# davidcombei/xAI-Audio-Deepfakes

Measured on AMD Instinct MI355X. Metric: explanations/sec (16 kHz, 4 s clips), higher is better.
Workload: dtype f32; 1 GPU; BASELINE config 2 extended to the full explanation: batch 64 x 4 s clips, STFT + wav2vec2-base embedder (to hidden layer 9) + logreg + U-Net mask decoder + masked ISTFT x2 + embedder re-forward x2 + LMAC metrics; batch_per_gpu=64, clip_samples=64000, embedder=wav2vec2-base (seeded random weights)

## Files before the change

include/addvisor_hip.h:

```cpp
#ifndef ADDVISOR_HIP_H
#define ADDVISOR_HIP_H

#include <stdint.h>

#ifdef __cplusplus
extern "C" {
#endif

typedef void* advh_stream_t;

enum {
    ADVH_OK = 0,
    ADVH_EINVAL = -1,
    ADVH_ELAUNCH = -2,
    ADVH_ENOTINIT = -3,
    ADVH_EUNSUPPORTED = -4
};

const char* advh_version(void);

int advh_init(void);

int advh_set_option(const char* name, int value);

int advh_stft_forward(const float* wave, int64_t wave_stride, int n_in, int B, int L, int hop, int win,
                      const float* window, float* X, float* mag, float* phase, int T, advh_stream_t stream);

enum { ADVH_MASK_NONE = 0, ADVH_MASK_LINEAR = 1, ADVH_MASK_LOG1P = 2 };
int advh_istft_masked(const float* mag, const float* phase, const float* mask, int Fm, int Tm, int mode,
                      float* wave_in, float* wave_out, int64_t wave_stride, int B, int T, int L, int hop,
                      int win, const float* window, advh_stream_t stream);

int advh_istft_masked_c64(const float* spec, const float* mask, int Fm, int Tm, int mode, float* wave_in, float* wave_out,
                          int64_t wave_stride, int B, int T, int L, int hop, int win, const float* window,
                          advh_stream_t stream);

int advh_istft_c64(const float* spec, float* wave, int64_t wave_stride, int B, int T, int L, int hop, int win,
                   const float* window, advh_stream_t stream);

int advh_istft_bandswap(const float* spec_a, const float* spec_b, int k0, int kw, int nbands, float* waves,
                        int64_t wave_stride, int64_t band_stride, int B, int T, int L, int hop, int win,
                        const float* window, advh_stream_t stream);

int advh_istft_masked_bwd(const float* g_wave, int64_t g_stride, const float* mag, const float* phase, const float* mask,
                          int Fm, int Tm, int mode, int which, float* dmask, int B, int T, int L, int hop, int win,
                          const float* window, advh_stream_t stream);

enum { ADVH_ACT_NONE = 0, ADVH_ACT_GELU = 1, ADVH_ACT_LEAKY = 2 };
enum { ADVH_TILE_AUTO = 0, ADVH_TILE_128x128 = 1, ADVH_TILE_256x64 = 2, ADVH_TILE_256x32 = 3,
       ADVH_TILE_256x128_W8 = 9, ADVH_TILE_128x256_W8 = 10  };

typedef struct advh_gemm_desc {
    const void* A0;
    const void* A1;
    const void* W;
    const int32_t* ktab;
    const float* bias;
    const void* resid;
    void* out_h;
    void* out_f;
    int32_t M, N, Ktot, w_rows;
    int32_t Hg, Wg, h0, h1, w0, w1, halo_zero;
    int64_t a_sB[2], a_sH[2], a_sW[2], a_c0[2], a_sZ[2];
    int64_t w_sZ, bias_sZ;
    int64_t o_sB, o_sH, o_sW, o_c0, o_sNhi, o_sZ;
    int32_t n_div, nz;
    int32_t act;
    float slope;
    int32_t resid_f32;
    int32_t ktab_identity;
    void* out_h2;
    float slope2;
    int32_t ph_r, ph_pad, ph_T;
    void* out_pre;
    const void* dact_src;
    int32_t wide;
    int64_t w_ld;
    int32_t sc;
    int32_t n_sub;
    int64_t o_sNhh;
    int32_t nz_lo, z_inner;
    int64_t a_sZ2[2];
    int64_t o_sZ2;
    int32_t plain;
    int32_t plain_out;
    int32_t split;
    int64_t a_lo[2];
    int64_t w_lo;
    int64_t o_lo;
} advh_gemm_desc;

int advh_gemm_f16(const advh_gemm_desc* desc, int tile, advh_stream_t stream);

int advh_w2v2_frontend(const float* wave, int64_t wave_stride, int n_in, int B, int L, const float* w0,
                       const float* bias0, const float* gamma, const float* beta, int mode, int normalize, float* stats_ws,
                       float* norm_ws, float* mr_ws, void* out, int T0, int P0, int C0, advh_stream_t stream);

int advh_layernorm(const void* in, int in_is_f32, int64_t in_ld, const float* gamma, const float* beta,
                   float* out_f, void* out_h, int64_t out_ld, int M, int C, float eps, int gelu,
                   advh_stream_t stream);
int advh_layernorm_add(const void* in, int in_is_f32, int64_t in_ld, const void* add_h, int64_t add_ld, const float* gamma,
                       const float* beta, float* out_f, void* out_h, int64_t out_ld, int M, int C, float eps, int gelu,
                       advh_stream_t stream);

int advh_posconv_gather(const float* h, void* xg, int B, int T, int H, int G, int K, int pad_left, const void* dact_src,
                        advh_stream_t stream);

typedef struct advh_posconv_desc {
    const void* xg;
    const void* W;
    const float* bias;
    const float* resid;
    float* out;
    int B, T, H, G, K;
} advh_posconv_desc;
int advh_posconv_tile_f16(const advh_posconv_desc* d, advh_stream_t stream);
int advh_posconv_tile_lds_bytes(int Cg, int T);

int advh_attention_f16(const void* qkv, void* ctx, int B, int T, int H, int heads, advh_stream_t stream);

int advh_pool_logreg(const float* h, const float* coef, float intercept, float* logit, float* prob,
                     float* pooled, int B, int T, int H, advh_stream_t stream);

int advh_unet_stem(const float* mag, int Fq, int Tq, int B, int H, int W, const float* wgt, const float* bias,
                   void* out, int PH, int PW, float slope, advh_stream_t stream);
int advh_unet_pack_x(const float* mag, int Fq, int Tq, int B, int H, int W, void* cat, int C, int c0, int PH, int PW,
                     advh_stream_t stream);
int advh_unet_head(const void* y, int B, int H, int W, int PH, int PW, const float* wgt, float bias, float* mask,
                   float* logits, advh_stream_t stream);

int advh_lmac_metrics_accumulate(const float* predictions, const float* theta_out, const float* masked_predictions,
                                 int n, double* sums6, float* per_clip, advh_stream_t stream);

int advh_hifigan_pack_mel(const float* mel, void* out, int B, int C, int T, int halo, advh_stream_t stream);
int advh_hifigan_pack_mel_pad(const float* mel, void* out, int B, int C, int T, int pad, int halo, advh_stream_t stream);
int advh_halo_fill_f16(void* x, int B, int T, int C, int halo, int mode, advh_stream_t stream);
int advh_hifigan_mrf_mix(const void* a, const void* b, const void* c, void* y, float slope, int64_t numel, advh_stream_t stream);
int advh_hifigan_conv_post(const void* x, const float* w, float bias, float* wav, int B, int C, int T, int halo, int k,
                           advh_stream_t stream);
int advh_mel_log(const float* mag, const float* fb, float* out, int B, int F, int T, int n_mels, advh_stream_t stream);

int advh_layernorm_bwd(const void* x, int x_is_f32, const void* dy, int dy_is_f32, const float* gamma, const float* beta,
                       int gelu_fwd, const float* add, const void* dact_src, float* out_f, void* out_h, int M, int C,
                       float eps, int remap_T, int remap_P, advh_stream_t stream);
int advh_attention_bwd_f16(const void* qkv, const void* dctx, void* dqkv, int B, int T, int H, int heads, advh_stream_t stream);
int advh_pool_logreg_bwd(const float* coef, const float* dlogit, float* dh, void* dh16, int B, int T, int H, advh_stream_t stream);
int advh_w2v2_frontend_bwd_group(const float* wave, int64_t wave_stride, int n_in, int B, int L, const float* w0,
                                 const float* gamma, const float* stats_ws, const float* norm_ws, const float* mr_ws,
                                 const void* dy0, float* part_ws, float* sums_ws, void* dz0, int T0, int P0, int C0,
                                 advh_stream_t stream);
int advh_wave_bwd(const float* g, const float* wave, int64_t wave_stride, int n_in, int B, int L, const float* stats_ws,
                  float* dxhat_ws, float* part_ws, int normalize, float out_scale, float* dx, int64_t dx_stride, int T0, int P0,
                  advh_stream_t stream);
int advh_scale_rows(const float* x, int x_rows, const float* alpha, float* y, int rows, int64_t n, int accumulate,
                    advh_stream_t stream);
int advh_attr_finalize(const float* g, const float* x, float* out, int mode, int64_t total, advh_stream_t stream);
int advh_time_mask(const float* attr, float* mask, float* wave_in, float* wave_out, const float* wave, int B, int64_t n,
                   advh_stream_t stream);

typedef struct advh_path_desc {
    const float* x;
    const float* base;
    const int32_t* bidx;
    int64_t n;
    uint64_t seed;
    int B, S, base_rows;
    int clip_major;
    float sigma;
} advh_path_desc;
int advh_attr_path_points(const advh_path_desc* d, const float* alpha, int64_t row0, int rows, float* out, advh_stream_t stream);
int advh_attr_path_accumulate(const advh_path_desc* d, const float* grad, const float* w, int mode, int64_t row0, int rows,
                              float* total, float* row_sum, advh_stream_t stream);
int advh_philox_normal(uint64_t seed, int64_t row0, int rows, int64_t n, int raw, float* out, advh_stream_t stream);

int advh_nt_fold(const float* attr, int B, int p, int64_t n, double* sum, double* sumsq, advh_stream_t stream);
int advh_nt_finalize(const double* sum, const double* sumsq, int B, int64_t n, int S, int nt_type, float* out, advh_stream_t stream);

typedef struct advh_metric_desc {
    const float* x;
    const float* attr;
    const float* base;
    int64_t n;
    uint64_t seed;
    int B, S, s0, p;
    int base_rows;
    int mode;
    int mul;
    float scale;
} advh_metric_desc;
int advh_metric_rows(const advh_metric_desc* d, int64_t row0, int rows, float* out, float* dot, advh_stream_t stream);
int advh_metric_row_dot(const float* pert, const float* attr, int B, int p, int64_t n, float* dot, advh_stream_t stream);
int advh_infidelity_fold(const float* dot, const float* f0, const float* fk, int B, int p, int normalize, double* acc, advh_stream_t stream);
int advh_infidelity_finalize(const double* acc, int B, int S, int normalize, float* out, advh_stream_t stream);
int advh_row_norm(const float* v, int rows, int64_t n, int ord, float* out, advh_stream_t stream);
int advh_sensitivity_fold(const float* e, const float* et, const float* enorm, int B, int p, int64_t n, int ord, float* ratio,
                          float* smax, advh_stream_t stream);

typedef struct advh_ablation_desc {
    const float* x;
    const float* base;
    const int32_t* mask;
    int64_t n;
    int B, base_rows, mask_rows;
    int mode;
    int win, stride;
    int K;
} advh_ablation_desc;
int advh_ablation_points(const advh_ablation_desc* d, int64_t row0, int rows, float* out, advh_stream_t stream);
int advh_ablation_accumulate(const advh_ablation_desc* d, const float* f0, const float* fk, float* attr, advh_stream_t stream);

typedef struct advh_coalition_desc {
    const float* x;
    const float* base;
    const int32_t* index;
    const int32_t* rank;
    const uint8_t* present;
    int64_t n;
    int64_t p0;
    int64_t rows;
    int B, base_rows, index_rows;
    int mode;
    int K;
    int P;
} advh_coalition_desc;
int advh_coalition_points(const advh_coalition_desc* d, int64_t row0, int rows, float* out, advh_stream_t stream);
int advh_shapley_accumulate(const advh_coalition_desc* d, const float* fbase, const float* fk, int64_t p0, int np, float* total,
                            float finalize_div, advh_stream_t stream);
int advh_coalition_scatter(const advh_coalition_desc* d, const float* coef, float* attr, advh_stream_t stream);

typedef struct advh_permutation_desc {
    const float* x;
    const int32_t* index;
    const int32_t* perm;
    int64_t n;
    int B, K;
} advh_permutation_desc;
int advh_permutation_points(const advh_permutation_desc* d, int64_t row0, int rows, float* out, advh_stream_t stream);
int advh_row_similarity(const float* rows_ptr, const float* x, int64_t row0, int rows, int B, int64_t n, int mode, float kernel_width,
                        float* sim, advh_stream_t stream);
int advh_lasso_cd(const double* X, const double* y, int S, int K, double alpha, double tol, int max_iter, double* coef, double* gap,
                  int* iters);

int advh_split_overflow(int reset);
int advh_w2v2_frontend_split(const float* wave, int64_t wave_stride, int n_in, int B, int L, const float* w0,
                             const float* bias0, const float* gamma, const float* beta, int mode, int normalize, float* stats_ws,
                             float* norm_ws, float* mr_ws, void* out, int64_t out_lo, int T0, int P0, int C0, advh_stream_t stream);
int advh_layernorm_split(const void* in, int in_is_f32, int64_t in_ld, int64_t in_lo, const void* add_h, int64_t add_ld,
                         int64_t add_lo, const float* gamma, const float* beta, float* out_f, void* out_h, int64_t out_ld,
                         int64_t out_lo, int M, int C, float eps, int gelu, advh_stream_t stream);
int advh_posconv_gather_split(const float* h, void* xg, int64_t xg_lo, int B, int T, int H, int G, int K, int pad_left,
                              advh_stream_t stream);
int advh_attention_split(const void* qkv, int64_t qkv_lo, void* ctx, int64_t ctx_lo, int B, int T, int H, int heads,
                         advh_stream_t stream);
int advh_unet_stem_split(const float* mag, int Fq, int Tq, int B, int H, int W, const float* wgt, const float* bias,
                         void* out, int64_t out_lo, int PH, int PW, float slope, advh_stream_t stream);
int advh_unet_pack_x_split(const float* mag, int Fq, int Tq, int B, int H, int W, void* cat, int64_t cat_lo, int C, int c0,
                           int PH, int PW, advh_stream_t stream);
int advh_unet_head_split(const void* y, int64_t y_lo, int B, int H, int W, int PH, int PW, const float* wgt, float bias,
                         float* mask, float* logits, advh_stream_t stream);
int advh_layernorm_bwd_split(const void* x, int x_is_f32, int64_t x_lo, const void* dy, int dy_is_f32, int64_t dy_lo,
                             const float* gamma, const float* beta, int gelu_fwd, const float* add, const void* dact_src,
                             int64_t dact_lo, float* out_f, void* out_h, int64_t out_lo, int M, int C, float eps, int remap_T,
                             int remap_P, advh_stream_t stream);
int advh_attention_bwd_split(const void* qkv, int64_t qkv_lo, const void* dctx, int64_t dctx_lo, void* dqkv, int64_t dqkv_lo,
                             int B, int T, int H, int heads, advh_stream_t stream);
int advh_pool_logreg_bwd_split(const float* coef, const float* dlogit, float* dh, void* dh16, int64_t dh16_lo, int B, int T, int H,
                               advh_stream_t stream);
int advh_split_f32(const float* src, void* dst, int64_t dst_lo, int64_t n, advh_stream_t stream);
int advh_posconv_gather_bwd_split(const float* dh, void* xg, int64_t xg_lo, int B, int T, int H, int G, int K, int pad_left,
                                  const void* dact_src, int64_t dact_lo, advh_stream_t stream);
int advh_w2v2_frontend_bwd_group_split(const float* wave, int64_t wave_stride, int n_in, int B, int L, const float* w0,
                                       const float* gamma, const float* stats_ws, const float* norm_ws, const float* mr_ws,
                                       const void* dy0, int64_t dy_lo, float* part_ws, float* sums_ws, void* dz0, int64_t dz_lo,
                                       int T0, int P0, int C0, advh_stream_t stream);
typedef struct advh_resblock_x3_desc {
    const void* X;
    const void* W1;
    const float* b1;
    const void* W2;
    const float* b2;
    void* out_h;
    int M, Wg, w0, w1, k, dil;
    float slope;
    int64_t x_lo, o_lo, w_lo;
} advh_resblock_x3_desc;
int advh_resblock_pair_x3_lds_bytes(int C, int k, int dil);
int advh_resblock_pair_x3(const advh_resblock_x3_desc* d, int C, advh_stream_t stream);
int advh_hifigan_pack_mel_split(const float* mel, void* out, int64_t out_lo, int B, int C, int T, int pad, int halo,
                                advh_stream_t stream);
int advh_hifigan_mrf_mix_split(const void* a, const void* b, const void* c, void* y, float slope, int64_t numel, int64_t lo,
                               advh_stream_t stream);
int advh_hifigan_conv_post_split(const void* x, int64_t x_lo, const float* w, float bias, float* wav, int B, int C, int T, int halo,
                                 int k, advh_stream_t stream);

typedef struct advh_taps_desc {
    const void* X;
    const void* W;
    const float* bias;
    const void* resid;
    void* out_h;
    void* out_h2;
    int M, Hg, Wg, h0, h1, w0, w1;
    int ntap;
    int toff[16];
    int act;
    float slope, slope2;
    int pre_act;
    float pre_slope;
} advh_taps_desc;
int advh_conv_taps_split_tile(int C, int ntap, int span);
int advh_conv_taps_split(const advh_taps_desc* d, int C, int64_t x_lo, int64_t w_lo, int64_t r_lo, int64_t o_lo, advh_stream_t stream);
typedef struct advh_taps2d_desc {
    const void* X;
    const void* W;
    const float* bias;
    void* out_h;
    int B, H, W_, PH, PW;
    int act;
    float slope;
} advh_taps2d_desc;
int advh_conv_taps2d_f16(const advh_taps2d_desc* d, int C, advh_stream_t stream);
int advh_conv_taps2d_split_lds_bytes(int C);
int advh_conv_taps2d_split(const advh_taps2d_desc* d, int C, int64_t x_lo, int64_t w_lo, int64_t o_lo, advh_stream_t stream);
typedef struct advh_upconv_desc {
    const void* Xc;
    const void* Xs;
    const void* W;
    const float* bias;
    void* out_h;
    int B, Hc, W_, PHc, PWc, PHs, PWs, PHo, PWo;
    int act;
    float slope;
} advh_upconv_desc;
int advh_upconv21_tile_f16(const advh_upconv_desc* d, advh_stream_t stream);
int advh_upconv21_tile_lds_bytes(void);
typedef struct advh_convs21_desc {
    const void* X;
    const void* W;
    const float* bias;
    void* out_h;
    int B, Ho, W_, PHi, PWi, PHo, PWo;
    int act;
    float slope;
} advh_convs21_desc;
int advh_conv53s21_tile_f16(const advh_convs21_desc* d, advh_stream_t stream);
int advh_conv53s21_tile_lds_bytes(void);
int advh_conv_taps_tile(int C, int ntap, int span);
int advh_conv_taps_lds_bytes(int C, int ntap, int span);
int advh_conv_taps_f16(const advh_taps_desc* d, int C, advh_stream_t stream);

typedef struct advh_map_geom { int B, H, W, C, PH, PW; } advh_map_geom;
int advh_bn_partial_count(void);
int advh_bn_coef(const float* sums, const float* gamma, const float* beta, int C, float n, float eps, float momentum,
                 float* running_mean, float* running_var, int64_t* num_batches_tracked, float* coef, advh_stream_t stream);
int advh_bn_bwd_coef(const float* sums, const float* coef, int C, float n, float inv_scale, float* coef_b, float* dgamma,
                     float* dbeta, advh_stream_t stream);
int advh_bn_stats(const void* z, const advh_map_geom* g, float* partial, float* sums, advh_stream_t stream);
int advh_bn_apply(const void* z, const advh_map_geom* g, const float* coef, float slope, void* a, advh_stream_t stream);
int advh_bn_bwd_sums(const void* z, const void* g_a, int g_f32, const advh_map_geom* g, const float* coef, float slope,
                     float* partial, float* sums, advh_stream_t stream);
int advh_bn_bwd_apply(const void* z, const void* g_a, int g_f32, const advh_map_geom* g, const float* coef, const float* coef_b, float slope,
                      void* dz, int64_t d_sB, int64_t d_sH, int64_t d_sW, int64_t d_c0, advh_stream_t stream);
typedef struct advh_transpose_desc {
    int B, Hg, Wg, GH, GW, H, W;
    int Hs, Ws, PHs, PWs, Cs, c0, nC;
    int sy, sx, ntap, oy[16], ox[16];
    int64_t ld, col0;
    int rpt, r0;
} advh_transpose_desc;
int advh_transpose_gather(const void* src, void* dst, const advh_transpose_desc* d, advh_stream_t stream);
int advh_unet_head_bwd(const float* dmask, const float* mask, const float* w32, float scale, int64_t total, float* dlogit,
                       void* dy1, int dy_f32, advh_stream_t stream);
int advh_unet_head_wgrad(const float* dlogit, const void* y1, int64_t total, float* partial, float* dw33, advh_stream_t stream);
int advh_unet_stem_wgrad(const void* dz, int Fq, int Tq, int B, int H, int W, const float* mag, int PH, int PW,
                         float* partial, float* dw, advh_stream_t stream);

int advh_bn_stats_split(const void* z, int64_t z_lo, const advh_map_geom* g, float* partial, float* sums, advh_stream_t stream);
int advh_bn_apply_split(const void* z, int64_t z_lo, const advh_map_geom* g, const float* coef, float slope, void* a, int64_t a_lo,
                        advh_stream_t stream);
int advh_bn_bwd_sums_split(const void* z, int64_t z_lo, const void* g_a, int64_t g_lo, const advh_map_geom* g, const float* coef,
                           float slope, float* partial, float* sums, advh_stream_t stream);
int advh_bn_bwd_apply_split(const void* z, int64_t z_lo, const void* g_a, int64_t g_lo, const advh_map_geom* g, const float* coef,
                            const float* coef_b, float slope, void* dz, int64_t dz_lo, int64_t d_sB, int64_t d_sH, int64_t d_sW,
                            int64_t d_c0, advh_stream_t stream);
int advh_unet_head_bwd_split(const float* dmask, const float* mask, const float* w32, float scale, int64_t total, float* dlogit,
                             void* dy1, int64_t dy_lo, advh_stream_t stream);
int advh_unet_head_wgrad_split(const float* dlogit, const void* y1, int64_t y_lo, int64_t total, float* partial, float* dw33,
                               advh_stream_t stream);
int advh_unet_stem_wgrad_split(const void* dz, int64_t dz_lo, int Fq, int Tq, int B, int H, int W, const float* mag, int PH, int PW,
                               float* partial, float* dw, advh_stream_t stream);
int advh_unet_skip_wgrad(const void* dz, int Fq, int Tq, int B, int H, int W, const float* mag, int PH, int PW, float* partial, float* dw,
                         advh_stream_t stream);
int advh_unet_skip_wgrad_split(const void* dz, int64_t dz_lo, int Fq, int Tq, int B, int H, int W, const float* mag, int PH, int PW,
                               float* partial, float* dw, advh_stream_t stream);

typedef struct advh_wgrad2d_desc {
    const void* X;
    const void* DZ;
    float* partial;
    int B, H, W_, PHx, PWx, PHz, PWz;
} advh_wgrad2d_desc;
int advh_conv_wgrad2d_parts(int C, int B, int H, int W);
int advh_conv_wgrad2d_f16(const advh_wgrad2d_desc* d, int C, float* dw, advh_stream_t stream);
int advh_conv_wgrad2d_split_parts(int CI, int CO, int B, int H, int W);
int advh_conv_wgrad2d_split(const advh_wgrad2d_desc* d, int CI, int CO, int Cx, int cx0, int Cz, int cz0, int64_t x_lo, int64_t dz_lo,
                            float* dw, advh_stream_t stream);

typedef struct advh_resblock_desc {
    const void* X;
    const void* W1;
    const float* b1;
    const void* W2;
    const float* b2;
    void* out_h;
    int M, Wg, w0, w1, k, dil;
    float slope;
} advh_resblock_desc;
int advh_resblock_pair_lds_bytes(int C, int k, int dil);
int advh_resblock_pair_f16(const advh_resblock_desc* d, int C, advh_stream_t stream);

#ifdef __cplusplus
}
#endif
#endif
```

xai-audio-deepfakes_amd/addvisor_hip/_lib.py:

```python
from __future__ import annotations

import ctypes as C
import os
import subprocess

_HERE = os.path.dirname(os.path.abspath(__file__))
LIB_PATH = os.environ.get("ADDVISOR_HIP_LIB") or os.path.join(_HERE, "libaddvisor_hip.so")
CSRC = os.path.join(os.path.dirname(_HERE), "csrc")

ERRORS = {-1: "ADVH_EINVAL (bad argument)", -2: "ADVH_ELAUNCH (HIP launch failed)",
          -3: "ADVH_ENOTINIT (advh_init not called)", -4: "ADVH_EUNSUPPORTED"}


class AdvhError(RuntimeError):
    pass


def build(verbose: bool = False) -> str:
    r = subprocess.run(["make", "-C", CSRC, "-j8"], capture_output=True, text=True)
    if r.returncode != 0:
        raise AdvhError("building libaddvisor_hip.so failed:\n" + r.stdout[-4000:] + r.stderr[-4000:])
    if verbose:
        print(r.stdout)
    return LIB_PATH


_p, _i, _i64, _f = C.c_void_p, C.c_int, C.c_int64, C.c_float

SIGNATURES = {
    "advh_version": (C.c_char_p, []),
    "advh_init": (_i, []),
    "advh_set_option": (_i, [C.c_char_p, _i]),
    "advh_stft_forward": (_i, [_p, _i64, _i, _i, _i, _i, _i, _p, _p, _p, _p, _i, _p]),
    "advh_istft_masked": (_i, [_p, _p, _p, _i, _i, _i, _p, _p, _i64, _i, _i, _i, _i, _i, _p, _p]),
    "advh_istft_masked_c64": (_i, [_p, _p, _i, _i, _i, _p, _p, _i64, _i, _i, _i, _i, _i, _p, _p]),
    "advh_istft_c64": (_i, [_p, _p, _i64, _i, _i, _i, _i, _i, _p, _p]),
    "advh_gemm_f16": (_i, [_p, _i, _p]),
    "advh_w2v2_frontend": (_i, [_p, _i64, _i, _i, _i, _p, _p, _p, _p, _i, _i, _p, _p, _p, _p, _i, _i, _i, _p]),
    "advh_layernorm": (_i, [_p, _i, _i64, _p, _p, _p, _p, _i64, _i, _i, _f, _i, _p]),
    "advh_layernorm_add": (_i, [_p, _i, _i64, _p, _i64, _p, _p, _p, _p, _i64, _i, _i, _f, _i, _p]),
    "advh_posconv_gather": (_i, [_p, _p, _i, _i, _i, _i, _i, _i, _p, _p]),
    "advh_attention_f16": (_i, [_p, _p, _i, _i, _i, _i, _p]),
    "advh_pool_logreg": (_i, [_p, _p, _f, _p, _p, _p, _i, _i, _i, _p]),
    "advh_unet_stem": (_i, [_p, _i, _i, _i, _i, _i, _p, _p, _p, _i, _i, _f, _p]),
    "advh_unet_pack_x": (_i, [_p, _i, _i, _i, _i, _i, _p, _i, _i, _i, _i, _p]),
    "advh_unet_head": (_i, [_p, _i, _i, _i, _i, _i, _p, _f, _p, _p, _p]),
    "advh_lmac_metrics_accumulate": (_i, [_p, _p, _p, _i, _p, _p, _p]),
    "advh_hifigan_pack_mel": (_i, [_p, _p, _i, _i, _i, _i, _p]),
    "advh_hifigan_pack_mel_pad": (_i, [_p, _p, _i, _i, _i, _i, _i, _p]),
    "advh_halo_fill_f16": (_i, [_p, _i, _i, _i, _i, _i, _p]),
    "advh_hifigan_mrf_mix": (_i, [_p, _p, _p, _p, _f, _i64, _p]),
    "advh_hifigan_conv_post": (_i, [_p, _p, _f, _p, _i, _i, _i, _i, _i, _p]),
    "advh_mel_log": (_i, [_p, _p, _p, _i, _i, _i, _i, _p]),
    "advh_layernorm_bwd": (_i, [_p, _i, _p, _i, _p, _p, _i, _p, _p, _p, _p, _i, _i, _f, _i, _i, _p]),
    "advh_attention_bwd_f16": (_i, [_p, _p, _p, _i, _i, _i, _i, _p]),
    "advh_pool_logreg_bwd": (_i, [_p, _p, _p, _p, _i, _i, _i, _p]),
    "advh_w2v2_frontend_bwd_group": (_i, [_p, _i64, _i, _i, _i, _p, _p, _p, _p, _p, _p, _p, _p, _p, _i, _i, _i, _p]),
    "advh_wave_bwd": (_i, [_p, _p, _i64, _i, _i, _i, _p, _p, _p, _i, _f, _p, _i64, _i, _i, _p]),
    "advh_scale_rows": (_i, [_p, _i, _p, _p, _i, _i64, _i, _p]),
    "advh_attr_finalize": (_i, [_p, _p, _p, _i, _i64, _p]),
    "advh_time_mask": (_i, [_p, _p, _p, _p, _p, _i, _i64, _p]),
    "advh_attr_path_points": (_i, [_p, _p, _i64, _i, _p, _p]),
    "advh_attr_path_accumulate": (_i, [_p, _p, _p, _i, _i64, _i, _p, _p, _p]),
    "advh_philox_normal": (_i, [C.c_uint64, _i64, _i, _i64, _i, _p, _p]),
    "advh_nt_fold": (_i, [_p, _i, _i, _i64, _p, _p, _p]),
    "advh_nt_finalize": (_i, [_p, _p, _i, _i64, _i, _i, _p, _p]),
    "advh_metric_rows": (_i, [_p, _i64, _i, _p, _p, _p]),
    "advh_metric_row_dot": (_i, [_p, _p, _i, _i, _i64, _p, _p]),
    "advh_infidelity_fold": (_i, [_p, _p, _p, _i, _i, _i, _p, _p]),
    "advh_infidelity_finalize": (_i, [_p, _i, _i, _i, _p, _p]),
    "advh_row_norm": (_i, [_p, _i, _i64, _i, _p, _p]),
    "advh_sensitivity_fold": (_i, [_p, _p, _p, _i, _i, _i64, _i, _p, _p, _p]),
    "advh_ablation_points": (_i, [_p, _i64, _i, _p, _p]),
    "advh_ablation_accumulate": (_i, [_p, _p, _p, _p, _p]),
    "advh_coalition_points": (_i, [_p, _i64, _i, _p, _p]),
    "advh_shapley_accumulate": (_i, [_p, _p, _p, _i64, _i, _p, _f, _p]),
    "advh_coalition_scatter": (_i, [_p, _p, _p, _p]),
    "advh_permutation_points": (_i, [_p, _i64, _i, _p, _p]),
    "advh_row_similarity": (_i, [_p, _p, _i64, _i, _i, _i64, _i, _f, _p, _p]),
    "advh_lasso_cd": (_i, [_p, _p, _i, _i, C.c_double, C.c_double, _i, _p, _p, _p]),
    "advh_istft_masked_bwd": (_i, [_p, _i64, _p, _p, _p, _i, _i, _i, _i, _p, _i, _i, _i, _i, _i, _p, _p]),
    "advh_istft_bandswap": (_i, [_p, _p, _i, _i, _i, _p, _i64, _i64, _i, _i, _i, _i, _i, _p, _p]),
    "advh_bn_partial_count": (_i, []),
    "advh_bn_stats": (_i, [_p, _p, _p, _p, _p]),
    "advh_bn_coef": (_i, [_p, _p, _p, _i, _f, _f, _f, _p, _p, _p, _p, _p]),
    "advh_bn_bwd_coef": (_i, [_p, _p, _i, _f, _f, _p, _p, _p, _p]),
    "advh_bn_apply": (_i, [_p, _p, _p, _f, _p, _p]),
    "advh_bn_bwd_sums": (_i, [_p, _p, _i, _p, _p, _f, _p, _p, _p]),
    "advh_bn_bwd_apply": (_i, [_p, _p, _i, _p, _p, _p, _f, _p, _i64, _i64, _i64, _i64, _p]),
    "advh_transpose_gather": (_i, [_p, _p, _p, _p]),
    "advh_split_f32": (_i, [_p, _p, _i64, _i64, _p]),
    "advh_unet_head_bwd": (_i, [_p, _p, _p, _f, _i64, _p, _p, _i, _p]),
    "advh_unet_head_wgrad": (_i, [_p, _p, _i64, _p, _p, _p]),
    "advh_unet_stem_wgrad": (_i, [_p, _i, _i, _i, _i, _i, _p, _i, _i, _p, _p, _p]),
    "advh_conv_wgrad2d_parts": (_i, [_i, _i, _i, _i]),
    "advh_conv_wgrad2d_f16": (_i, [_p, _i, _p, _p]),
    "advh_conv_wgrad2d_split_parts": (_i, [_i, _i, _i, _i, _i]),
    "advh_conv_wgrad2d_split": (_i, [_p, _i, _i, _i, _i, _i, _i, _i64, _i64, _p, _p]),
    "advh_resblock_pair_lds_bytes": (_i, [_i, _i, _i]),
    "advh_resblock_pair_f16": (_i, [_p, _i, _p]),
    "advh_conv_taps_tile": (_i, [_i, _i, _i]),
    "advh_conv_taps_lds_bytes": (_i, [_i, _i, _i]),
    "advh_conv_taps_f16": (_i, [_p, _i, _p]),
    "advh_conv_taps_split_tile": (_i, [_i, _i, _i]),
    "advh_conv_taps_split": (_i, [_p, _i, _i64, _i64, _i64, _i64, _p]),
    "advh_conv_taps2d_f16": (_i, [_p, _i, _p]),
    "advh_conv_taps2d_split_lds_bytes": (_i, [_i]),
    "advh_conv_taps2d_split": (_i, [_p, _i, _i64, _i64, _i64, _p]),
    "advh_upconv21_tile_f16": (_i, [_p, _p]),
    "advh_posconv_tile_f16": (_i, [_p, _p]),
    "advh_conv53s21_tile_f16": (_i, [_p, _p]),
    "advh_conv53s21_tile_lds_bytes": (_i, []),
    "advh_posconv_tile_lds_bytes": (_i, [_i, _i]),
    "advh_w2v2_frontend_split": (_i, [_p, _i64, _i, _i, _i, _p, _p, _p, _p, _i, _i, _p, _p, _p, _p, _i64, _i, _i, _i, _p]),
    "advh_layernorm_split": (_i, [_p, _i, _i64, _i64, _p, _i64, _i64, _p, _p, _p, _p, _i64, _i64, _i, _i, _f, _i, _p]),
    "advh_posconv_gather_split": (_i, [_p, _p, _i64, _i, _i, _i, _i, _i, _i, _p]),
    "advh_attention_split": (_i, [_p, _i64, _p, _i64, _i, _i, _i, _i, _p]),
    "advh_unet_stem_split": (_i, [_p, _i, _i, _i, _i, _i, _p, _p, _p, _i64, _i, _i, _f, _p]),
    "advh_unet_pack_x_split": (_i, [_p, _i, _i, _i, _i, _i, _p, _i64, _i, _i, _i, _i, _p]),
    "advh_hifigan_pack_mel_split": (_i, [_p, _p, _i64, _i, _i, _i, _i, _i, _p]),
    "advh_hifigan_mrf_mix_split": (_i, [_p, _p, _p, _p, _f, _i64, _i64, _p]),
    "advh_hifigan_conv_post_split": (_i, [_p, _i64, _p, _f, _p, _i, _i, _i, _i, _i, _p]),
    "advh_unet_head_split": (_i, [_p, _i64, _i, _i, _i, _i, _i, _p, _f, _p, _p, _p]),
    "advh_upconv21_tile_lds_bytes": (_i, []),
    "advh_bn_stats_split": (_i, [_p, _i64, _p, _p, _p, _p]),
    "advh_bn_apply_split": (_i, [_p, _i64, _p, _p, _f, _p, _i64, _p]),
    "advh_bn_bwd_sums_split": (_i, [_p, _i64, _p, _i64, _p, _p, _f, _p, _p, _p]),
    "advh_bn_bwd_apply_split": (_i, [_p, _i64, _p, _i64, _p, _p, _p, _f, _p, _i64, _i64, _i64, _i64, _i64, _p]),
    "advh_unet_head_bwd_split": (_i, [_p, _p, _p, _f, _i64, _p, _p, _i64, _p]),
    "advh_unet_head_wgrad_split": (_i, [_p, _p, _i64, _i64, _p, _p, _p]),
    "advh_unet_stem_wgrad_split": (_i, [_p, _i64, _i, _i, _i, _i, _i, _p, _i, _i, _p, _p, _p]),
    "advh_unet_skip_wgrad": (_i, [_p, _i, _i, _i, _i, _i, _p, _i, _i, _p, _p, _p]),
    "advh_unet_skip_wgrad_split": (_i, [_p, _i64, _i, _i, _i, _i, _i, _p, _i, _i, _p, _p, _p]),
    "advh_split_overflow": (_i, [_i]),
    "advh_resblock_pair_x3_lds_bytes": (_i, [_i, _i, _i]),
    "advh_resblock_pair_x3": (_i, [_p, _i, _p]),
    "advh_layernorm_bwd_split": (_i, [_p, _i, _i64, _p, _i, _i64, _p, _p, _i, _p, _p, _i64, _p, _p, _i64, _i, _i, _f, _i, _i, _p]),
    "advh_attention_bwd_split": (_i, [_p, _i64, _p, _i64, _p, _i64, _i, _i, _i, _i, _p]),
    "advh_pool_logreg_bwd_split": (_i, [_p, _p, _p, _p, _i64, _i, _i, _i, _p]),
    "advh_posconv_gather_bwd_split": (_i, [_p, _p, _i64, _i, _i, _i, _i, _i, _i, _p, _i64, _p]),
    "advh_w2v2_frontend_bwd_group_split": (_i, [_p, _i64, _i, _i, _i, _p, _p, _p, _p, _p, _p, _i64, _p, _p, _p, _i64, _i, _i, _i, _p]),
}

_lib = None


def lib() -> C.CDLL:
    global _lib
    if _lib is None:
        import torch
        if not os.path.exists(LIB_PATH):
            raise AdvhError(f"{LIB_PATH} is missing: run `python -c 'import __graft_entry__ as g; g.build()'` "
                            "(there is no fallback path)")
        l = C.CDLL(LIB_PATH)
        for name, (res, args) in SIGNATURES.items():
            fn = getattr(l, name)
            fn.restype, fn.argtypes = res, args
        _lib = l
    return _lib


class SplitRangeError(AdvhError, FloatingPointError):
    """A kernel of the fp32-class mode met a value outside the split format's range (|x| > 65504)."""


def check_overflow(what: str = "") -> None:
    if _lib is not None and _lib.advh_split_overflow(1):
        raise SplitRangeError((what + ": " if what else "") + "a value left the fp32-class format's range (|x| > 65504 between two "
                              "matrix products): the split planes saturated.  Scale the input / weights, or run precision='f16' "
                              "diagnostics; the reference's fp32 has no such limit (include/addvisor_hip.h, advh_split_overflow)")


def check(rc: int, what: str) -> None:
    if rc != 0:
        raise AdvhError(f"{what}: {ERRORS.get(rc, rc)}")
    check_overflow(what)


_inited = set()


def init() -> None:
    import torch
    dev = torch.cuda.current_device() if torch.cuda.is_available() else -1
    if dev not in _inited:
        check(lib().advh_init(), "advh_init")
        _inited.add(dev)
```

xai-audio-deepfakes_amd/addvisor_hip/gemm.py:

```python
from __future__ import annotations

import ctypes as C
import os
from dataclasses import dataclass
from typing import Optional, Sequence, Tuple

import numpy as np
import torch

from . import _lib

BK = 64
ACT = {"none": 0, "gelu": 1, "leaky": 2}
WIDE_EPILOGUE = os.environ.get("ADDVISOR_GEMM_WIDE", "1") != "0"


def packed_row_channel(rows: int) -> np.ndarray:
    R = np.arange(rows)
    return ((R >> 5) << 5) + (((R >> 2) & 3) << 3) + (((R >> 4) & 1) << 2) + (R & 3)
TILE_AUTO, TILE_128x128, TILE_256x64, TILE_256x32 = 0, 1, 2, 3
TILE_256x128_W8, TILE_128x256_W8 = 9, 10
TILE_BN = {TILE_128x128: 128, TILE_256x64: 64, TILE_256x32: 32, TILE_256x128_W8: 128, TILE_128x256_W8: 256}
TILE_NAMES = {TILE_128x128: "128x128", TILE_256x64: "256x64", TILE_256x32: "256x32", TILE_256x128_W8: "256x128w8", TILE_128x256_W8: "128x256w8"}
TILE_KERNELS = {TILE_128x128: "gemm_f16_kernel<128, 128, 2, 2, 4>", TILE_128x256_W8: "gemm_f16_kernel<128, 256, 2, 4, 3>",
                TILE_256x128_W8: "gemm_f16_kernel<256, 128, 4, 2, 3>"}


class GemmDesc(C.Structure):
    _fields_ = [
        ("A0", C.c_void_p), ("A1", C.c_void_p), ("W", C.c_void_p), ("ktab", C.c_void_p),
        ("bias", C.c_void_p), ("resid", C.c_void_p), ("out_h", C.c_void_p), ("out_f", C.c_void_p),
        ("M", C.c_int32), ("N", C.c_int32), ("Ktot", C.c_int32), ("w_rows", C.c_int32),
        ("Hg", C.c_int32), ("Wg", C.c_int32), ("h0", C.c_int32), ("h1", C.c_int32),
        ("w0", C.c_int32), ("w1", C.c_int32), ("halo_zero", C.c_int32),
        ("a_sB", C.c_int64 * 2), ("a_sH", C.c_int64 * 2), ("a_sW", C.c_int64 * 2),
        ("a_c0", C.c_int64 * 2), ("a_sZ", C.c_int64 * 2),
        ("w_sZ", C.c_int64), ("bias_sZ", C.c_int64),
        ("o_sB", C.c_int64), ("o_sH", C.c_int64), ("o_sW", C.c_int64), ("o_c0", C.c_int64),
        ("o_sNhi", C.c_int64), ("o_sZ", C.c_int64),
        ("n_div", C.c_int32), ("nz", C.c_int32), ("act", C.c_int32), ("slope", C.c_float),
        ("resid_f32", C.c_int32), ("ktab_identity", C.c_int32),
        ("out_h2", C.c_void_p), ("slope2", C.c_float), ("ph_r", C.c_int32), ("ph_pad", C.c_int32), ("ph_T", C.c_int32),
        ("out_pre", C.c_void_p), ("dact_src", C.c_void_p), ("wide", C.c_int32), ("w_ld", C.c_int64), ("sc", C.c_int32), ("n_sub", C.c_int32), ("o_sNhh", C.c_int64),
        ("nz_lo", C.c_int32), ("z_inner", C.c_int32), ("a_sZ2", C.c_int64 * 2), ("o_sZ2", C.c_int64), ("plain", C.c_int32), ("plain_out", C.c_int32),
        ("split", C.c_int32), ("a_lo", C.c_int64 * 2), ("w_lo", C.c_int64), ("o_lo", C.c_int64),
    ]


X3_KERNELS = {TILE_128x128: "gemm_x3_kernel<128, 128, 2, 2", TILE_256x64: "gemm_x3_kernel<256, 64, 4, 1", TILE_256x32: "gemm_x3_kernel<256, 32, 4, 1"}


def kernel_name(tile: int, plain: bool, split: bool = False) -> str:
    if split:
        return X3_KERNELS[tile] + (", true>" if plain else ", false>")
    k = TILE_KERNELS.get(tile, "gemm_f16_kernel")
    if k.startswith("gemm_f16_kernel<"):
        k = k[:-1] + (", true>" if plain and tile == TILE_128x128 else ", false>")
    return k


class _Profile:

    def __init__(self):
        self.reset(False)

    def reset(self, enabled: bool):
        self.enabled, self.events = enabled, []

    def summary(self, kernel=None):
        per = {}
        for a, b, f, t, shape in self.events:
            r = per.setdefault(kernel_name(t, shape[4], shape[5] if len(shape) > 5 else False), [0.0, 0.0, 0])
            r[0] += a.elapsed_time(b); r[1] += f; r[2] += 1
        if not per:
            return 0.0, 0.0, 0
        if kernel is None:
            kernel = max(per, key=lambda k: per[k][0])
        self.kernel = kernel
        return tuple(per.get(kernel, (0.0, 0.0, 0)))

    def by_shape(self):
        per = {}
        for a, b, f, t, shape in self.events:
            r = per.setdefault(shape[:4] + (TILE_NAMES.get(t, str(t)) + ("+" if shape[4] else "") + ("x3" if len(shape) > 5 and shape[5] else ""),), [0.0, 0.0, 0])
            r[0] += a.elapsed_time(b); r[1] += f; r[2] += 1
        return per


PROFILE = _Profile()


class _Tuner:
    active = False
    log = []


TUNER = _Tuner()


def round_up(x: int, m: int) -> int:
    return (x + m - 1) // m * m


def split_planes(x: torch.Tensor) -> torch.Tensor:
    if x.is_cuda and x.dtype == torch.float32 and x.numel() % 4 == 0:
        src = x.detach().contiguous()
        if src.data_ptr() % 16:
            src = src.clone()
        out = torch.empty((2,) + tuple(src.shape), dtype=torch.float16, device=src.device)
        if src.numel():
            _lib.check(_lib.lib().advh_split_f32(src.data_ptr(), out.data_ptr(), src.numel(), src.numel(),
                                                 torch.cuda.current_stream(src.device).cuda_stream), "advh_split_f32")
        return out
    x64 = x.detach().to(torch.float64)
    bad = ~(x64.abs() <= 65504.0)
    if bool(bad.any()):
        raise ValueError(f"split format: {int(bad.sum())} value(s) outside |x| <= 65504 (or NaN); max |x| = {float(x64.abs().nan_to_num(float('inf')).max()):g}")
    hi = x64.to(torch.float16)
    hi = torch.where(x64.abs() < 2.0 ** -14, torch.zeros_like(hi), hi)
    lo = ((x64 - hi.to(torch.float64)) * 2048.0).to(torch.float16)
    return torch.stack([hi, lo])


def join_planes(t: torch.Tensor) -> torch.Tensor:
    return t[0].float() + t[1].float() * (1.0 / 2048.0)


W8_RULE = int(os.environ.get("ADDVISOR_GEMM_W8_MIN_M", "0"))
X3_SUPER_COLUMN_BYTES = int(os.environ.get("ADDVISOR_X3_SC_BYTES", "1600000"))
SUPER_COLUMN_BYTES = int(os.environ.get("ADDVISOR_GEMM_SC_BYTES", "1600000"))


def super_columns(N: int, Kp: int, M: int, bn: int = 128, split: bool = False) -> int:
    bpe = 4 if split else 2
    budget = X3_SUPER_COLUMN_BYTES if split else SUPER_COLUMN_BYTES
    if budget <= 0 or N <= bn:
        return 0
    tiles_n = (N + bn - 1) // bn
    if tiles_n * bn * Kp * bpe <= 3 * 1024 * 1024:
        return 0
    sc = min(tiles_n, budget // (bn * Kp * bpe))
    return sc if sc >= (3 if split else 4) else 0


PLAIN_ROWS = os.environ.get("ADDVISOR_GEMM_PLAIN", "1") != "0"


def pick_tile(N: int, M: int = 0) -> Tuple[int, int]:
    if N <= 32:
        return TILE_256x32, 32
    if N <= 64:
        return TILE_256x64, 64
    return TILE_128x128, 128


@dataclass
class Source:
    sB: int
    sH: int
    sW: int
    c0: int
    sZ: int = 0
    sZ2: int = 0


class GemmPlan:

    def __init__(self, *, M: int, N: int, w2: torch.Tensor, ktab: np.ndarray, sources: Sequence[Source],
                 Hg: int, Wg: int, window: Tuple[int, int, int, int], halo_zero: bool,
                 out: Tuple[int, int, int, int], n_div: Optional[int] = None, o_sNhi: int = 0,
                 o_sZ: int = 0, nz: int = 1, bias: Optional[torch.Tensor] = None, act: str = "none",
                 slope: float = 0.0, device=None, w_sZ: Optional[int] = None, bias_sZ: int = 0,
                 slope2: float = 0.0, phase: Tuple[int, int, int] = (0, 0, 0), cache: Optional[tuple] = None,
                 n_sub: int = 0, o_sNhh: int = 0, nz_lo: int = 0, z_inner: bool = False, o_sZ2: int = 0, plain: bool = False,
                 split: bool = False):
        K = 8 * len(ktab)
        self.split = bool(split)
        Kp = round_up(K, BK)
        n_div_v = n_div if n_div is not None else round_up(N, 4)
        wide = WIDE_EPILOGUE and N % 8 == 0 and n_div_v % 8 == 0 and all(int(x) % 8 == 0 for x in (*out, o_sNhi, o_sZ, o_sNhh, o_sZ2))
        tile, BN = pick_tile(N, M)
        if W8_RULE and N % 256 == 0 and M >= W8_RULE and bool((np.asarray(ktab) == np.arange(len(ktab))).all()):
            tile, BN = TILE_128x256_W8, 256
        w_rows = round_up(N, 256)
        store, ckey = cache if cache is not None else (None, None)
        hit = store.get(ckey) if store is not None else None
        if hit is None:
            w2t = w2() if callable(w2) else w2
            assert w2t.dim() == 3 and w2t.shape[0] == nz and w2t.shape[1] == N and w2t.shape[2] == K, (w2t.shape, nz, N, K)
            wp = torch.zeros(((2, nz, w_rows, Kp) if split else (nz, w_rows, Kp)), dtype=torch.float16)
            w16 = split_planes(w2t) if split else w2t.to(torch.float16)
            if wide:
                src = packed_row_channel(w_rows)
                keep = src < N
                wp[..., torch.from_numpy(np.nonzero(keep)[0]), :K] = w16[..., torch.from_numpy(src[keep]), :]
            else:
                wp[..., :N, :K] = w16
            wd = wp.to(device) if device is not None else wp
            bd = None
            if bias is not None:
                assert bias.numel() == nz * N or bias_sZ == 0
                bd = bias.to(torch.float32).contiguous()
                bd = bd.to(device) if device is not None else bd
            hit = (wd, bd, wide)
            if store is not None:
                store[ckey] = hit
        assert hit[2] == wide, "a cached packed weight is shared between plans of different output alignment"
        kt = np.concatenate([ktab, np.full((Kp - K) // 8, ktab[0], dtype=np.int64)]).astype(np.int64)
        assert (kt & 0x7FFFFFFF).max() < 2 ** 31
        self.ktab_host = kt
        self.K, self.Kp, self.tile, self.BN = K, Kp, tile, BN
        self.device = device
        self.w, self.bias = hit[0], hit[1]
        kt32 = torch.from_numpy(kt.astype(np.uint32).view(np.int32).copy())
        self.ktab = kt32.to(device) if device is not None else kt32
        d = GemmDesc()
        d.M, d.N, d.Ktot, d.w_rows = M, N, Kp, w_rows
        d.Hg, d.Wg = Hg, Wg
        d.h0, d.h1, d.w0, d.w1 = window
        d.halo_zero = int(halo_zero)
        for s, src in enumerate(sources):
            d.a_sB[s], d.a_sH[s], d.a_sW[s], d.a_c0[s], d.a_sZ[s] = src.sB, src.sH, src.sW, src.c0, src.sZ
            d.a_sZ2[s] = src.sZ2
        d.w_sZ = w_rows * Kp if w_sZ is None else w_sZ
        d.split = int(split)
        d.w_lo = nz * w_rows * Kp if split else 0
        assert not split or w_sZ is None
        d.bias_sZ = bias_sZ
        d.o_sB, d.o_sH, d.o_sW, d.o_c0 = out
        d.o_sNhi, d.o_sZ = o_sNhi, o_sZ
        d.n_sub, d.o_sNhh = n_sub, o_sNhh
        d.nz_lo, d.z_inner, d.o_sZ2 = nz_lo, int(z_inner), o_sZ2
        assert nz_lo <= 1 or nz % nz_lo == 0
        d.n_div = n_div_v
        d.wide = int(wide)
        d.nz = nz
        d.act, d.slope = ACT[act], slope
        d.slope2 = slope2
        d.ph_r, d.ph_pad, d.ph_T = phase
        d.ktab_identity = int(bool((kt == np.arange(len(kt))).all()))
        d.plain = int(bool(plain and PLAIN_ROWS and d.ktab_identity and len(sources) == 1))
        if d.plain:
            src = sources[0]
            assert Hg == 1 or src.sH == Wg * src.sW, "plain rows need h * a_sH == (h * Wg) * a_sW"
            assert M <= Hg * Wg or src.sB == Hg * Wg * src.sW, "plain rows need b * a_sB == (b * Hg * Wg) * a_sW"
        o_sB, o_sH, o_sW, _ = out
        d.plain_out = int(bool(d.plain and n_div_v >= N and phase[0] == 0 and n_sub <= 1 and tuple(window) == (0, Hg, 0, Wg)
                               and (Hg == 1 or o_sH == Wg * o_sW) and (M <= Hg * Wg or o_sB == Hg * Wg * o_sW)))
        d.sc = super_columns(N, Kp, M, 128, split)
        self.desc = d
        self.nsrc = len(sources)
        self.flops = 2.0 * M * N * K * nz

    def load_weights(self, w2: torch.Tensor, bias: Optional[torch.Tensor] = None):
        N, K = self.desc.N, self.K
        assert w2.shape == (self.desc.nz, N, K) and w2.device == self.w.device, (w2.shape, (self.desc.nz, N, K))
        w16 = split_planes(w2) if self.split else w2.to(torch.float16)
        if self.desc.wide:
            if not hasattr(self, "_perm"):
                src = packed_row_channel(self.w.shape[-2])
                keep = np.nonzero(src < N)[0]
                self._perm = (torch.from_numpy(keep).to(self.w.device), torch.from_numpy(src[keep]).to(self.w.device))
            dst_rows, src_rows = self._perm
            self.w[..., dst_rows, :K] = w16[..., src_rows, :]
        else:
            self.w[..., :N, :K] = w16
        if bias is not None:
            self.bias.copy_(bias.reshape(self.bias.shape).to(torch.float32))

    def run(self, A0: torch.Tensor, A1: Optional[torch.Tensor] = None, *, out_h: Optional[torch.Tensor] = None,
            out_f: Optional[torch.Tensor] = None, resid: Optional[torch.Tensor] = None, stream: Optional[int] = None,
            out_h2: Optional[torch.Tensor] = None, out_pre: Optional[torch.Tensor] = None,
            dact_src: Optional[torch.Tensor] = None):
        d = self.desc
        d.out_h2 = out_h2.data_ptr() if out_h2 is not None else None
        d.out_pre = out_pre.data_ptr() if out_pre is not None else None
        d.dact_src = dact_src.data_ptr() if dact_src is not None else None
        assert out_pre is None or out_pre.dtype == torch.float16
        assert dact_src is None or dact_src.dtype == torch.float16
        assert A0.dtype == torch.float16 and A0.is_cuda
        if self.split:
            o_lo = None
            for s_, t in enumerate((A0, A1)):
                if t is not None:
                    assert t.shape[0] == 2 and t.stride(0) % 8 == 0, "split operand must be a [2, ...] plane pair"
                    d.a_lo[s_] = t.stride(0) // 8
            for t in (out_h, out_h2, out_pre, dact_src, resid if (resid is not None and resid.dtype == torch.float16) else None):
                if t is not None:
                    assert t.shape[0] == 2 and t.stride(0) % 8 == 0 and o_lo in (None, t.stride(0)), "split outputs share one plane pitch"
                    o_lo = t.stride(0)
            d.o_lo = o_lo or 0
        d.A0 = A0.data_ptr()
        d.A1 = A1.data_ptr() if A1 is not None else None
        assert (A1 is not None) == (self.nsrc == 2)
        if d.plain:
            plane = A0.stride(0) if self.split else A0.numel()
            need = (int(d.a_c0[0]) + (d.M - 1) * int(d.a_sW[0])) * 8 + d.Ktot + int(d.a_sZ[0]) * 8 * max(0, d.nz - 1)
            if need > plane:
                raise ValueError(f"affine-row GEMM operand too small: the plan reads {need} halfs per plane, the tensor holds {plane} "
                                 "(missing slack rows behind the buffer?)")
        d.W, d.ktab = self.w.data_ptr(), self.ktab.data_ptr()
        d.bias = self.bias.data_ptr() if self.bias is not None else None
        d.out_h = out_h.data_ptr() if out_h is not None else None
        d.out_f = out_f.data_ptr() if out_f is not None else None
        if out_h is not None:
            assert out_h.dtype == torch.float16
        if out_f is not None:
            assert out_f.dtype == torch.float32
        if resid is not None:
            assert resid.dtype in (torch.float16, torch.float32)
            d.resid, d.resid_f32 = resid.data_ptr(), int(resid.dtype == torch.float32)
        else:
            d.resid, d.resid_f32 = None, 0
        if stream is None:
            stream = torch.cuda.current_stream().cuda_stream
        if self.split:
            d.sc = super_columns(d.N, self.Kp, d.M, TILE_BN.get(self.tile, 128), True)
        if TUNER.active and not getattr(self, "_tuned", False):
            self._tune(d, stream)
        prof = PROFILE.enabled and self.tile not in (TILE_256x64, TILE_256x32)
        if prof:
            e0, e1 = torch.cuda.Event(enable_timing=True), torch.cuda.Event(enable_timing=True)
            e0.record()
        _lib.check(_lib.lib().advh_gemm_f16(C.byref(d), self.tile, stream), "advh_gemm_f16")
        if prof:
            e1.record()
            PROFILE.events.append((e0, e1, self.flops, self.tile, (self.desc.M, self.desc.N, self.K, self.desc.nz, bool(self.desc.plain), self.split)))


def _tune(self, d, stream):
    cands = [TILE_128x128, TILE_128x256_W8, TILE_256x128_W8] if (self.desc.N > 64 and not self.split) else [self.tile]
    best, best_ms = self.tile, None
    if len(cands) > 1:
        for t in cands:
            _lib.check(_lib.lib().advh_gemm_f16(C.byref(d), t, stream), "advh_gemm_f16")
            e0, e1 = torch.cuda.Event(enable_timing=True), torch.cuda.Event(enable_timing=True)
            e0.record()
            for _ in range(3):
                _lib.check(_lib.lib().advh_gemm_f16(C.byref(d), t, stream), "advh_gemm_f16")
            e1.record()
            e1.synchronize()
            ms = e0.elapsed_time(e1) / 3
            if best_ms is None or ms < best_ms:
                best, best_ms = t, ms
        TUNER.log.append((self.desc.M, self.desc.N, self.K, self.desc.nz, TILE_NAMES[best], best_ms))
    self.tile, self._tuned = best, True


GemmPlan._tune = _tune


@dataclass
class FMap:
    B: int
    H: int
    W: int
    C: int
    PH: int
    PW: int
    t: Optional[torch.Tensor] = None
    split: bool = False

    @property
    def Hp(self):
        return self.H + 2 * self.PH

    @property
    def Wp(self):
        return self.W + 2 * self.PW

    def alloc(self, device):
        shape = (self.B, self.Hp, self.Wp, self.C)
        self.t = torch.zeros(((2,) + shape) if self.split else shape, dtype=torch.float16, device=device)
        return self

    def interior(self) -> torch.Tensor:
        t = self.t[0] if self.split else self.t
        return t[:, self.PH:self.PH + self.H, self.PW:self.PW + self.W, :]


def plan_linear(M: int, weight: torch.Tensor, bias: Optional[torch.Tensor], *, lda: Optional[int] = None,
                ldo: Optional[int] = None, o_c0: int = 0, act: str = "none", device=None, cache=None,
                split: bool = False) -> GemmPlan:
    N, K = weight.shape
    assert K % 8 == 0
    lda = K if lda is None else lda
    ldo = N if ldo is None else ldo
    assert lda % 8 == 0 and ldo % 4 == 0
    return GemmPlan(M=M, N=N, w2=lambda: weight[None].float(), ktab=np.arange(K // 8, dtype=np.int64),
                    sources=[Source(0, 0, lda // 8, 0)], Hg=1, Wg=M, window=(0, 1, 0, M), halo_zero=False,
                    out=(0, 0, ldo, o_c0), bias=bias, act=act, device=device, cache=cache, plain=True, split=split)


def plan_conv1d_cl(B: int, P_in: int, P_out: int, L_out: int, weight: torch.Tensor, bias: Optional[torch.Tensor],
                   stride: int, *, act: str = "gelu", compact_out: bool = False, device=None, cache=None,
                   slack_rows: int = 0, split: bool = False) -> GemmPlan:
    Cout, Cin, k = weight.shape
    assert Cin % 8 == 0
    w2 = lambda: weight.permute(0, 2, 1).reshape(1, Cout, k * Cin).float()
    out = (L_out * Cout, 0, Cout, 0) if compact_out else (P_out * Cout, 0, Cout, 0)
    return GemmPlan(M=B * P_out, N=Cout, w2=w2, ktab=np.arange(k * Cin // 8, dtype=np.int64),
                    sources=[Source(P_in * Cin // 8, 0, stride * Cin // 8, 0)], Hg=1, Wg=P_out,
                    window=(0, 1, 0, L_out), halo_zero=not compact_out, out=out, bias=bias, act=act, device=device,
                    cache=cache, plain=(slack_rows >= k - stride and P_in == P_out * stride), split=split)


def plan_conv2d(srcs: Sequence[FMap], dst: FMap, weight: torch.Tensor, bias: Optional[torch.Tensor], *,
                stride=(1, 1), padding=(1, 1), dilation=(1, 1), act: str = "leaky", slope: float = 0.2,
                dst_c0: int = 0, device=None) -> GemmPlan:
    Cout, Cin, KH, KW = weight.shape
    assert sum(s.C for s in srcs) == Cin and len(srcs) <= 2
    sh, sw = stride
    ph, pw = padding
    dh, dw = dilation
    B = dst.B
    Ho = (srcs[0].H + 2 * ph - dh * (KH - 1) - 1) // sh + 1
    Wo = (srcs[0].W + 2 * pw - dw * (KW - 1) - 1) // sw + 1
    assert (Ho, Wo) == (dst.H, dst.W), ((Ho, Wo), (dst.H, dst.W))
    ktabs, ws, sources = [], [], []
    c_lo = 0
    for s, f in enumerate(srcs):
        assert f.C % 8 == 0 and f.PH >= ph and f.PW >= pw and (f.H, f.W, f.B) == (srcs[0].H, srcs[0].W, B)
        cc = f.C // 8
        taps = (np.arange(KH)[:, None] * dh * f.Wp + np.arange(KW)[None, :] * dw).reshape(-1)
        kt = (taps[:, None] * cc + np.arange(cc)[None, :]).reshape(-1).astype(np.int64) | (s << 31)
        ktabs.append(kt)
        ws.append(weight[:, c_lo:c_lo + f.C].permute(0, 2, 3, 1).reshape(Cout, KH * KW * f.C))
        c0 = ((-sh * dst.PH + f.PH - ph) * f.Wp + (-sw * dst.PW + f.PW - pw)) * cc
        sources.append(Source(f.Hp * f.Wp * cc, sh * f.Wp * cc, sw * cc, c0))
        c_lo += f.C
    Ct = dst.C
    split = dst.split
    assert all(f.split == split for f in srcs)
    return GemmPlan(M=B * dst.Hp * dst.Wp, N=Cout, w2=torch.cat(ws, 1)[None] if split else torch.cat(ws, 1)[None].float(), ktab=np.concatenate(ktabs), split=split,
                    sources=sources, Hg=dst.Hp, Wg=dst.Wp,
                    window=(dst.PH, dst.PH + dst.H, dst.PW, dst.PW + dst.W), halo_zero=True,
                    out=(dst.Hp * dst.Wp * Ct, dst.Wp * Ct, Ct, dst_c0), bias=bias, act=act, slope=slope,
                    device=device)


def plan_convT2d(src: FMap, dst: FMap, weight: torch.Tensor, bias: torch.Tensor, *, stride, dst_c0: int = 0,
                 device=None) -> GemmPlan:
    Cin, Cout, KH, KW = weight.shape
    sh, sw = stride
    assert (KH, KW) == (sh, sw) and src.C == Cin and Cin % 8 == 0 and Cout % 4 == 0
    assert (dst.H, dst.W) == (src.H * sh, src.W * sw)
    cc = Cin // 8
    Ct = dst.C
    w2 = weight.permute(2, 3, 1, 0).reshape(1, sh * sw * Cout, Cin)
    w2 = w2 if dst.split else w2.float()
    assert src.split == dst.split
    b2 = bias.float().repeat(sh * sw)
    o_c0 = ((-sh * src.PH + dst.PH) * dst.Wp + (-sw * src.PW + dst.PW)) * Ct + dst_c0
    return GemmPlan(M=src.B * src.Hp * src.Wp, N=sh * sw * Cout, w2=w2, ktab=np.arange(cc, dtype=np.int64),
                    sources=[Source(src.Hp * src.Wp * cc, src.Wp * cc, cc, 0)], Hg=src.Hp, Wg=src.Wp,
                    window=(src.PH, src.PH + src.H, src.PW, src.PW + src.W), halo_zero=False,
                    out=(dst.Hp * dst.Wp * Ct, sh * dst.Wp * Ct, sw * Ct, o_c0), n_div=Cout,
                    o_sNhi=Ct if sw > 1 else dst.Wp * Ct, n_sub=sw if sw > 1 else 0, o_sNhh=dst.Wp * Ct if sw > 1 else 0,
                    bias=b2, bias_sZ=0, act="none", device=device, split=dst.split)


class PlanGroup:

    def __init__(self, plans: Sequence[GemmPlan], flops: float):
        self.plans, self.flops = list(plans), flops
        self.tile = self.plans[0].tile

    def run(self, A0: torch.Tensor, A1: Optional[torch.Tensor] = None, *, out_h: torch.Tensor, stream: Optional[int] = None):
        for p in self.plans:
            p.run(A0, A1, out_h=out_h, stream=stream)


def add_indicator(f: FMap, channel: int) -> FMap:
    f.interior()[..., channel] = 1.0
    return f


def compose_upconv_weights(wt: torch.Tensor, bt: torch.Tensor, wc: torch.Tensor, stride, indicator: Tuple[str, int]):
    sh, sw = stride
    Cb, Cu = wt.shape[:2]
    N, Cs = wc.shape[0], wc.shape[1] - Cu
    where, ich = indicator
    assert where in ("coarse", "skip") and ich >= (Cb if where == "coarse" else Cs)
    wt64, wc64, bt64 = wt.double(), wc.double(), bt.double()
    nth, ntw = 2, (2 if sw == 2 else 3)
    cu0 = (max(Cb, ich + 1 if where == "coarse" else 0) + 7) // 8
    cu1 = (max(Cs, ich + 1 if where == "skip" else 0) + 7) // 8
    w1 = torch.zeros(N, 3, 3, cu1 * 8, dtype=torch.float64)
    w1[..., :Cs] = wc64[:, Cu:].permute(0, 2, 3, 1)
    if where == "skip":
        w1[..., ich] = torch.einsum("nukl,u->nkl", wc64[:, :Cu], bt64)
    w2 = []
    for ph in range(sh):
        dh_min = (ph - 1) // sh
        for pw in range(sw):
            dw_min = (pw - 1) // sw
            w0 = torch.zeros(N, nth, ntw, cu0 * 8, dtype=torch.float64)
            for kh in range(3):
                for kw in range(3):
                    r, c = ph + kh - 1, pw + kw - 1
                    ti, tj = r // sh - dh_min, c // sw - dw_min
                    w0[:, ti, tj, :Cb] += torch.einsum("nu,bu->nb", wc64[:, :Cu, kh, kw], wt64[:, :, r % sh, c % sw])
                    if where == "coarse":
                        w0[:, ti, tj, ich] += wc64[:, :Cu, kh, kw] @ bt64
            w2.append(torch.cat([w0.reshape(N, -1), w1.reshape(N, -1)], 1))
    return w2, cu0, cu1


def plan_upconv2d(coarse: FMap, skip: FMap, dst: FMap, wt: torch.Tensor, bt: torch.Tensor, wc: torch.Tensor,
                  bc: torch.Tensor, *, stride, coarse_C: int, skip_C: int, indicator: Tuple[str, int],
                  slope: float = 0.2, device=None) -> PlanGroup:
    sh, sw = stride
    Cb, Cu = wt.shape[:2]
    N = wc.shape[0]
    Cs = wc.shape[1] - Cu
    assert (wt.shape[2], wt.shape[3]) == (sh, sw) and sh == 2 and sw in (1, 2) and wc.shape[2:] == (3, 3)
    assert coarse_C == Cb and skip_C == Cs and coarse.C >= Cb and skip.C >= Cs and coarse.C % 8 == 0 and skip.C % 8 == 0
    assert (dst.H, dst.W) == (coarse.H * sh, coarse.W * sw) == (skip.H, skip.W) and dst.B == coarse.B == skip.B
    assert coarse.PH >= 1 and coarse.PW >= 1 and skip.PH >= 1 and skip.PW >= 1 and dst.C % 8 == 0
    nth, ntw = 2, (2 if sw == 2 else 3)
    cc0, cc1, Ct = coarse.C // 8, skip.C // 8, dst.C
    w2, cu0, cu1 = compose_upconv_weights(wt, bt, wc, stride, indicator)
    assert cu0 <= cc0 and cu1 <= cc1
    where = indicator[0]
    kt1 = ((np.arange(3)[:, None] * skip.Wp + np.arange(3)[None, :]).reshape(-1)[:, None] * cc1
           + np.arange(cu1)[None, :]).reshape(-1).astype(np.int64) | (1 << 31)
    kt0 = ((np.arange(nth)[:, None] * coarse.Wp + np.arange(ntw)[None, :]).reshape(-1)[:, None] * cc0
           + np.arange(cu0)[None, :]).reshape(-1).astype(np.int64)
    c0_0 = ((coarse.PH - 1) * coarse.Wp + coarse.PW - 1) * cc0
    c0_1 = ((skip.PH - 1) * skip.Wp + skip.PW - 1) * cc1
    o_c0 = (dst.PH * dst.Wp + dst.PW) * Ct
    plan = GemmPlan(
        M=coarse.B * coarse.H * coarse.W, N=N, w2=torch.stack(w2) if dst.split else torch.stack(w2).float(), ktab=np.concatenate([kt0, kt1]), split=dst.split,
        sources=[Source(coarse.Hp * coarse.Wp * cc0, coarse.Wp * cc0, cc0, c0_0, sZ=coarse.Wp * cc0, sZ2=cc0 if sw == 2 else 0),
                 Source(skip.Hp * skip.Wp * cc1, sh * skip.Wp * cc1, sw * cc1, c0_1, sZ=skip.Wp * cc1, sZ2=cc1 if sw == 2 else 0)],
        Hg=coarse.H, Wg=coarse.W, window=(0, coarse.H, 0, coarse.W), halo_zero=False,
        out=(dst.Hp * dst.Wp * Ct, sh * dst.Wp * Ct, sw * Ct, o_c0), o_sZ=dst.Wp * Ct, o_sZ2=Ct if sw == 2 else 0,
        nz=sh * sw, nz_lo=sw, z_inner=os.environ.get("ADDVISOR_UPCONV_Z_INNER", "1") != "0", bias=bc, bias_sZ=0, act="leaky", slope=slope, device=device)
    plans = [plan]
    flops = 2.0 * dst.B * dst.H * dst.W * N * (nth * ntw * Cb + 9 * Cs + (nth * ntw if where == "coarse" else 9))
    return PlanGroup(plans, flops)


class ConvS21Desc(C.Structure):
    _fields_ = [("X", C.c_void_p), ("W", C.c_void_p), ("bias", C.c_void_p), ("out_h", C.c_void_p), ("B", C.c_int),
                ("Ho", C.c_int), ("W_", C.c_int), ("PHi", C.c_int), ("PWi", C.c_int), ("PHo", C.c_int), ("PWo", C.c_int),
                ("act", C.c_int), ("slope", C.c_float)]


def conv_s21_supported(srcs: Sequence[FMap], dst: FMap, weight: torch.Tensor, stride=(1, 1), padding=(1, 1),
                       dilation=(1, 1)) -> bool:
    return (len(srcs) == 1 and tuple(weight.shape) == (64, 32, 5, 3) and tuple(stride) == (2, 1) and tuple(padding) == (2, 1)
            and tuple(dilation) == (1, 1) and srcs[0].C == 32 and dst.C == 64 and srcs[0].PH >= 2 and srcs[0].PW >= 1
            and srcs[0].H == 2 * dst.H and srcs[0].W == dst.W)


class ConvS21TilePlan:

    def __init__(self, src: FMap, dst: FMap, weight: torch.Tensor, bias: torch.Tensor, *, slope: float = 0.2, device=None):
        assert conv_s21_supported([src], dst, weight, (2, 1), (2, 1))
        R = np.arange(64)
        ch = 32 * (R >> 5) + 8 * ((R >> 2) & 3) + 4 * ((R >> 4) & 1) + (R & 3)
        wp = weight.float()[torch.from_numpy(ch)].permute(2, 3, 0, 1).reshape(15, 64, 32).to(torch.float16).contiguous()
        self.w = wp.to(device) if device is not None else wp
        self.bias = bias.to(torch.float32).contiguous()
        self.bias = self.bias.to(device) if device is not None else self.bias
        d = ConvS21Desc()
        d.B, d.Ho, d.W_ = dst.B, dst.H, dst.W
        d.PHi, d.PWi, d.PHo, d.PWo = src.PH, src.PW, dst.PH, dst.PW
        d.act, d.slope = ACT["leaky"], slope
        self.desc = d
        self.numels = (src.B * src.Hp * src.Wp * 32, dst.B * dst.Hp * dst.Wp * 64)
        self.flops = 2.0 * dst.B * dst.H * dst.W * 64 * 32 * 15
        self.tile = None

    def run(self, A0: torch.Tensor, A1=None, *, out_h: torch.Tensor, stream: Optional[int] = None):
        d = self.desc
        for t, n in zip((A0, out_h), self.numels):
            assert t.dtype == torch.float16 and t.is_cuda and t.is_contiguous() and t.numel() == n
        d.X, d.W, d.bias, d.out_h = A0.data_ptr(), self.w.data_ptr(), self.bias.data_ptr(), out_h.data_ptr()
        if stream is None:
            stream = torch.cuda.current_stream().cuda_stream
        _lib.check(_lib.lib().advh_conv53s21_tile_f16(C.byref(d), stream), "advh_conv53s21_tile_f16")


class UpconvDesc(C.Structure):
    _fields_ = [("Xc", C.c_void_p), ("Xs", C.c_void_p), ("W", C.c_void_p), ("bias", C.c_void_p), ("out_h", C.c_void_p),
                ("B", C.c_int), ("Hc", C.c_int), ("W_", C.c_int), ("PHc", C.c_int), ("PWc", C.c_int), ("PHs", C.c_int),
                ("PWs", C.c_int), ("PHo", C.c_int), ("PWo", C.c_int), ("act", C.c_int), ("slope", C.c_float)]


def upconv_tile_supported(coarse: FMap, skip: FMap, dst: FMap, wt: torch.Tensor, wc: torch.Tensor, stride, indicator) -> bool:
    return (tuple(stride) == (2, 1) and tuple(wt.shape) == (64, 32, 2, 1) and tuple(wc.shape) == (32, 33, 3, 3)
            and coarse.C == 64 and skip.C == 8 and dst.C == 32 and tuple(indicator) == ("skip", 1) and coarse.H % 8 == 0
            and min(coarse.PH, coarse.PW, skip.PH, skip.PW) >= 1)


class UpconvTilePlan:

    def __init__(self, coarse: FMap, skip: FMap, dst: FMap, wt: torch.Tensor, bt: torch.Tensor, wc: torch.Tensor,
                 bc: torch.Tensor, *, slope: float = 0.2, device=None):
        assert upconv_tile_supported(coarse, skip, dst, wt, wc, (2, 1), ("skip", 1))
        w2, cu0, cu1 = compose_upconv_weights(wt, bt, wc, (2, 1), ("skip", 1))
        assert (cu0, cu1) == (8, 1) and w2[0].shape == (32, 456)
        R = np.arange(32)
        ch = 8 * ((R >> 2) & 3) + 4 * ((R >> 4) & 1) + (R & 3)
        wp = torch.zeros(2, 15, 32, 32, dtype=torch.float16)
        for ph in range(2):
            full = torch.zeros(32, 480, dtype=torch.float64)
            full[:, :456] = w2[ph]
            wp[ph] = full[torch.from_numpy(ch)].reshape(32, 15, 32).permute(1, 0, 2).to(torch.float16)
        self.w = wp.contiguous().to(device) if device is not None else wp.contiguous()
        self.bias = bc.to(torch.float32).contiguous()
        self.bias = self.bias.to(device) if device is not None else self.bias
        d = UpconvDesc()
        d.B, d.Hc, d.W_ = coarse.B, coarse.H, coarse.W
        d.PHc, d.PWc, d.PHs, d.PWs, d.PHo, d.PWo = coarse.PH, coarse.PW, skip.PH, skip.PW, dst.PH, dst.PW
        d.act, d.slope = ACT["leaky"], slope
        self.desc = d
        self.numels = (coarse.t.numel() if coarse.t is not None else 0, skip.t.numel() if skip.t is not None else 0,
                       dst.t.numel() if dst.t is not None else 0)
        self.flops = 2.0 * dst.B * dst.H * dst.W * 32 * (6 * 64 + 9 * 2)
        self.tile = None

    def run(self, A0: torch.Tensor, A1: torch.Tensor, *, out_h: torch.Tensor, stream: Optional[int] = None):
        d = self.desc
        for t, n in zip((A0, A1, out_h), self.numels):
            assert t.dtype == torch.float16 and t.is_cuda and t.is_contiguous() and (n == 0 or t.numel() == n)
        d.Xc, d.Xs, d.W, d.bias, d.out_h = A0.data_ptr(), A1.data_ptr(), self.w.data_ptr(), self.bias.data_ptr(), out_h.data_ptr()
        if stream is None:
            stream = torch.cuda.current_stream().cuda_stream
        _lib.check(_lib.lib().advh_upconv21_tile_f16(C.byref(d), stream), "advh_upconv21_tile_f16")


def replay_on_cpu(plan: GemmPlan, A0: torch.Tensor, A1: Optional[torch.Tensor], out_numel: int,
                  resid: Optional[torch.Tensor] = None, out_init: Optional[torch.Tensor] = None) -> torch.Tensor:
    d = plan.desc
    srcs = [A0.reshape(-1).float().numpy(), None if A1 is None else A1.reshape(-1).float().numpy()]
    W = plan.w.float().numpy()
    if d.wide:
        src = packed_row_channel(W.shape[1])
        Wl = np.zeros_like(W)
        Wl[:, src] = W
        W = Wl
    bias = None if plan.bias is None else plan.bias.numpy().reshape(-1)
    out = np.full(out_numel, np.nan, dtype=np.float32) if out_init is None else out_init.reshape(-1).float().numpy().copy()
    kt = plan.ktab_host
    sel, off = (kt >> 31).astype(np.int64), (kt & 0x7FFFFFFF).astype(np.int64)
    for z in range(d.nz):
        for m in range(d.M):
            w_, t_ = m % d.Wg, m // d.Wg
            h_, b_ = t_ % d.Hg, t_ // d.Hg
            ok = d.h0 <= h_ < d.h1 and d.w0 <= w_ < d.w1
            if not ok and not d.halo_zero:
                continue
            zh, zw = (z // d.nz_lo, z % d.nz_lo) if d.nz_lo > 1 else (z, 0)
            orow = b_ * d.o_sB + h_ * d.o_sH + w_ * d.o_sW + d.o_c0 + d.o_sZ * zh + d.o_sZ2 * zw
            cols = np.arange(d.N)
            qn = cols // d.n_div
            hi = (qn // d.n_sub) * d.o_sNhh + (qn % d.n_sub) * d.o_sNhi if d.n_sub > 1 else qn * d.o_sNhi
            o = orow + hi + cols % d.n_div
            if not ok:
                out[o] = 0.0
                continue
            row = np.empty(d.Ktot, dtype=np.float32)
            for c in range(d.Ktot // 8):
                s = sel[c]
                rb = b_ * d.a_sB[s] + h_ * d.a_sH[s] + w_ * d.a_sW[s] + d.a_c0[s] + d.a_sZ[s] * zh + d.a_sZ2[s] * zw
                a = (rb + off[c]) * 8
                row[c * 8:(c + 1) * 8] = srcs[s][a:a + 8]
            v = W[z, :d.N] @ row
            if bias is not None:
                v = v + bias[d.bias_sZ * z: d.bias_sZ * z + d.N]
            if d.act == 1:
                v = torch.nn.functional.gelu(torch.from_numpy(v)).numpy()
            elif d.act == 2:
                v = np.where(v > 0, v, d.slope * v)
            if resid is not None:
                v = v + resid.reshape(-1).float().numpy()[o]
            if d.ph_r > 0:
                to = w_ * d.ph_r + cols // d.n_div - d.ph_pad
                keep = (to >= 0) & (to < d.ph_T)
                o, v = o[keep], v[keep]
            out[o] = v
    return torch.from_numpy(out)


@dataclass
class Map1D:
    B: int
    T: int
    C: int
    halo: int
    t: Optional[torch.Tensor] = None
    split: bool = False

    @property
    def P(self):
        return self.T + 2 * self.halo

    def alloc(self, device):
        shape = (self.B, self.P, self.C)
        self.t = torch.zeros(((2,) + shape) if self.split else shape, dtype=torch.float16, device=device)
        return self

    def interior(self) -> torch.Tensor:
        t = self.t[0] if self.split else self.t
        return t[:, self.halo:self.halo + self.T]


def plan_conv1d_same(src: Map1D, dst: Map1D, weight: torch.Tensor, bias: Optional[torch.Tensor], *, dilation: int = 1,
                     act: str = "none", slope: float = 0.0, slope2: float = 0.0, device=None) -> GemmPlan:
    Cout, Cin, k = weight.shape
    pad = (k - 1) * dilation // 2
    assert src.C == Cin and Cin % 8 == 0 and src.halo >= pad and (src.B, src.T) == (dst.B, dst.T) and Cout <= dst.C
    cc = Cin // 8
    kt = (np.arange(k)[:, None] * dilation * cc + np.arange(cc)[None, :]).reshape(-1).astype(np.int64)
    w2 = weight.permute(0, 2, 1).reshape(1, Cout, k * Cin).float()
    assert src.split == dst.split
    return GemmPlan(M=dst.B * dst.P, N=Cout, w2=w2, ktab=kt,
                    sources=[Source(src.P * cc, 0, cc, (src.halo - dst.halo - pad) * cc)], Hg=1, Wg=dst.P,
                    window=(0, 1, dst.halo, dst.halo + dst.T), halo_zero=True, out=(dst.P * dst.C, 0, dst.C, 0),
                    bias=bias, act=act, slope=slope, slope2=slope2, device=device, split=dst.split)



class TapsDesc(C.Structure):
    _fields_ = [("X", C.c_void_p), ("W", C.c_void_p), ("bias", C.c_void_p), ("resid", C.c_void_p),
                ("out_h", C.c_void_p), ("out_h2", C.c_void_p),
                ("M", C.c_int), ("Hg", C.c_int), ("Wg", C.c_int), ("h0", C.c_int), ("h1", C.c_int),
                ("w0", C.c_int), ("w1", C.c_int), ("ntap", C.c_int), ("toff", C.c_int * 16),
                ("act", C.c_int), ("slope", C.c_float), ("slope2", C.c_float), ("pre_act", C.c_int), ("pre_slope", C.c_float)]


TAPS_MAX_LDS = 160 * 1024


def taps_tile(Cn: int, ntap: int, span: int) -> int:
    for nj in (4, 3, 2):
        if ntap * Cn * Cn * 2 + 2 * (((64 * nj + span) * (Cn // 8) + 63) // 64 * 64) * 16 <= TAPS_MAX_LDS:
            return 64 * nj
    return 0


def taps_lds_bytes(Cn: int, ntap: int, span: int) -> int:
    tt = taps_tile(Cn, ntap, span)
    return -1 if not tt else ntap * Cn * Cn * 2 + 2 * (((tt + span) * (Cn // 8) + 63) // 64 * 64) * 16


class TapsPlan:

    def __init__(self, *, M: int, Cn: int, w_taps: torch.Tensor, toff: Sequence[int], Hg: int, Wg: int,
                 window: Tuple[int, int, int, int], bias: Optional[torch.Tensor], act: str = "none",
                 slope: float = 0.0, slope2: float = 0.0, device=None, pre_slope: Optional[float] = None, split: bool = False):
        ntap = len(toff)
        assert w_taps.shape == (ntap, Cn, Cn) and Cn in (32, 64) and 0 < ntap <= 16
        span = max(max(toff), 0) - min(min(toff), 0)
        self.split = split
        if split:
            assert pre_slope is None and taps_split_tile(Cn, ntap, span) > 0
        else:
            assert taps_tile(Cn, ntap, span) > 0
        self.Cn, self.device = Cn, device
        self.w = split_planes(w_taps.double()).contiguous() if split else w_taps.to(torch.float16).contiguous()
        self.bias = None if bias is None else bias.to(torch.float32).contiguous()
        if device is not None:
            self.w = self.w.to(device)
            self.bias = None if self.bias is None else self.bias.to(device)
        d = TapsDesc()
        d.M, d.Hg, d.Wg = M, Hg, Wg
        d.h0, d.h1, d.w0, d.w1 = window
        d.ntap = ntap
        for i, t in enumerate(toff):
            d.toff[i] = int(t)
        d.act, d.slope, d.slope2 = ACT[act], slope, slope2
        d.pre_act, d.pre_slope = int(pre_slope is not None), float(pre_slope or 0.0)
        self.desc = d
        valid = (window[1] - window[0]) * (window[3] - window[2]) * (M // (Hg * Wg))
        self.flops = 2.0 * valid * Cn * Cn * ntap

    def run(self, A0: torch.Tensor, A1=None, *, out_h: torch.Tensor, resid: Optional[torch.Tensor] = None,
            out_h2: Optional[torch.Tensor] = None, stream: Optional[int] = None):
        d = self.desc
        planes = 2 if self.split else 1
        for t in (A0, out_h, resid, out_h2):
            assert t is None or (t.dtype == torch.float16 and t.is_cuda and t.numel() == planes * d.M * self.Cn and t.is_contiguous())
        d.X, d.W = A0.data_ptr(), self.w.data_ptr()
        d.bias = self.bias.data_ptr() if self.bias is not None else None
        d.resid = resid.data_ptr() if resid is not None else None
        d.out_h = out_h.data_ptr()
        d.out_h2 = out_h2.data_ptr() if out_h2 is not None else None
        if stream is None:
            stream = torch.cuda.current_stream().cuda_stream
        if self.split:
            n = d.M * self.Cn
            _lib.check(_lib.lib().advh_conv_taps_split(C.byref(d), self.Cn, n, self.w.stride(0), n if resid is not None else 0, n, stream),
                       "advh_conv_taps_split")
        else:
            _lib.check(_lib.lib().advh_conv_taps_f16(C.byref(d), self.Cn, stream), "advh_conv_taps_f16")


class Taps2dDesc(C.Structure):
    _fields_ = [("X", C.c_void_p), ("W", C.c_void_p), ("bias", C.c_void_p), ("out_h", C.c_void_p),
                ("B", C.c_int), ("H", C.c_int), ("W_", C.c_int), ("PH", C.c_int), ("PW", C.c_int),
                ("act", C.c_int), ("slope", C.c_float)]


def taps2d_supported(srcs: Sequence[FMap], dst: FMap, weight: torch.Tensor, stride=(1, 1), padding=(1, 1),
                     dilation=(1, 1)) -> bool:
    if len(srcs) != 1 or tuple(weight.shape[2:]) != (3, 3) or tuple(stride) != (1, 1) or tuple(padding) != (1, 1) \
            or tuple(dilation) != (1, 1):
        return False
    s, Cn = srcs[0], weight.shape[0]
    return (Cn in (32, 64) and weight.shape[1] == Cn and s.C == Cn and dst.C == Cn and s.PH >= 1 and s.PW >= 1
            and (s.B, s.H, s.W, s.PH, s.PW) == (dst.B, dst.H, dst.W, dst.PH, dst.PW))


class Taps2dPlan:

    def __init__(self, src: FMap, dst: FMap, weight: torch.Tensor, bias: Optional[torch.Tensor], *, act: str = "leaky",
                 slope: float = 0.2, device=None):
        assert taps2d_supported([src], dst, weight)
        Cn = weight.shape[0]
        self.Cn = Cn
        self.w = weight.permute(2, 3, 0, 1).reshape(9, Cn, Cn).to(torch.float16).contiguous()
        self.bias = None if bias is None else bias.to(torch.float32).contiguous()
        if device is not None:
            self.w = self.w.to(device)
            self.bias = None if self.bias is None else self.bias.to(device)
        d = Taps2dDesc()
        d.B, d.H, d.W_, d.PH, d.PW = dst.B, dst.H, dst.W, dst.PH, dst.PW
        d.act, d.slope = ACT[act], slope
        self.desc = d
        self.flops = 2.0 * dst.B * dst.H * dst.W * Cn * Cn * 9

    def run(self, A0: torch.Tensor, A1=None, *, out_h: torch.Tensor, stream: Optional[int] = None):
        d = self.desc
        n = d.B * (d.H + 2 * d.PH) * (d.W_ + 2 * d.PW) * self.Cn
        for t in (A0, out_h):
            assert t.dtype == torch.float16 and t.is_cuda and t.is_contiguous() and t.numel() == n
        d.X, d.W, d.out_h = A0.data_ptr(), self.w.data_ptr(), out_h.data_ptr()
        d.bias = self.bias.data_ptr() if self.bias is not None else None
        if stream is None:
            stream = torch.cuda.current_stream().cuda_stream
        _lib.check(_lib.lib().advh_conv_taps2d_f16(C.byref(d), self.Cn, stream), "advh_conv_taps2d_f16")


def taps2d_split_supported(srcs: Sequence[FMap], dst: FMap, weight: torch.Tensor, stride=(1, 1), padding=(1, 1),
                           dilation=(1, 1)) -> bool:
    return (len(srcs) == 1 and srcs[0].split and dst.split
            and taps2d_supported(srcs, dst, weight, stride=stride, padding=padding, dilation=dilation))


class Taps2dSplitPlan:

    def __init__(self, src: FMap, dst: FMap, weight: torch.Tensor, bias: Optional[torch.Tensor], *, act: str = "leaky",
                 slope: float = 0.2, device=None):
        assert taps2d_split_supported([src], dst, weight)
        Cn = weight.shape[0]
        self.Cn = Cn
        self.w = split_planes(weight.permute(2, 3, 0, 1).reshape(9, Cn, Cn)).contiguous()
        self.bias = None if bias is None else bias.to(torch.float32).contiguous()
        if device is not None:
            self.w = self.w.to(device)
            self.bias = None if self.bias is None else self.bias.to(device)
        d = Taps2dDesc()
        d.B, d.H, d.W_, d.PH, d.PW = dst.B, dst.H, dst.W, dst.PH, dst.PW
        d.act, d.slope = ACT[act], slope
        self.desc = d
        self.flops = 2.0 * dst.B * dst.H * dst.W * Cn * Cn * 9

    def run(self, A0: torch.Tensor, A1=None, *, out_h: torch.Tensor, stream: Optional[int] = None):
        d = self.desc
        n = d.B * (d.H + 2 * d.PH) * (d.W_ + 2 * d.PW) * self.Cn
        for t in (A0, out_h):
            assert t.dtype == torch.float16 and t.is_cuda and t.is_contiguous() and t.shape[0] == 2 and t.numel() == 2 * n
        d.X, d.W, d.out_h = A0.data_ptr(), self.w.data_ptr(), out_h.data_ptr()
        d.bias = self.bias.data_ptr() if self.bias is not None else None
        if stream is None:
            stream = torch.cuda.current_stream().cuda_stream
        _lib.check(_lib.lib().advh_conv_taps2d_split(C.byref(d), self.Cn, n, self.w.stride(0), n, stream), "advh_conv_taps2d_split")


class ResblockDesc(C.Structure):
    _fields_ = [("X", C.c_void_p), ("W1", C.c_void_p), ("b1", C.c_void_p), ("W2", C.c_void_p), ("b2", C.c_void_p),
                ("out_h", C.c_void_p), ("M", C.c_int), ("Wg", C.c_int), ("w0", C.c_int), ("w1", C.c_int), ("k", C.c_int),
                ("dil", C.c_int), ("slope", C.c_float)]


def resblock_pair_lds_bytes(Cn: int, k: int, dil: int) -> int:
    rows = max(256 + (k - 1) * dil, 272)
    buf = ((rows * (Cn // 8) + 63) // 64 * 64) * 16
    one = 2 * k * Cn * Cn * 2 + buf
    return one if (one <= 80 * 1024 or one + buf > TAPS_MAX_LDS) else one + buf


def resblock_pair_supported(src: Map1D, dst: Map1D, w1: torch.Tensor, w2: torch.Tensor, dilation: int) -> bool:
    Cn, k = w1.shape[0], w1.shape[2]
    return (Cn in (32, 64) and tuple(w1.shape) == (Cn, Cn, k) and tuple(w2.shape) == (Cn, Cn, k) and k % 2 == 1 and src.C == Cn
            and dst.C == Cn and (src.B, src.T, src.halo) == (dst.B, dst.T, dst.halo) and src.halo >= (k - 1) * dilation // 2
            and resblock_pair_lds_bytes(Cn, k, dilation) <= TAPS_MAX_LDS)


class ResblockPairPlan:

    def __init__(self, src: Map1D, dst: Map1D, w1, b1, w2, b2, *, dilation: int, slope: float, device=None):
        assert resblock_pair_supported(src, dst, w1, w2, dilation)
        Cn, k = w1.shape[0], w1.shape[2]
        self.Cn = Cn
        pack = lambda w: w.permute(2, 0, 1).to(torch.float16).contiguous()
        self.w1, self.w2 = pack(w1), pack(w2)
        self.b1, self.b2 = b1.to(torch.float32).contiguous(), b2.to(torch.float32).contiguous()
        if device is not None:
            self.w1, self.w2, self.b1, self.b2 = (t.to(device) for t in (self.w1, self.w2, self.b1, self.b2))
        d = ResblockDesc()
        d.M, d.Wg, d.w0, d.w1, d.k, d.dil, d.slope = dst.B * dst.P, dst.P, dst.halo, dst.halo + dst.T, k, dilation, slope
        self.desc = d
        self.flops = 2 * 2.0 * dst.B * dst.T * Cn * Cn * k

    def run(self, A0: torch.Tensor, A1=None, *, out_h: torch.Tensor, stream: Optional[int] = None, **_):
        d = self.desc
        for t in (A0, out_h):
            assert t.dtype == torch.float16 and t.is_cuda and t.is_contiguous() and t.numel() == d.M * self.Cn
        assert A0.data_ptr() != out_h.data_ptr()
        d.X, d.out_h = A0.data_ptr(), out_h.data_ptr()
        d.W1, d.W2, d.b1, d.b2 = self.w1.data_ptr(), self.w2.data_ptr(), self.b1.data_ptr(), self.b2.data_ptr()
        if stream is None:
            stream = torch.cuda.current_stream().cuda_stream
        _lib.check(_lib.lib().advh_resblock_pair_f16(C.byref(d), self.Cn, stream), "advh_resblock_pair_f16")


class ResblockX3Desc(C.Structure):
    _fields_ = [("X", C.c_void_p), ("W1", C.c_void_p), ("b1", C.c_void_p), ("W2", C.c_void_p), ("b2", C.c_void_p),
                ("out_h", C.c_void_p), ("M", C.c_int), ("Wg", C.c_int), ("w0", C.c_int), ("w1", C.c_int), ("k", C.c_int),
                ("dil", C.c_int), ("slope", C.c_float), ("x_lo", C.c_int64), ("o_lo", C.c_int64), ("w_lo", C.c_int64)]


def resblock_pair_x3_lds_bytes(Cn: int, k: int, dil: int) -> int:
    if Cn != 32 or k < 1 or k % 2 == 0 or k > 15 or dil < 1:
        return -1
    rows = max(256 + (k - 1) * dil, 272)
    buf = 2 * ((rows * 4 + 63) // 64 * 64) * 16
    one = 4 * k * 32 * 32 * 2 + buf
    lds = one if (one <= 80 * 1024 or one + buf > TAPS_MAX_LDS) else one + buf
    return lds if lds <= TAPS_MAX_LDS else -1


def resblock_pair_x3_supported(src: Map1D, dst: Map1D, w1: torch.Tensor, w2: torch.Tensor, dilation: int) -> bool:
    Cn, k = w1.shape[0], w1.shape[2]
    return (src.split and dst.split and Cn == 32 and tuple(w1.shape) == (Cn, Cn, k) and tuple(w2.shape) == (Cn, Cn, k) and k % 2 == 1
            and src.C == Cn and dst.C == Cn and (src.B, src.T, src.halo) == (dst.B, dst.T, dst.halo)
            and src.halo >= (k - 1) * dilation // 2 and resblock_pair_x3_lds_bytes(Cn, k, dilation) > 0)


class ResblockPairX3Plan:

    def __init__(self, src: Map1D, dst: Map1D, w1, b1, w2, b2, *, dilation: int, slope: float, device=None):
        assert resblock_pair_x3_supported(src, dst, w1, w2, dilation)
        Cn, k = w1.shape[0], w1.shape[2]
        self.Cn = Cn
        pack = lambda w: split_planes(w.permute(2, 0, 1)).contiguous()
        self.w1, self.w2 = pack(w1), pack(w2)
        self.b1, self.b2 = b1.to(torch.float32).contiguous(), b2.to(torch.float32).contiguous()
        if device is not None:
            self.w1, self.w2, self.b1, self.b2 = (t.to(device) for t in (self.w1, self.w2, self.b1, self.b2))
        d = ResblockX3Desc()
        d.M, d.Wg, d.w0, d.w1, d.k, d.dil, d.slope = dst.B * dst.P, dst.P, dst.halo, dst.halo + dst.T, k, dilation, slope
        d.w_lo = k * Cn * Cn
        self.desc = d
        self.flops = 2 * 2.0 * dst.B * dst.T * Cn * Cn * k
        self.tile = None

    def run(self, A0: torch.Tensor, A1=None, *, out_h: torch.Tensor, stream: Optional[int] = None, **_):
        d = self.desc
        for t in (A0, out_h):
            assert t.dtype == torch.float16 and t.is_cuda and t.shape[0] == 2 and t[0].is_contiguous() and t[0].numel() == d.M * self.Cn
        assert A0.data_ptr() != out_h.data_ptr()
        d.X, d.out_h, d.x_lo, d.o_lo = A0.data_ptr(), out_h.data_ptr(), A0.stride(0), out_h.stride(0)
        d.W1, d.W2, d.b1, d.b2 = self.w1.data_ptr(), self.w2.data_ptr(), self.b1.data_ptr(), self.b2.data_ptr()
        if stream is None:
            stream = torch.cuda.current_stream().cuda_stream
        _lib.check(_lib.lib().advh_resblock_pair_x3(C.byref(d), self.Cn, stream), "advh_resblock_pair_x3")


def taps_split_tile(Cn: int, ntap: int, span: int) -> int:
    if Cn != 64 or not 0 < ntap <= 16:
        return 0
    return 256 if 4 * 2 * 64 * 64 * 2 + 2 * (((256 + span) * 8 + 63) // 64 * 64) * 16 <= 160 * 1024 else 0


def taps_split_supported(src: Map1D, dst: Map1D, weight: torch.Tensor, dilation: int, min_k: int = 7) -> bool:
    Cout, Cin, k = weight.shape
    return (src.split and dst.split and Cout == Cin == 64 and src.C == 64 and dst.C == 64 and src.halo == dst.halo and min_k <= k <= 16
            and taps_split_tile(64, k, (k - 1) * dilation) > 0)


def taps_supported(src: Map1D, dst: Map1D, weight: torch.Tensor, dilation: int) -> bool:
    Cout, Cin, k = weight.shape
    return (Cout == Cin and Cin in (32, 64) and src.C == Cin and dst.C == Cout and src.halo == dst.halo and k <= 16
            and taps_tile(Cin, k, (k - 1) * dilation) > 0)


def plan_conv1d_taps(src: Map1D, dst: Map1D, weight: torch.Tensor, bias: Optional[torch.Tensor], *, dilation: int = 1,
                     act: str = "none", slope: float = 0.0, slope2: float = 0.0, device=None,
                     pre_slope: Optional[float] = None) -> TapsPlan:
    Cout, Cin, k = weight.shape
    pad = (k - 1) * dilation // 2
    split = bool(src.split)
    assert (taps_split_supported(src, dst, weight, dilation, min_k=1) if split else taps_supported(src, dst, weight, dilation))
    assert src.halo >= pad and (src.B, src.T) == (dst.B, dst.T)
    toff = [j * dilation - pad for j in range(k)]
    return TapsPlan(M=dst.B * dst.P, Cn=Cin, w_taps=weight.permute(2, 0, 1).float(), toff=toff, Hg=1, Wg=dst.P,
                    window=(0, 1, dst.halo, dst.halo + dst.T), bias=bias, act=act, slope=slope, slope2=slope2,
                    device=device, pre_slope=pre_slope, split=split)


def replay_taps_on_cpu(plan: TapsPlan, X: torch.Tensor, resid: Optional[torch.Tensor] = None) -> torch.Tensor:
    d, Cn = plan.desc, plan.Cn
    x = X.reshape(-1, Cn).float().numpy()
    W = plan.w.float().cpu().numpy()
    out = np.zeros((d.M, Cn), dtype=np.float32)
    rows = np.arange(d.M)
    w_, h_ = rows % d.Wg, (rows // d.Wg) % d.Hg
    ok = (h_ >= d.h0) & (h_ < d.h1) & (w_ >= d.w0) & (w_ < d.w1)
    if d.pre_act:
        x = np.where(x > 0, x, np.float32(np.float16(d.pre_slope)) * x).astype(np.float16).astype(np.float32)
    for t in range(d.ntap):
        src = np.clip(rows + d.toff[t], 0, d.M - 1)
        out += x[src] @ W[t].T
    if plan.bias is not None:
        out += plan.bias.cpu().numpy()[None]
    if d.act == 2:
        out = np.where(out > 0, out, d.slope * out)
    if resid is not None:
        out += resid.reshape(-1, Cn).float().numpy()
    out[~ok] = 0.0
    return torch.from_numpy(out)


def plan_convT1d(src: Map1D, dst: Map1D, weight: torch.Tensor, bias: torch.Tensor, *, stride: int,
                 slope2: float = 0.0, device=None) -> GemmPlan:
    Cin, Cout, k = weight.shape
    r = stride
    pad = (k - r) // 2
    assert k == 2 * r and src.C == Cin and Cin % 8 == 0 and Cout % 4 == 0 and src.halo >= 1
    assert dst.T == src.T * r and dst.C == Cout and dst.halo >= pad and dst.B == src.B
    cc = Cin // 8
    wk = weight.permute(2, 1, 0)
    w2 = torch.cat([wk[r:2 * r], wk[0:r]], dim=2).reshape(1, r * Cout, 2 * Cin).float()
    return GemmPlan(M=src.B * (src.T + 1), N=r * Cout, w2=w2, ktab=np.arange(2 * cc, dtype=np.int64),
                    sources=[Source(src.P * cc, 0, cc, (src.halo - 1) * cc)], Hg=1, Wg=src.T + 1,
                    window=(0, 1, 0, src.T + 1), halo_zero=False,
                    out=(dst.P * dst.C, 0, r * dst.C, (dst.halo - pad) * dst.C), n_div=Cout, o_sNhi=dst.C,
                    bias=bias.float().repeat(r), slope2=slope2, phase=(r, pad, dst.T), device=device, split=dst.split)
```

xai-audio-deepfakes_amd/addvisor_hip/unet.py:

```python
from __future__ import annotations

import os
from typing import Dict, Optional, Tuple

import torch

from . import _lib, gemm as G

SLOPE = 0.2
BN_EPS = 1e-5


def _fold_bn(sd, conv: str, bn: str, dtype=torch.float32) -> Tuple[torch.Tensor, torch.Tensor]:
    w, b = sd[conv + ".weight"].to(dtype), sd[conv + ".bias"].to(dtype)
    s = sd[bn + ".weight"].to(dtype) / torch.sqrt(sd[bn + ".running_var"].to(dtype) + BN_EPS)
    return w * s.view(-1, 1, 1, 1), (b - sd[bn + ".running_mean"].to(dtype)) * s + sd[bn + ".bias"].to(dtype)


def reference_flops(B: int, H: int, W: int) -> float:
    def conv(h, w, cin, cout, taps):
        return 2.0 * B * h * w * cin * cout * taps
    f = conv(H // 2, W, 1, 32, 15) + conv(H // 2, W, 32, 32, 9)
    f += conv(H // 4, W, 32, 64, 15) + conv(H // 4, W, 64, 64, 9)
    f += conv(H // 8, W // 2, 64, 128, 9) + conv(H // 8, W // 2, 128, 128, 9)
    f += conv(H // 16, W // 4, 128, 256, 9) + conv(H // 16, W // 4, 256, 256, 9)
    f += conv(H // 16, W // 4, 256, 512, 9) + conv(H // 16, W // 4, 512, 512, 9)
    f += conv(H // 16, W // 4, 512, 256, 4) + conv(H // 8, W // 2, 384, 256, 9) + conv(H // 8, W // 2, 256, 256, 9)
    f += conv(H // 8, W // 2, 256, 128, 4) + conv(H // 4, W, 192, 128, 9) + conv(H // 4, W, 128, 128, 9)
    f += conv(H // 4, W, 128, 64, 2) + conv(H // 2, W, 96, 64, 9) + conv(H // 2, W, 64, 64, 9)
    f += conv(H // 2, W, 64, 32, 2) + conv(H, W, 33, 32, 9) + conv(H, W, 32, 32, 9)
    return f + conv(H, W, 32, 1, 1)


class HipUNet:

    def __init__(self, sd: Dict[str, torch.Tensor], device, line_tile: Optional[bool] = None, fuse_up: Optional[bool] = None,
                 precision: Optional[str] = None):
        _lib.init()
        from .embedder import default_precision
        self.precision = precision or default_precision()
        if self.precision not in ("f16", "f32"):
            raise ValueError("precision must be 'f16' or 'f32'")
        self.split = self.precision == "f32"
        self.wdtype = torch.float64 if self.split else torch.float32
        if line_tile is None:
            line_tile = os.environ.get("ADDVISOR_UNET_LINE_TILE", "1") != "0"
        if fuse_up is None:
            fuse_up = os.environ.get("ADDVISOR_UNET_FUSE_UP", "1") != "0"
        self.dev, self.line_tile, self.fuse_up = device, line_tile, fuse_up
        self.sd = {k.replace("module.", ""): v.detach() for k, v in sd.items()}
        w, b = _fold_bn(self.sd, "e1.block.0", "e1.block.1", self.wdtype)
        self.stem_w = w.reshape(32, 15).float().contiguous().to(device)
        self.stem_b = b.float().contiguous().to(device)
        self.head_w = self.sd["mask_head.0.weight"].float().reshape(32).contiguous().to(device)
        self.head_b = float(self.sd["mask_head.0.bias"].float().reshape(-1)[0])
        self._ws: Dict[Tuple[int, int, int], dict] = {}

    def _line_tile_plan(self, srcs, dst, m, w, b, kw):
        if not self.line_tile:
            return None
        fs = [m[s] for s in srcs]
        if self.split:
            if G.taps2d_split_supported(fs, m[dst], w, **kw):
                return G.Taps2dSplitPlan(fs[0], m[dst], w, b, slope=SLOPE, device=self.dev)
        elif G.taps2d_supported(fs, m[dst], w, **kw):
            return G.Taps2dPlan(fs[0], m[dst], w, b, slope=SLOPE, device=self.dev)
        return None

    def _workspace(self, B: int, H: int, W: int) -> dict:
        key = (B, H, W)
        if key in self._ws:
            return self._ws[key]
        if H % 16 or W % 4:
            raise ValueError("U-Net input needs H % 16 == 0 and W % 4 == 0 (SURVEY.md D2)")
        dev, sd = self.dev, self.sd
        F = lambda h, w, c, ph, pw: G.FMap(B, h, w, c, ph, pw, split=self.split).alloc(dev)
        if self.fuse_up:
            return self._workspace_fused(B, H, W)
        m = dict(
            x1a=F(H // 2, W, 32, 2, 1), x1=F(H // 2, W, 32, 2, 1),
            x2a=F(H // 4, W, 64, 1, 1), x2=F(H // 4, W, 64, 1, 1),
            x3a=F(H // 8, W // 2, 128, 1, 1), x3=F(H // 8, W // 2, 128, 1, 1),
            x4a=F(H // 16, W // 4, 256, 1, 1), x4=F(H // 16, W // 4, 256, 2, 2),
            b1=F(H // 16, W // 4, 512, 4, 4), b2=F(H // 16, W // 4, 512, 0, 0),
            u4=F(H // 8, W // 2, 256, 1, 1), y4a=F(H // 8, W // 2, 256, 1, 1), y4=F(H // 8, W // 2, 256, 0, 0),
            u3=F(H // 4, W, 128, 1, 1), y3a=F(H // 4, W, 128, 1, 1), y3=F(H // 4, W, 128, 0, 0),
            u2=F(H // 2, W, 64, 1, 1), y2a=F(H // 2, W, 64, 1, 1), y2=F(H // 2, W, 64, 1, 1),
            u1=F(H, W, 40, 1, 1), y1a=F(H, W, 32, 1, 1), y1=F(H, W, 32, 1, 1),
        )
        steps = []

        def conv(srcs, dst, conv_name, bn_name, **kw):
            w, b = _fold_bn(sd, conv_name, bn_name, self.wdtype)
            cin = sum(m[s].C for s in srcs)
            if cin != w.shape[1]:
                w = torch.cat([w, w.new_zeros(w.shape[0], cin - w.shape[1], *w.shape[2:])], 1)
            plan = self._line_tile_plan(srcs, dst, m, w, b, kw)
            if plan is None:
                plan = G.plan_conv2d([m[s] for s in srcs], m[dst], w, b, slope=SLOPE, device=dev, **kw)
            steps.append((plan, srcs, dst))

        def block(srcs, mid, dst, name, **first):
            conv(srcs, mid, f"{name}.block.0", f"{name}.block.1", **first)
            conv([mid], dst, f"{name}.block.3", f"{name}.block.4")

        def up(src, dst, name, stride):
            plan = G.plan_convT2d(m[src], m[dst], sd[name + ".weight"].to(self.wdtype), sd[name + ".bias"].float(),
                                  stride=stride, device=dev)
            steps.append((plan, [src], dst))

        conv(["x1a"], "x1", "e1.block.3", "e1.block.4")
        block(["x1"], "x2a", "x2", "e2", stride=(2, 1), padding=(2, 1))
        block(["x2"], "x3a", "x3", "e3", stride=(2, 2))
        block(["x3"], "x4a", "x4", "e4", stride=(2, 2))
        conv(["x4"], "b1", "bottleneck.0", "bottleneck.1", padding=(2, 2), dilation=(2, 2))
        conv(["b1"], "b2", "bottleneck.3", "bottleneck.4", padding=(4, 4), dilation=(4, 4))
        up("b2", "u4", "up4", (2, 2))
        block(["u4", "x3"], "y4a", "y4", "d4")
        up("y4", "u3", "up3", (2, 2))
        block(["u3", "x2"], "y3a", "y3", "d3")
        up("y3", "u2", "up2", (2, 1))
        block(["u2", "x1"], "y2a", "y2", "d2")
        up("y2", "u1", "up1", (2, 1))
        block(["u1"], "y1a", "y1", "d1")
        ws = dict(maps=m, steps=steps, mask=torch.empty(B, H, W, dtype=torch.float32, device=dev),
                  logits=torch.empty(B, H, W, dtype=torch.float32, device=dev))
        ws["flops"] = reference_flops(B, H, W)
        self._ws[key] = ws
        return ws

    def _workspace_fused(self, B: int, H: int, W: int) -> dict:
        dev, sd = self.dev, self.sd
        F = lambda h, w, c, ph, pw: G.FMap(B, h, w, c, ph, pw, split=self.split).alloc(dev)
        m = dict(
            x1a=F(H // 2, W, 32, 2, 1), x1=F(H // 2, W, 32, 2, 1),
            x2a=F(H // 4, W, 64, 1, 1), x2=F(H // 4, W, 64, 1, 1),
            x3a=F(H // 8, W // 2, 128, 1, 1), x3=F(H // 8, W // 2, 128, 1, 1),
            x4a=F(H // 16, W // 4, 256, 1, 1), x4=F(H // 16, W // 4, 256, 2, 2),
            b1=F(H // 16, W // 4, 512, 4, 4), b2=G.add_indicator(F(H // 16, W // 4, 576, 1, 1), 512),
            y4a=F(H // 8, W // 2, 256, 1, 1), y4=G.add_indicator(F(H // 8, W // 2, 320, 1, 1), 256),
            y3a=F(H // 4, W, 128, 1, 1), y3=G.add_indicator(F(H // 4, W, 192, 1, 1), 128),
            y2a=F(H // 2, W, 64, 1, 1), y2=F(H // 2, W, 64, 1, 1),
            xin=G.add_indicator(F(H, W, 8, 1, 1), 1), y1a=F(H, W, 32, 1, 1), y1=F(H, W, 32, 1, 1),
        )
        steps = []

        def conv(srcs, dst, conv_name, bn_name, **kw):
            w, b = _fold_bn(sd, conv_name, bn_name, self.wdtype)
            plan = self._line_tile_plan(srcs, dst, m, w, b, kw)
            if plan is None and self.line_tile and not self.split and G.conv_s21_supported([m[s] for s in srcs], m[dst], w, **kw):
                plan = G.ConvS21TilePlan(m[srcs[0]], m[dst], w, b, slope=SLOPE, device=dev)
            if plan is None:
                plan = G.plan_conv2d([m[s] for s in srcs], m[dst], w, b, slope=SLOPE, device=dev, **kw)
            steps.append((plan, srcs, dst))

        def block(srcs, mid, dst, name, **first):
            conv(srcs, mid, f"{name}.block.0", f"{name}.block.1", **first)
            conv([mid], dst, f"{name}.block.3", f"{name}.block.4")

        def up_block(coarse, skip, mid, dst, up_name, name, stride, coarse_C, skip_C, indicator):
            wc, bc = _fold_bn(sd, f"{name}.block.0", f"{name}.block.1", self.wdtype)
            wt, bt = sd[up_name + ".weight"].to(self.wdtype), sd[up_name + ".bias"].to(self.wdtype)
            if self.line_tile and not self.split and G.upconv_tile_supported(m[coarse], m[skip], m[mid], wt, wc, stride, indicator):
                plan = G.UpconvTilePlan(m[coarse], m[skip], m[mid], wt, bt, wc, bc, slope=SLOPE, device=dev)
            else:
                plan = G.plan_upconv2d(m[coarse], m[skip], m[mid], wt, bt, wc, bc, stride=stride, coarse_C=coarse_C,
                                       skip_C=skip_C, indicator=indicator, slope=SLOPE, device=dev)
            steps.append((plan, [coarse, skip], mid))
            conv([mid], dst, f"{name}.block.3", f"{name}.block.4")

        conv(["x1a"], "x1", "e1.block.3", "e1.block.4")
        block(["x1"], "x2a", "x2", "e2", stride=(2, 1), padding=(2, 1))
        block(["x2"], "x3a", "x3", "e3", stride=(2, 2))
        block(["x3"], "x4a", "x4", "e4", stride=(2, 2))
        conv(["x4"], "b1", "bottleneck.0", "bottleneck.1", padding=(2, 2), dilation=(2, 2))
        conv(["b1"], "b2", "bottleneck.3", "bottleneck.4", padding=(4, 4), dilation=(4, 4))
        up_block("b2", "x3", "y4a", "y4", "up4", "d4", (2, 2), 512, 128, ("coarse", 512))
        up_block("y4", "x2", "y3a", "y3", "up3", "d3", (2, 2), 256, 64, ("coarse", 256))
        up_block("y3", "x1", "y2a", "y2", "up2", "d2", (2, 1), 128, 32, ("coarse", 128))
        up_block("y2", "xin", "y1a", "y1", "up1", "d1", (2, 1), 64, 1, ("skip", 1))
        ws = dict(maps=m, steps=steps, mask=torch.empty(B, H, W, dtype=torch.float32, device=dev),
                  logits=torch.empty(B, H, W, dtype=torch.float32, device=dev))
        ws["flops"] = reference_flops(B, H, W)
        self._ws[(B, H, W)] = ws
        return ws

    def flops(self, B: int, H: int, W: int) -> float:
        return self._workspace(B, H, W)["flops"]

    def forward(self, mag: torch.Tensor, H: int = 512, W: Optional[int] = None, want_logits: bool = False):
        if mag.dim() != 3 or mag.dtype != torch.float32 or not mag.is_cuda:
            raise ValueError("mag must be a CUDA fp32 tensor [B, F, T]")
        mag = mag.contiguous()
        B, Fq, Tq = mag.shape
        W = (Tq // 4) * 4 if W is None else W
        if H > Fq or W > Tq:
            raise ValueError("crop exceeds the spectrogram")
        ws = self._workspace(B, H, W)
        m, lib = ws["maps"], _lib.lib()
        st = torch.cuda.current_stream().cuda_stream
        x1a = m["x1a"]
        xcat, xc0 = (m["xin"], 0) if self.fuse_up else (m["u1"], 32)
        if self.split:
            _lib.check(lib.advh_unet_stem_split(mag.data_ptr(), Fq, Tq, B, H, W, self.stem_w.data_ptr(), self.stem_b.data_ptr(),
                                                x1a.t.data_ptr(), x1a.t.stride(0), x1a.PH, x1a.PW, SLOPE, st), "advh_unet_stem_split")
            _lib.check(lib.advh_unet_pack_x_split(mag.data_ptr(), Fq, Tq, B, H, W, xcat.t.data_ptr(), xcat.t.stride(0), xcat.C, xc0,
                                                  xcat.PH, xcat.PW, st), "advh_unet_pack_x_split")
        else:
            _lib.check(lib.advh_unet_stem(mag.data_ptr(), Fq, Tq, B, H, W, self.stem_w.data_ptr(), self.stem_b.data_ptr(),
                                          x1a.t.data_ptr(), x1a.PH, x1a.PW, SLOPE, st), "advh_unet_stem")
            _lib.check(lib.advh_unet_pack_x(mag.data_ptr(), Fq, Tq, B, H, W, xcat.t.data_ptr(), xcat.C, xc0, xcat.PH, xcat.PW, st),
                       "advh_unet_pack_x")
        for plan, srcs, dst in ws["steps"]:
            a0 = m[srcs[0]].t
            a1 = m[srcs[1]].t if len(srcs) > 1 else None
            plan.run(a0, a1, out_h=m[dst].t)
        y1 = m["y1"]
        if self.split:
            _lib.check(lib.advh_unet_head_split(y1.t.data_ptr(), y1.t.stride(0), B, H, W, y1.PH, y1.PW, self.head_w.data_ptr(),
                                                self.head_b, ws["mask"].data_ptr(), ws["logits"].data_ptr(), st), "advh_unet_head_split")
        else:
            _lib.check(lib.advh_unet_head(y1.t.data_ptr(), B, H, W, y1.PH, y1.PW, self.head_w.data_ptr(), self.head_b,
                                          ws["mask"].data_ptr(), ws["logits"].data_ptr(), st), "advh_unet_head")
        mask = ws["mask"].clone()
        return (mask, ws["logits"].clone()) if want_logits else mask
```

xai-audio-deepfakes_amd/csrc/common.h:

```cpp
#pragma once
#include <hip/hip_runtime.h>
#include "addvisor_hip.h"

int advh_init_rest();
int advh_init_attention();
int advh_split_flag_attention(int* flag);
int advh_split_flag_attention_bwd_f32(int* flag);
int advh_split_flag_attention_bwd_x3(int* flag);
int advh_split_flag_backward(int* flag);
int advh_split_flag_conv_taps(int* flag);
int advh_split_flag_frontend(int* flag);
int advh_split_flag_frontend_bwd(int* flag);
int advh_split_flag_gemm(int* flag);
int advh_split_flag_hifigan(int* flag);
int advh_split_flag_rowops(int* flag);
int advh_split_flag_unet_misc(int* flag);
int advh_split_flag_unet_train(int* flag);
int advh_split_flag_resblock_pair_x3(int* flag);
int advh_split_flag_conv_taps2d_x3(int* flag);

int advh_attention_bwd_x3_launch(const void* qkv, long qkv_lo, const void* dctx, long dctx_lo, void* dqkv, long dqkv_lo, int B, int T, int H,
                                 int heads, hipStream_t s);
extern int g_att_bwd_force_f32;

#include <mutex>
#include <set>
#include <utility>
inline int advh_ensure_lds(const void* fn, int bytes = 160 * 1024) {
    static std::mutex mu;
    static std::set<std::pair<const void*, int>> done;
    int dev = 0;
    if (hipGetDevice(&dev) != hipSuccess) return ADVH_ELAUNCH;
    std::lock_guard<std::mutex> lk(mu);
    if (done.count({fn, dev})) return ADVH_OK;
    if (hipFuncSetAttribute(fn, hipFuncAttributeMaxDynamicSharedMemorySize, bytes) != hipSuccess) return ADVH_ELAUNCH;
    done.insert({fn, dev});
    return ADVH_OK;
}

#define ADVH_LAUNCH_CHECK() (hipGetLastError() == hipSuccess ? ADVH_OK : ADVH_ELAUNCH)
```

xai-audio-deepfakes_amd/csrc/conv_taps2d_x3.hip:

```cpp
#include <hip/hip_runtime.h>
#include <hip/hip_fp16.h>
#include "addvisor_hip.h"
#include "common.h"
#include "device_math.h"

namespace advh {

typedef _Float16 f16x8 __attribute__((ext_vector_type(8)));
typedef float f32x4 __attribute__((ext_vector_type(4)));

#define GLOBAL_PTR(p) ((const __attribute__((address_space(1))) void*)(p))
#define LDS_PTR(p) ((__attribute__((address_space(3))) void*)(p))

template <int C> __device__ __forceinline__ int swz2(int r) { return C == 64 ? (r & 7) : ((r >> 1) & 2); }
__device__ __forceinline__ int cout_of2(int R) { return ((R >> 5) << 5) + (((R >> 2) & 3) << 3) + (((R >> 4) & 1) << 2) + (R & 3); }

template <int C> struct Taps2dX3Cfg;
template <> struct Taps2dX3Cfg<32> { static constexpr int NJ = 4, NW = 4, NSLOT = 9; static constexpr bool RES = true; };
template <> struct Taps2dX3Cfg<64> { static constexpr int NJ = 2, NW = 8, NSLOT = 4; static constexpr bool RES = false; };

constexpr int T2_PR = 18, T2_SR = T2_PR * T2_PR;

template <int C> constexpr int taps2d_x3_src() { return (T2_SR * (C / 8) + 63) & ~63; }
template <int C> constexpr int taps2d_x3_lds() { return Taps2dX3Cfg<C>::NSLOT * 2 * C * C * 2 + 2 * taps2d_x3_src<C>() * 16; }

template <int C>
__global__ __launch_bounds__(64 * Taps2dX3Cfg<C>::NW, 2 * 4 / Taps2dX3Cfg<C>::NW)
void conv_taps2d_x3_kernel(const advh_taps2d_desc p, long x_lo, long w_lo, long o_lo) {
    constexpr int NJ = Taps2dX3Cfg<C>::NJ, NW = Taps2dX3Cfg<C>::NW, NSLOT = Taps2dX3Cfg<C>::NSLOT;
    constexpr bool RES = Taps2dX3Cfg<C>::RES;
    static_assert(NJ * NW == 16, "one 16 x 16 output tile per workgroup");
    constexpr int CH = C / 8, CT = C / 16, KS = C / 32, NTH = 64 * NW, WTAP = C * C * 2, SRC = taps2d_x3_src<C>();
    constexpr int AHEAD = NSLOT - 1, WPT = RES ? 0 : 2 * (C * CH / NTH);
    static_assert(RES || C * CH == NTH, "a streamed tap is one 16-byte chunk per thread and plane");
    extern __shared__ __attribute__((aligned(16))) char lds[];
    const int tid = threadIdx.x, lane = tid & 63, wv = tid >> 6;
    const int fr = lane & 15, g = lane >> 4;
    char* Wl = lds;
    char* Xl = lds + NSLOT * 2 * WTAP;
    const _Float16* Wg = (const _Float16*)p.W;
    const _Float16* X = (const _Float16*)p.X;
    const int Hp = p.H + 2 * p.PH, Wp = p.W_ + 2 * p.PW;
    const int tx = (p.W_ + 15) / 16, ty = (p.H + 15) / 16, ntiles = p.B * ty * tx;
    auto origin = [&](int tile, int& b, int& y0, int& x0) {
        x0 = (tile % tx) * 16;
        const int r = tile / tx;
        y0 = (r % ty) * 16;
        b = r / ty;
    };
    auto load_weights = [&](int t, int slot) {
        char* dst = Wl + (size_t)slot * 2 * WTAP;
        for (int i = tid; i < C * CH; i += NTH) {
            const int row = i / CH, pos = i % CH;
            const _Float16* src = Wg + ((long)t * C + cout_of2(row)) * C + ((pos ^ swz2<C>(row)) * 8);
            __builtin_amdgcn_global_load_lds(GLOBAL_PTR(src), LDS_PTR(dst + (size_t)(i - lane) * 16), 16, 0, 0);
            __builtin_amdgcn_global_load_lds(GLOBAL_PTR(src + w_lo), LDS_PTR(dst + WTAP + (size_t)(i - lane) * 16), 16, 0, 0);
        }
    };
    auto load_patch = [&](int tile) {
        int b, y0, x0;
        origin(tile, b, y0, x0);
        for (int i = tid; i < SRC; i += NTH) {
            int row = i / CH;
            const int pos = i % CH;
            if (row >= T2_SR) row = 0;
            const int gy = min(y0 + p.PH - 1 + row / T2_PR, Hp - 1), gx = min(x0 + p.PW - 1 + row % T2_PR, Wp - 1);
            const _Float16* src = X + (((long)b * Hp + gy) * Wp + gx) * C + ((pos ^ swz2<C>(i / CH)) * 8);
            __builtin_amdgcn_global_load_lds(GLOBAL_PTR(src), LDS_PTR(Xl + (size_t)(i - lane) * 16), 16, 0, 0);
            __builtin_amdgcn_global_load_lds(GLOBAL_PTR(src + x_lo), LDS_PTR(Xl + (size_t)SRC * 16 + (size_t)(i - lane) * 16), 16, 0, 0);
        }
    };
    float4 bias[CT];
#pragma unroll
    for (int i = 0; i < CT; ++i)
        bias[i] = p.bias ? *(const float4*)(p.bias + (i >> 1) * 32 + g * 8 + (i & 1) * 4) : make_float4(0.f, 0.f, 0.f, 0.f);

    const int mytiles = (int)blockIdx.x < ntiles ? (ntiles - 1 - (int)blockIdx.x) / (int)gridDim.x + 1 : 0;
    const int ntot = mytiles * 9;
    if (RES) {
        if (mytiles)
            for (int t = 0; t < 9; ++t) load_weights(t, t);
    } else {
        for (int n = 0; n < AHEAD && n < ntot; ++n) load_weights(n % 9, n % NSLOT);
    }
    if (mytiles) load_patch(blockIdx.x);
    int n = 0;
    for (int tile = blockIdx.x; tile < ntiles; tile += gridDim.x) {
        f32x4 acc[CT][NJ], accx[CT][NJ];
#pragma unroll
        for (int i = 0; i < CT; ++i)
#pragma unroll
            for (int j = 0; j < NJ; ++j) { acc[i][j] = f32x4{0.f, 0.f, 0.f, 0.f}; accx[i][j] = f32x4{0.f, 0.f, 0.f, 0.f}; }
        f16x8 fwh[2][CT], fwl[2][CT], fxh[2][NJ], fxl[2][NJ];
        auto fetch = [&](int set, int slot, int t, int ks) {
            const char* wb = Wl + (size_t)slot * 2 * WTAP;
            const int c = ks * 4 + g, kh = t / 3, kw = t - kh * 3;
#pragma unroll
            for (int i = 0; i < CT; ++i) {
                const int wo = ((i * 16 + fr) * CH + (c ^ swz2<C>(fr))) * 16;
                fwh[set][i] = *(const f16x8*)(wb + wo);
                fwl[set][i] = *(const f16x8*)(wb + WTAP + wo);
            }
#pragma unroll
            for (int j = 0; j < NJ; ++j) {
                const int row = (wv * NJ + j + kh) * T2_PR + kw + fr;
                const int xo = (row * CH + (c ^ swz2<C>(row))) * 16;
                fxh[set][j] = *(const f16x8*)(Xl + xo);
                fxl[set][j] = *(const f16x8*)(Xl + (size_t)SRC * 16 + xo);
            }
        };
        auto mma = [&](int set) {
#pragma unroll
            for (int j = 0; j < NJ; ++j) {
#pragma unroll
                for (int i = 0; i < CT; ++i) accx[i][j] = __builtin_amdgcn_mfma_f32_16x16x32_f16(fwh[set][i], fxl[set][j], accx[i][j], 0, 0, 0);
#pragma unroll
                for (int i = 0; i < CT; ++i) acc[i][j] = __builtin_amdgcn_mfma_f32_16x16x32_f16(fwh[set][i], fxh[set][j], acc[i][j], 0, 0, 0);
#pragma unroll
                for (int i = 0; i < CT; ++i) accx[i][j] = __builtin_amdgcn_mfma_f32_16x16x32_f16(fwl[set][i], fxh[set][j], accx[i][j], 0, 0, 0);
            }
        };
        auto slot_of = [&](int t) { return RES ? t : (n + t) % NSLOT; };
#pragma unroll
        for (int t = 0; t < 9; ++t) {
            if (t == 0 || !RES) {
                if (t == 0 || n + t + 2 >= ntot) asm volatile("s_waitcnt vmcnt(0)" ::: "memory");
                else asm volatile("s_waitcnt vmcnt(%0)" ::"n"(WPT) : "memory");
                __syncthreads();
                if (!RES && n + t + AHEAD < ntot) load_weights((n + t + AHEAD) % 9, (n + t + AHEAD) % NSLOT);
            }
            if (t == 0) fetch(0, slot_of(0), 0, 0);
#pragma unroll
            for (int ks = 0; ks < KS; ++ks) {
                const int s = t * KS + ks, cur = s & 1;
                if (ks + 1 < KS) fetch(cur ^ 1, slot_of(t), t, ks + 1);
                else if (t + 1 < 9) fetch(cur ^ 1, slot_of(t + 1), t + 1, 0);
                __builtin_amdgcn_sched_barrier(0);
                mma(cur);
                __builtin_amdgcn_sched_barrier(0);
            }
        }
        n += 9;
        if (tile + (int)gridDim.x < ntiles) {
            __syncthreads();
            load_patch(tile + gridDim.x);
        }
        int b, y0, x0;
        origin(tile, b, y0, x0);
#pragma unroll
        for (int j = 0; j < NJ; ++j) {
            const int gy = y0 + wv * NJ + j, gx = x0 + fr;
            if (gy >= p.H || gx >= p.W_) continue;
            const long pos = ((long)b * Hp + gy + p.PH) * Wp + gx + p.PW;
#pragma unroll
            for (int q = 0; q < CT / 2; ++q) {
                const long o = pos * C + q * 32 + g * 8;
                float v[8];
#pragma unroll
                for (int r = 0; r < 4; ++r) {
                    v[r] = fmaf(accx[2 * q][j][r], SPLIT_LO_INV, acc[2 * q][j][r]);
                    v[4 + r] = fmaf(accx[2 * q + 1][j][r], SPLIT_LO_INV, acc[2 * q + 1][j][r]);
                }
                v[0] += bias[2 * q].x; v[1] += bias[2 * q].y; v[2] += bias[2 * q].z; v[3] += bias[2 * q].w;
                v[4] += bias[2 * q + 1].x; v[5] += bias[2 * q + 1].y; v[6] += bias[2 * q + 1].z; v[7] += bias[2 * q + 1].w;
                if (p.act == ADVH_ACT_LEAKY) {
#pragma unroll
                    for (int r = 0; r < 8; ++r) v[r] = v[r] > 0.f ? v[r] : p.slope * v[r];
                }
                store_h_rt<8>((_Float16*)p.out_h, o, o_lo, v);
            }
        }
    }
    asm volatile("s_waitcnt vmcnt(0)" ::: "memory");
}

}

using namespace advh;

extern "C" int advh_conv_taps2d_split_lds_bytes(int C) {
    return C == 32 ? taps2d_x3_lds<32>() : (C == 64 ? taps2d_x3_lds<64>() : -1);
}

extern "C" int advh_conv_taps2d_split(const advh_taps2d_desc* d, int C, int64_t x_lo, int64_t w_lo, int64_t o_lo, advh_stream_t stream) {
    if (!d || !d->X || !d->W || !d->out_h || d->B <= 0 || d->H <= 0 || d->W_ <= 0 || d->PH < 1 || d->PW < 1) return ADVH_EINVAL;
    if (C != 32 && C != 64) return ADVH_EUNSUPPORTED;
    if (d->act != ADVH_ACT_NONE && d->act != ADVH_ACT_LEAKY) return ADVH_EINVAL;
    if (d->X == d->out_h) return ADVH_EINVAL;
    const long plane = (long)d->B * (d->H + 2 * d->PH) * (d->W_ + 2 * d->PW) * C;
    if (x_lo < plane || o_lo < plane || w_lo < 9L * C * C || x_lo % 8 || w_lo % 8 || o_lo % 8) return ADVH_EINVAL;
    const long ntiles = (long)d->B * ((d->H + 15) / 16) * ((d->W_ + 15) / 16);
    if (ntiles > 0x7fffffffL) return ADVH_EINVAL;
    const int lds = advh_conv_taps2d_split_lds_bytes(C);
    const void* fn = C == 64 ? (const void*)conv_taps2d_x3_kernel<64> : (const void*)conv_taps2d_x3_kernel<32>;
    if (advh_ensure_lds(fn) != ADVH_OK) return ADVH_ELAUNCH;
    const long per_cu = 160 * 1024 / lds;
    const long grid = ntiles < 256 * per_cu ? ntiles : 256 * per_cu;
    if (C == 64) hipLaunchKernelGGL(conv_taps2d_x3_kernel<64>, dim3((unsigned)grid), dim3(512), lds, (hipStream_t)stream, *d, (long)x_lo, (long)w_lo, (long)o_lo);
    else hipLaunchKernelGGL(conv_taps2d_x3_kernel<32>, dim3((unsigned)grid), dim3(256), lds, (hipStream_t)stream, *d, (long)x_lo, (long)w_lo, (long)o_lo);
    return ADVH_LAUNCH_CHECK();
}

ADVH_SPLIT_FLAG_SETTER(advh_split_flag_conv_taps2d_x3)
```

xai-audio-deepfakes_amd/csrc/stft.hip:

```cpp
#include <hip/hip_runtime.h>
#include <mutex>
#include <string.h>
#include "addvisor_hip.h"
#include "common.h"
#include "fft512.h"

namespace advh {

__device__ cf g_twiddle[1024];
#ifdef ADVH_STAMPS
__device__ long long g_stamps[16];
#define STAMP(i) do { if (blockIdx.x == 3 && blockIdx.y == 5 && threadIdx.x == 0) g_stamps[i] = __builtin_amdgcn_s_memtime(); } while (0)
#else
#define STAMP(i) do { } while (0)
#endif
static bool g_init_done[64] = {false};
static bool init_done_here() { int dev = 0; return hipGetDevice(&dev) == hipSuccess && dev >= 0 && dev < 64 && g_init_done[dev]; }

constexpr int NFFT = 1024;
constexpr int NBIN = 513;
static int g_stft_fb = 8;
constexpr int THREADS = 512;

__device__ __forceinline__ void wave_fence() {
    __builtin_amdgcn_fence(__ATOMIC_ACQ_REL, "wavefront");
    __builtin_amdgcn_wave_barrier();
}

struct LaneTw { cf p8[7], p64[7], glue[4]; };
__device__ __forceinline__ void load_lane_twiddles(int lane, LaneTw& t) {
    fft512_lane_twiddles<8>(g_twiddle, lane, t.p8);
    fft512_lane_twiddles<64>(g_twiddle, lane, t.p64);
#pragma unroll
    for (int q = 0; q < 4; ++q) t.glue[q] = g_twiddle[lane + 1 + 64 * q];
}

template <int DIR, bool FROM_REGS, bool TO_REGS>
__device__ __forceinline__ void fft512_wave(float* re, float* im, int lane, const LaneTw& t, cf (&v)[8]) {
    if (FROM_REGS) dft8<DIR>(v);
    else { fft512_pass_load_tw<DIR, 1>(re, im, lane, t.p8, v); wave_fence(); }
    fft512_pass_store<1>(re, im, lane, v);
    wave_fence();
    fft512_pass_load_tw<DIR, 8>(re, im, lane, t.p8, v);
    wave_fence();
    fft512_pass_store<8>(re, im, lane, v);
    wave_fence();
    fft512_pass_load_tw<DIR, 64>(re, im, lane, t.p64, v);
    if (!TO_REGS) {
        wave_fence();
        fft512_pass_store<64>(re, im, lane, v);
        wave_fence();
    }
}

template <int FB> struct RowPitch { static constexpr int value = FFT_ROW + ((32 / FB - FFT_ROW % 32) + 32) % 32; };
static_assert(RowPitch<8>::value % 32 == 4 && RowPitch<16>::value % 32 == 2, "row pitch");

template <int FB>
__device__ __forceinline__ void carve(float* smem, float*& re, float*& im, float*& scratch) {
    re = smem;
    im = smem + FB * RowPitch<FB>::value;
    scratch = smem + 2 * FB * RowPitch<FB>::value;
}

__device__ __forceinline__ float fast_log1p(float x) {
    const float u = 1.f + x, d = u - 1.f;
    return d == 0.f ? x : __logf(u) * (x * __builtin_amdgcn_rcpf(d));
}
__device__ __forceinline__ float fast_expm1(float y) {
    const float u = __expf(y), d = u - 1.f;
    if (d == 0.f) return y;
    return d * (y * __builtin_amdgcn_rcpf(__logf(u)));
}
__device__ __forceinline__ float mask_factor(float m, float M, int mode) {
    if (mode == ADVH_MASK_LINEAR) return m;
    if (M < 1e-12f) return m;
    return (__builtin_amdgcn_exp2f(m * __builtin_amdgcn_logf(1.f + M)) - 1.f) * __builtin_amdgcn_rcpf(M);
}

struct AdjArgs { const float* mask; float* dmask; int Fm, Tm, mode, which; };

template <int FB, int ADJ>
__global__ __launch_bounds__(THREADS, 6) void stft_fwd_kernel(
    const float* __restrict__ wave, long wave_stride, int n_in, int L, int hop, int win,
    const float* __restrict__ window, float* __restrict__ X, float* __restrict__ mag,
    float* __restrict__ phase, int T, AdjArgs adj) {
    extern __shared__ __attribute__((aligned(16))) float smem[];
    constexpr int ROWP = RowPitch<FB>::value;
    float *re, *im, *smp;
    carve<FB>(smem, re, im, smp);
    const int tid = threadIdx.x, lane = tid & 63, wv = tid >> 6;
    const int b = blockIdx.y, tA = blockIdx.x * FB;
    const int left = (NFFT - win) / 2;
    const int span = (FB - 1) * hop + win;

    STAMP(0);
    const float* w = wave + (long)b * wave_stride;
    if (ADJ)
    for (int i = tid; i < span; i += THREADS) {
        int src = tA * hop + left + i - NFFT / 2;
        float v = 0.f;
        if (ADJ) {
            if (src >= 0 && src < L && src < n_in) {
                const int pp = tA * hop + left + i;
                const int R = (win + hop - 1) / hop, thi = (pp - left) / hop;
                float env = 0.f;
                for (int r = 0; r < R; ++r) {
                    int t = thi - r, j = pp - left - t * hop;
                    if (t >= 0 && t < T && j >= 0 && j < win) { float ww = window ? window[j] : 1.f; env += ww * ww; }
                }
                v = env > 1e-11f ? w[src] / env : 0.f;
            }
        } else {
            if (src < 0) src = -src;
            if (src >= L) src = 2 * (L - 1) - src;
            if (src >= 0 && src < n_in && src < L) v = w[src];
        }
        smp[i] = v;
    }
    if (ADJ) __syncthreads();
    STAMP(1);

    LaneTw ltw;
    load_lane_twiddles(lane, ltw);
    for (int f = wv; f < FB; f += THREADS / 64) {
        if (tA + f >= T) break;
        float* rr = re + f * ROWP;
        float* ii = im + f * ROWP;
        const float* fs = smp + f * hop;
        cf zv[8];
        if (ADJ) {
#pragma unroll
            for (int q = 0; q < 8; ++q) {
                const int n = lane + 64 * q;
                const int j0 = 2 * n - left, j1 = j0 + 1;
                float a = 0.f, c = 0.f;
                if (j0 >= 0 && j0 < win) a = window ? fs[j0] * window[j0] : fs[j0];
                if (j1 >= 0 && j1 < win) c = window ? fs[j1] * window[j1] : fs[j1];
                zv[q] = cf{a, c};
            }
        } else {
            const int s0 = (tA + f) * hop + left - NFFT / 2;
            const int nmax = min(n_in, L);
            float xa[8], xc[8], wa[8], wc[8];
            const bool interior = s0 >= 0 && s0 + win <= nmax && !window && !(left & 1) && !(s0 & 1) && !(wave_stride & 1);
            if (interior) {
#pragma unroll
                for (int q = 0; q < 8; ++q) {
                    const int j0 = 2 * (lane + 64 * q) - left;
                    const bool ok = j0 >= 0 && j0 < win;
                    const float2 v = ok ? *reinterpret_cast<const float2*>(w + s0 + j0) : make_float2(0.f, 0.f);
                    zv[q] = cf{v.x, v.y};
                }
            } else {
#pragma unroll
            for (int q = 0; q < 8; ++q) {
                const int n = lane + 64 * q;
                const int j0 = 2 * n - left, j1 = j0 + 1;
                int a0 = s0 + j0, a1 = s0 + j1;
                if (a0 < 0) a0 = -a0;
                if (a0 >= L) a0 = 2 * (L - 1) - a0;
                if (a1 < 0) a1 = -a1;
                if (a1 >= L) a1 = 2 * (L - 1) - a1;
                const bool ok0 = j0 >= 0 && j0 < win && a0 >= 0 && a0 < nmax, ok1 = j1 >= 0 && j1 < win && a1 >= 0 && a1 < nmax;
                xa[q] = ok0 ? w[a0] : 0.f;
                xc[q] = ok1 ? w[a1] : 0.f;
                wa[q] = (window && ok0) ? window[j0] : 1.f;
                wc[q] = (window && ok1) ? window[j1] : 1.f;
            }
#pragma unroll
            for (int q = 0; q < 8; ++q) zv[q] = cf{xa[q] * wa[q], xc[q] * wc[q]};
            }
        }
        fft512_wave<-1, true, false>(rr, ii, lane, ltw, zv);
        cf A[4], Bv[4];
#pragma unroll
        for (int q = 0; q < 4; ++q) {
            int k = lane + 1 + 64 * q;
            A[q] = cf{rr[fidx(k)], ii[fidx(k)]};
            Bv[q] = cf{rr[fidx(512 - k)], ii[fidx(512 - k)]};
        }
        cf Z0 = cf{rr[0], ii[0]};
        wave_fence();
#pragma unroll
        for (int q = 0; q < 4; ++q) {
            int k = lane + 1 + 64 * q;
            cf xk, xm;
            rfft_post_pair(A[q], Bv[q], ltw.glue[q], xk, xm);
            rr[fidx(k)] = xk.x; ii[fidx(k)] = xk.y;
            rr[fidx(512 - k)] = xm.x; ii[fidx(512 - k)] = xm.y;
        }
        if (lane == 0) {
            rr[0] = Z0.x + Z0.y; ii[0] = 0.f;
            rr[fidx(512)] = Z0.x - Z0.y; ii[fidx(512)] = 0.f;
        }
    }
    __syncthreads();
    STAMP(2);

    const int nvalid = min(FB, T - tA);
    for (int idx = tid; idx < NBIN * FB; idx += THREADS) {
        int tl = idx & (FB - 1), k = idx / FB;
        if (tl >= nvalid) continue;
        float xr = re[tl * ROWP + fidx(k)], xi = im[tl * ROWP + fidx(k)];
        long o = ((long)b * NBIN + k) * T + tA + tl;
        if (ADJ) {
            const int t = tA + tl;
            if (k >= adj.Fm || t >= adj.Tm) continue;
            const bool edge = k == 0 || k == NFFT / 2;
            const float sc = (edge ? 1.f : 2.f) / NFFT;
            float sn, cs;
            sincosf(phase[o], &sn, &cs);
            const float da = sc * (xr * cs + (edge ? 0.f : xi * sn));
            const long om = ((long)b * adj.Fm + k) * adj.Tm + t;
            const float M = mag[o];
            float dm;
            if (adj.mode == ADVH_MASK_LINEAR) {
                dm = adj.which ? -M * da : M * da;
            } else {
                float m = adj.mask[om];
                if (adj.which) m = 1.f - m;
                const float lg = log1pf(M);
                dm = lg * expf(m * lg) * da;
                if (adj.which) dm = -dm;
            }
            adj.dmask[om] = dm;
            continue;
        }
        if (X) reinterpret_cast<float2*>(X)[o] = make_float2(xr, xi);
        if (mag) mag[o] = __builtin_sqrtf(fmaf(xr, xr, xi * xi));
        if (phase) phase[o] = atan2f(xi, xr);
    }
    STAMP(3);
}

template <int SRC, int FB>
__global__ __launch_bounds__(THREADS, 4) void istft_kernel(
    const float* __restrict__ mag, const float* __restrict__ phase, const float* __restrict__ mask,
    int Fm, int Tm, int mode, int which0, float* __restrict__ out0, float* __restrict__ out1,
    long wave_stride, int T, int L, int hop, int win, int R, const float* __restrict__ window, long zstride) {
    extern __shared__ __attribute__((aligned(16))) float smem[];
    constexpr int ROWP = RowPitch<FB>::value;
    float *re, *im, *unused_scratch;
    carve<FB>(smem, re, im, unused_scratch);
    (void)unused_scratch;
    const int tid = threadIdx.x, lane = tid & 63, wv = tid >> 6;
    const int b = blockIdx.y, g = blockIdx.x;
    const int left = (NFFT - win) / 2;
    const int S = FB - R + 1;
    const int tA = g * S - (R - 1);
    const int pass = blockIdx.z;
    constexpr int NIT = (NBIN * FB + THREADS - 1) / THREADS;
    float2 ld0[NIT];
    float ldm[NIT];
    bool valid[NIT];
#pragma unroll
    for (int it = 0; it < NIT; ++it) {
        const int idx = tid + it * THREADS;
        const int tl = idx & (FB - 1), k = idx / FB, t = tA + tl;
        valid[it] = idx < NBIN * FB && t >= 0 && t < T;
        ld0[it] = make_float2(0.f, 0.f);
        ldm[it] = 0.f;
        if (valid[it]) {
            const long o = ((long)b * NBIN + k) * T + t;
            if (SRC == 0) ld0[it] = make_float2(mag[o], phase[o]);
            else if (SRC == 2) {
                const int lo = Fm + (int)blockIdx.z * Tm;
                ld0[it] = reinterpret_cast<const float2*>((k >= lo && k < lo + Tm) ? phase : mag)[o];
            } else ld0[it] = reinterpret_cast<const float2*>(mag)[o];
            if ((SRC == 0 || SRC == 3) && mode != ADVH_MASK_NONE && k < Fm && t < Tm) ldm[it] = mask[((long)b * Fm + k) * Tm + t];
        }
    }
    const int which = which0 + (SRC == 2 ? 0 : pass);
    float* out = (SRC == 2 ? out0 + (long)blockIdx.z * zstride : (pass == 0 ? out0 : out1)) + (long)b * wave_stride;
    if (pass == 0) STAMP(4);

#pragma unroll
    for (int it = 0; it < NIT; ++it) {
        const int idx = tid + it * THREADS;
        if (idx >= NBIN * FB) break;
        const int tl = idx & (FB - 1), k = idx / FB;
        float xr = ld0[it].x, xi = ld0[it].y;
        if (SRC == 3) {
            float m = ldm[it];
            if (which == 1) m = 1.f - m;
            const float f = valid[it] ? mask_factor(m, __builtin_sqrtf(fmaf(xr, xr, xi * xi)), mode) : 0.f;
            xr *= f; xi *= f;
        } else if (SRC == 0) {
            float a = ld0[it].x;
            const float ph = ld0[it].y;
            if (mode != ADVH_MASK_NONE) {
                float m = ldm[it];
                if (which == 1) m = 1.f - m;
                a = (mode == ADVH_MASK_LINEAR) ? m * a : fast_expm1(m * fast_log1p(a));
            }
            float sn, cs;
            sincosf(ph, &sn, &cs);
            xr = valid[it] ? a * cs : 0.f; xi = valid[it] ? a * sn : 0.f;
        }
        re[tl * ROWP + fidx(k)] = xr;
        im[tl * ROWP + fidx(k)] = xi;
    }
    __syncthreads();
    if (pass == 0) STAMP(5);
    LaneTw ltw;
    load_lane_twiddles(lane, ltw);

    static_assert(2 * RowPitch<FB>::value >= NFFT, "a frame's time samples must fit its two LDS rows");
    for (int f = wv; f < FB; f += THREADS / 64) {
        int t = tA + f;
        if (t < 0 || t >= T) continue;
        float* rr = re + f * ROWP;
        float* ii = im + f * ROWP;
        cf A[4], Bv[4];
#pragma unroll
        for (int q = 0; q < 4; ++q) {
            int k = lane + 1 + 64 * q;
            A[q] = cf{rr[fidx(k)], ii[fidx(k)]};
            Bv[q] = cf{rr[fidx(512 - k)], ii[fidx(512 - k)]};
        }
        float x0 = rr[0], xn = rr[fidx(512)];
        wave_fence();
#pragma unroll
        for (int q = 0; q < 4; ++q) {
            int k = lane + 1 + 64 * q;
            cf zk, zm;
            irfft_pre_pair(A[q], Bv[q], ltw.glue[q], zk, zm);
            rr[fidx(k)] = zk.x; ii[fidx(k)] = zk.y;
            rr[fidx(512 - k)] = zm.x; ii[fidx(512 - k)] = zm.y;
        }
        if (lane == 0) { rr[0] = 0.5f * (x0 + xn); ii[0] = 0.5f * (x0 - xn); }
        wave_fence();
        cf yv[8];
        fft512_wave<+1, false, true>(rr, ii, lane, ltw, yv);
        wave_fence();
#pragma unroll
        for (int q = 0; q < 8; ++q) {
            const int n = lane + 64 * q;
            const int j0 = 2 * n - left, j1 = j0 + 1;
            float a = yv[q].x * (1.f / 512.f), c = yv[q].y * (1.f / 512.f);
            if (!(left & 1)) {
                if (j0 < 0 || j0 >= win) continue;
                if (window) { a *= window[j0]; c *= window[j1]; }
                *reinterpret_cast<float2*>(j0 < ROWP ? rr + j0 : ii + (j0 - ROWP)) = make_float2(a, c);
            } else {
                if (j0 >= 0 && j0 < win) *(j0 < ROWP ? rr + j0 : ii + (j0 - ROWP)) = window ? a * window[j0] : a;
                if (j1 >= 0 && j1 < win) *(j1 < ROWP ? rr + j1 : ii + (j1 - ROWP)) = window ? c * window[j1] : c;
            }
        }
    }
    __syncthreads();
    if (pass == 0) STAMP(6);

    for (int sgm = 0; sgm < S; ++sgm) {
        const int thi = tA + R - 1 + sgm;
        const int n0 = thi * hop + left - NFFT / 2;
        for (int u = tid; u < hop; u += THREADS) {
            const int n = n0 + u;
            if (n < 0 || n >= L) continue;
            float env = 0.f, sum = 0.f;
            for (int r = 0; r < R; ++r) {
                const int t = thi - r, j = u + r * hop;
                if (t >= 0 && t < T && j < win) {
                    const float ww = window ? window[j] : 1.f;
                    env += ww * ww;
                    const int f = t - tA;
                    sum += j < ROWP ? re[f * ROWP + j] : im[f * ROWP + j - ROWP];
                }
            }
            out[n] = env > 1e-11f ? sum / env : 0.f;
        }
    }
    if (pass == 0) STAMP(7);
}

static size_t lds_rows_bytes(int FB) { return sizeof(float) * 2 * FB * (FB == 8 ? RowPitch<8>::value : RowPitch<16>::value); }
static size_t lds_bytes(int FB, int hop, int win) {
    const int pitch = FB == 8 ? RowPitch<8>::value : RowPitch<16>::value;
    return sizeof(float) * (2 * FB * pitch + (FB - 1) * hop + win);
}

}

using namespace advh;

extern "C" const char* advh_version(void) { return "addvisor_hip 0.1 (gfx950, wave64)"; }

#ifdef ADVH_STAMPS
extern "C" int advh_debug_stamps(long long* out) { return hipMemcpyFromSymbol(out, HIP_SYMBOL(g_stamps), sizeof(long long) * 16) == hipSuccess ? ADVH_OK : ADVH_ELAUNCH; }
#endif

static int* g_split_flag_host = nullptr;

extern "C" int advh_set_option(const char* name, int value) {
    if (!name) return ADVH_EINVAL;
    if (!strcmp(name, "stft_frames_per_workgroup")) {
        if (value != 8 && value != 16) return ADVH_EINVAL;
        g_stft_fb = value;
        return ADVH_OK;
    }
    if (!strcmp(name, "attention_bwd_mfma_f32")) {
        g_att_bwd_force_f32 = value != 0;
        return ADVH_OK;
    }
    return ADVH_EINVAL;
}

extern "C" int advh_init(void) {
    static std::mutex mu;
    std::lock_guard<std::mutex> lk(mu);
    int dev = 0;
    if (hipGetDevice(&dev) != hipSuccess || dev < 0 || dev >= 64) return ADVH_ELAUNCH;
    if (g_init_done[dev]) return ADVH_OK;
    cf host[1024];
    for (int k = 0; k < 1024; ++k) {
        host[k].x = (float)cos(2.0 * M_PI * k / 1024.0);
        host[k].y = (float)sin(2.0 * M_PI * k / 1024.0);
    }
    if (hipMemcpyToSymbol(HIP_SYMBOL(g_twiddle), host, sizeof(host)) != hipSuccess) return ADVH_ELAUNCH;
    const int maxlds = 160 * 1024;
    const void* big[] = {(const void*)stft_fwd_kernel<16, 0>, (const void*)stft_fwd_kernel<8, 0>, (const void*)stft_fwd_kernel<16, 1>,
                         (const void*)stft_fwd_kernel<8, 1>, (const void*)istft_kernel<0, 16>,
                         (const void*)istft_kernel<2, 16>, (const void*)istft_kernel<2, 8>,
                         (const void*)istft_kernel<1, 16>, (const void*)istft_kernel<0, 8>, (const void*)istft_kernel<1, 8>,
                         (const void*)istft_kernel<3, 16>, (const void*)istft_kernel<3, 8>};
    for (const void* f : big)
        if (hipFuncSetAttribute(f, hipFuncAttributeMaxDynamicSharedMemorySize, maxlds) != hipSuccess) return ADVH_ELAUNCH;
    int rc = advh_init_rest();
    if (rc != ADVH_OK) return rc;
    rc = advh_init_attention();
    if (rc != ADVH_OK) return rc;
    if (!g_split_flag_host) {
        if (hipHostMalloc((void**)&g_split_flag_host, sizeof(int), hipHostMallocMapped) != hipSuccess) return ADVH_ELAUNCH;
        *g_split_flag_host = 0;
    }
    int* dflag = nullptr;
    if (hipHostGetDevicePointer((void**)&dflag, g_split_flag_host, 0) != hipSuccess) return ADVH_ELAUNCH;
    int (*const setters[])(int*) = {advh_split_flag_attention, advh_split_flag_attention_bwd_f32, advh_split_flag_attention_bwd_x3, advh_split_flag_backward, advh_split_flag_conv_taps, advh_split_flag_frontend, advh_split_flag_frontend_bwd, advh_split_flag_gemm, advh_split_flag_hifigan, advh_split_flag_rowops, advh_split_flag_unet_misc, advh_split_flag_unet_train, advh_split_flag_resblock_pair_x3,
                                   advh_split_flag_conv_taps2d_x3};
    for (auto set : setters)
        if ((rc = set(dflag)) != ADVH_OK) return rc;
    g_init_done[dev] = true;
    return ADVH_OK;
}

extern "C" int advh_split_overflow(int reset) {
    if (!g_split_flag_host) return 0;
    const int v = *(volatile int*)g_split_flag_host;
    if (reset) *(volatile int*)g_split_flag_host = 0;
    return v != 0;
}

static int check_frame_args(int B, int T, int L, int hop, int win) {
    if (!init_done_here()) return ADVH_ENOTINIT;
    if (B <= 0 || L <= 0 || hop <= 0 || win <= 0 || win > NFFT || (win & 1) || T != 1 + L / hop) return ADVH_EINVAL;
    if (L <= NFFT / 2) return ADVH_EINVAL;
    if (lds_bytes(g_stft_fb, hop, win) > 160 * 1024) return ADVH_EUNSUPPORTED;
    return ADVH_OK;
}

extern "C" int advh_stft_forward(const float* wave, int64_t wave_stride, int n_in, int B, int L, int hop, int win,
                                 const float* window, float* X, float* mag, float* phase, int T,
                                 advh_stream_t stream) {
    int rc = check_frame_args(B, T, L, hop, win);
    if (rc) return rc;
    if (!wave || n_in <= 0 || wave_stride < (n_in < L ? n_in : L)) return ADVH_EINVAL;
    const int FB = g_stft_fb;
    dim3 grid((T + FB - 1) / FB, B);
    const AdjArgs none = {nullptr, nullptr, 0, 0, 0, 0};
    if (FB == 8)
        hipLaunchKernelGGL((stft_fwd_kernel<8, 0>), grid, dim3(THREADS), lds_rows_bytes(8), (hipStream_t)stream, wave,
                           (long)wave_stride, n_in, L, hop, win, window, X, mag, phase, T, none);
    else
        hipLaunchKernelGGL((stft_fwd_kernel<16, 0>), grid, dim3(THREADS), lds_rows_bytes(16), (hipStream_t)stream, wave,
                           (long)wave_stride, n_in, L, hop, win, window, X, mag, phase, T, none);
    return hipGetLastError() == hipSuccess ? ADVH_OK : ADVH_ELAUNCH;
}

extern "C" int advh_istft_masked_bwd(const float* g_wave, int64_t g_stride, const float* mag, const float* phase,
                                     const float* mask, int Fm, int Tm, int mode, int which, float* dmask, int B, int T,
                                     int L, int hop, int win, const float* window, advh_stream_t stream) {
    int rc = check_frame_args(B, T, L, hop, win);
    if (rc) return rc;
    if (!g_wave || !mag || !phase || !dmask || g_stride < L || Fm <= 0 || Tm <= 0 || Fm > NBIN || Tm > T) return ADVH_EINVAL;
    if (mode != ADVH_MASK_LINEAR && mode != ADVH_MASK_LOG1P) return ADVH_EINVAL;
    if (mode == ADVH_MASK_LOG1P && !mask) return ADVH_EINVAL;
    if (which != 0 && which != 1) return ADVH_EINVAL;
    const int FB = g_stft_fb;
    dim3 grid((Tm + FB - 1) / FB, B);
    const AdjArgs adj = {mask, dmask, Fm, Tm, mode, which};
    float* magp = const_cast<float*>(mag);
    float* php = const_cast<float*>(phase);
    if (FB == 8)
        hipLaunchKernelGGL((stft_fwd_kernel<8, 1>), grid, dim3(THREADS), lds_bytes(8, hop, win), (hipStream_t)stream, g_wave,
                           (long)g_stride, L, L, hop, win, window, (float*)nullptr, magp, php, T, adj);
    else
        hipLaunchKernelGGL((stft_fwd_kernel<16, 1>), grid, dim3(THREADS), lds_bytes(16, hop, win), (hipStream_t)stream, g_wave,
                           (long)g_stride, L, L, hop, win, window, (float*)nullptr, magp, php, T, adj);
    return hipGetLastError() == hipSuccess ? ADVH_OK : ADVH_ELAUNCH;
}

static int launch_istft(int src, const float* a, const float* ph, const float* mask, int Fm, int Tm, int mode,
                        float* o0, float* o1, int64_t ws, int B, int T, int L, int hop, int win,
                        const float* window, advh_stream_t stream, int nbands = 0, int64_t zstride = 0) {
    int rc = check_frame_args(B, T, L, hop, win);
    if (rc) return rc;
    const int R = (win + hop - 1) / hop;
    const int FB = g_stft_fb;
    if (R > FB / 2) return ADVH_EUNSUPPORTED;
    const int S = FB - R + 1, left = (NFFT - win) / 2;
    int which0 = 0, nz = 2;
    float *p0 = o0, *p1 = o1;
    if (!o0 && !o1) return ADVH_EINVAL;
    if (!o0) { which0 = 1; p0 = o1; nz = 1; }
    else if (!o1) { nz = 1; }
    if (src == 1) p1 = nullptr;
    if (src == 2) nz = nbands;
    else if (nz == 1) p1 = nullptr;
    const int nG = (NFFT / 2 + L - left + S * hop - 1) / (S * hop);
    dim3 grid(nG, B, nz);
#define ISTFT_LAUNCH(SRC_, FB_)                                                                                          \
    hipLaunchKernelGGL((istft_kernel<SRC_, FB_>), grid, dim3(THREADS), lds_rows_bytes(FB_), (hipStream_t)stream, a, ph,  \
                       mask, Fm, Tm, mode, which0, p0, p1, (long)ws, T, L, hop, win, R, window, (long)zstride)
    if (src == 0) { if (FB == 8) ISTFT_LAUNCH(0, 8); else ISTFT_LAUNCH(0, 16); }
    else if (src == 1) { if (FB == 8) ISTFT_LAUNCH(1, 8); else ISTFT_LAUNCH(1, 16); }
    else if (src == 3) { if (FB == 8) ISTFT_LAUNCH(3, 8); else ISTFT_LAUNCH(3, 16); }
    else { if (FB == 8) ISTFT_LAUNCH(2, 8); else ISTFT_LAUNCH(2, 16); }
#undef ISTFT_LAUNCH
    return hipGetLastError() == hipSuccess ? ADVH_OK : ADVH_ELAUNCH;
}

extern "C" int advh_istft_masked(const float* mag, const float* phase, const float* mask, int Fm, int Tm, int mode,
                                 float* wave_in, float* wave_out, int64_t wave_stride, int B, int T, int L, int hop,
                                 int win, const float* window, advh_stream_t stream) {
    if (!mag || !phase || wave_stride < L) return ADVH_EINVAL;
    if (mode != ADVH_MASK_NONE && (!mask || Fm <= 0 || Tm <= 0 || Fm > NBIN || Tm > T)) return ADVH_EINVAL;
    if (mode < 0 || mode > ADVH_MASK_LOG1P) return ADVH_EINVAL;
    if (mode == ADVH_MASK_NONE && wave_out) return ADVH_EINVAL;
    return launch_istft(0, mag, phase, mask, Fm, Tm, mode, wave_in, wave_out, wave_stride, B, T, L, hop, win, window, stream);
}

extern "C" int advh_istft_masked_c64(const float* spec, const float* mask, int Fm, int Tm, int mode, float* wave_in, float* wave_out,
                                     int64_t wave_stride, int B, int T, int L, int hop, int win, const float* window,
                                     advh_stream_t stream) {
    if (!spec || !mask || wave_stride < L || Fm <= 0 || Tm <= 0 || Fm > NBIN || Tm > T) return ADVH_EINVAL;
    if (mode != ADVH_MASK_LINEAR && mode != ADVH_MASK_LOG1P) return ADVH_EINVAL;
    return launch_istft(3, spec, nullptr, mask, Fm, Tm, mode, wave_in, wave_out, wave_stride, B, T, L, hop, win, window, stream);
}

extern "C" int advh_istft_bandswap(const float* spec_a, const float* spec_b, int k0, int kw, int nbands, float* waves,
                                   int64_t wave_stride, int64_t band_stride, int B, int T, int L, int hop, int win,
                                   const float* window, advh_stream_t stream) {
    if (!spec_a || !spec_b || !waves || wave_stride < L || nbands <= 0 || nbands > 65535 || k0 < 0 || kw <= 0 ||
        k0 + (long)nbands * kw > NBIN || band_stride < (int64_t)B * wave_stride)
        return ADVH_EINVAL;
    return launch_istft(2, spec_a, spec_b, nullptr, k0, kw, ADVH_MASK_NONE, waves, nullptr, wave_stride, B, T, L, hop, win, window,
                        stream, nbands, band_stride);
}

extern "C" int advh_istft_c64(const float* spec, float* wave, int64_t wave_stride, int B, int T, int L, int hop, int win,
                              const float* window, advh_stream_t stream) {
    if (!spec || !wave || wave_stride < L) return ADVH_EINVAL;
    return launch_istft(1, spec, nullptr, nullptr, 0, 0, ADVH_MASK_NONE, wave, nullptr, wave_stride, B, T, L, hop, win, window, stream);
}
```

Measured before the change: 1367 explanations/s.

## Fuse U-Net mask head into last split conv and add split-precision upconv tile kernel

Adds a templated head variant of the split-precision 3x3 32-channel conv kernel. It computes the final 32-channel dot product plus bias to write the mask and logits directly, so the y1 feature map is never allocated or stored and the separate head kernel launch is dropped. Also adds a new tiled MFMA kernel for the (2,1) upconv+skip+3x3 block on split-plane f16 data. Previously that block fell back to the generic composed upconv GEMM path when split precision was on. The new kernels add code and shape-specific restrictions and need correct hi/lo plane handling in the fused epilogue.

```diff
diff --git a/include/addvisor_hip.h b/include/addvisor_hip.h
--- a/include/addvisor_hip.h
+++ b/include/addvisor_hip.h
@@ -322,6 +322,8 @@
 int advh_conv_taps2d_f16(const advh_taps2d_desc* d, int C, advh_stream_t stream);
 int advh_conv_taps2d_split_lds_bytes(int C);
 int advh_conv_taps2d_split(const advh_taps2d_desc* d, int C, int64_t x_lo, int64_t w_lo, int64_t o_lo, advh_stream_t stream);
+int advh_conv_taps2d_split_head(const advh_taps2d_desc* d, int C, int64_t x_lo, int64_t w_lo, const float* head_w, float head_b,
+                                float* mask, float* logits, advh_stream_t stream);
 typedef struct advh_upconv_desc {
     const void* Xc;
     const void* Xs;
@@ -334,6 +336,9 @@
 } advh_upconv_desc;
 int advh_upconv21_tile_f16(const advh_upconv_desc* d, advh_stream_t stream);
 int advh_upconv21_tile_lds_bytes(void);
+int advh_upconv21_tile_split_lds_bytes(void);
+int advh_upconv21_tile_split(const advh_upconv_desc* d, int Cc, int N, int64_t xc_lo, int64_t xs_lo, int64_t w_lo, int64_t o_lo,
+                             advh_stream_t stream);
 typedef struct advh_convs21_desc {
     const void* X;
     const void* W;
diff --git a/xai-audio-deepfakes_amd/addvisor_hip/_lib.py b/xai-audio-deepfakes_amd/addvisor_hip/_lib.py
--- a/xai-audio-deepfakes_amd/addvisor_hip/_lib.py
+++ b/xai-audio-deepfakes_amd/addvisor_hip/_lib.py
@@ -107,6 +107,7 @@
     "advh_conv_taps2d_f16": (_i, [_p, _i, _p]),
     "advh_conv_taps2d_split_lds_bytes": (_i, [_i]),
     "advh_conv_taps2d_split": (_i, [_p, _i, _i64, _i64, _i64, _p]),
+    "advh_conv_taps2d_split_head": (_i, [_p, _i, _i64, _i64, _p, _f, _p, _p, _p]),
     "advh_upconv21_tile_f16": (_i, [_p, _p]),
     "advh_posconv_tile_f16": (_i, [_p, _p]),
     "advh_conv53s21_tile_f16": (_i, [_p, _p]),
@@ -123,6 +124,8 @@
     "advh_hifigan_conv_post_split": (_i, [_p, _i64, _p, _f, _p, _i, _i, _i, _i, _i, _p]),
     "advh_unet_head_split": (_i, [_p, _i64, _i, _i, _i, _i, _i, _p, _f, _p, _p, _p]),
     "advh_upconv21_tile_lds_bytes": (_i, []),
+    "advh_upconv21_tile_split_lds_bytes": (_i, []),
+    "advh_upconv21_tile_split": (_i, [_p, _i, _i, _i64, _i64, _i64, _i64, _p]),
     "advh_bn_stats_split": (_i, [_p, _i64, _p, _p, _p, _p]),
     "advh_bn_apply_split": (_i, [_p, _i64, _p, _p, _f, _p, _i64, _p]),
     "advh_bn_bwd_sums_split": (_i, [_p, _i64, _p, _i64, _p, _p, _f, _p, _p, _p]),
diff --git a/xai-audio-deepfakes_amd/addvisor_hip/gemm.py b/xai-audio-deepfakes_amd/addvisor_hip/gemm.py
--- a/xai-audio-deepfakes_amd/addvisor_hip/gemm.py
+++ b/xai-audio-deepfakes_amd/addvisor_hip/gemm.py
@@ -633,6 +633,50 @@
         _lib.check(_lib.lib().advh_upconv21_tile_f16(C.byref(d), stream), "advh_upconv21_tile_f16")
 
 
+def upconv_tile_split_supported(coarse: FMap, skip: FMap, dst: FMap, wt: torch.Tensor, wc: torch.Tensor, stride, indicator) -> bool:
+    return (coarse.split and skip.split and dst.split
+            and tuple(stride) == (2, 1) and tuple(wt.shape) == (64, 32, 2, 1) and tuple(wc.shape) == (32, 33, 3, 3)
+            and coarse.C == 64 and skip.C == 8 and dst.C == 32 and tuple(indicator) == ("skip", 1)
+            and min(coarse.PH, coarse.PW, skip.PH, skip.PW) >= 1
+            and (dst.B, dst.H, dst.W) == (coarse.B, 2 * coarse.H, coarse.W) == (skip.B, skip.H, skip.W))
+
+
+class UpconvSplitTilePlan:
+
+    def __init__(self, coarse: FMap, skip: FMap, dst: FMap, wt: torch.Tensor, bt: torch.Tensor, wc: torch.Tensor,
+                 bc: torch.Tensor, *, slope: float = 0.2, device=None):
+        assert upconv_tile_split_supported(coarse, skip, dst, wt, wc, (2, 1), ("skip", 1))
+        w2, cu0, cu1 = compose_upconv_weights(wt, bt, wc, (2, 1), ("skip", 1))
+        assert (cu0, cu1) == (8, 1) and w2[0].shape == (32, 456)
+        R = np.arange(32)
+        ch = torch.from_numpy(8 * ((R >> 2) & 3) + 4 * ((R >> 4) & 1) + (R & 3))
+        full = torch.zeros(2, 32, 480, dtype=torch.float64)
+        for ph in range(2):
+            full[ph, :, :456] = w2[ph]
+        wp = split_planes(full[:, ch].reshape(2, 32, 15, 32).permute(0, 2, 1, 3)).contiguous()
+        self.w = wp.to(device) if device is not None else wp
+        self.bias = bc.to(torch.float32).contiguous()
+        self.bias = self.bias.to(device) if device is not None else self.bias
+        d = UpconvDesc()
+        d.B, d.Hc, d.W_ = coarse.B, coarse.H, coarse.W
+        d.PHc, d.PWc, d.PHs, d.PWs, d.PHo, d.PWo = coarse.PH, coarse.PW, skip.PH, skip.PW, dst.PH, dst.PW
+        d.act, d.slope = ACT["leaky"], slope
+        self.desc = d
+        self.numels = tuple(2 * f.B * f.Hp * f.Wp * f.C for f in (coarse, skip, dst))
+        self.flops = 2.0 * dst.B * dst.H * dst.W * 32 * (6 * 64 + 9 * 2)
+        self.tile = None
+
+    def run(self, A0: torch.Tensor, A1: torch.Tensor, *, out_h: torch.Tensor, stream: Optional[int] = None):
+        d = self.desc
+        for t, n in zip((A0, A1, out_h), self.numels):
+            assert t.dtype == torch.float16 and t.is_cuda and t.is_contiguous() and t.shape[0] == 2 and t.numel() == n
+        d.Xc, d.Xs, d.W, d.bias, d.out_h = A0.data_ptr(), A1.data_ptr(), self.w.data_ptr(), self.bias.data_ptr(), out_h.data_ptr()
+        if stream is None:
+            stream = torch.cuda.current_stream().cuda_stream
+        _lib.check(_lib.lib().advh_upconv21_tile_split(C.byref(d), 64, 32, A0.stride(0), A1.stride(0), self.w.stride(0), out_h.stride(0),
+                                                       stream), "advh_upconv21_tile_split")
+
+
 def replay_on_cpu(plan: GemmPlan, A0: torch.Tensor, A1: Optional[torch.Tensor], out_numel: int,
                   resid: Optional[torch.Tensor] = None, out_init: Optional[torch.Tensor] = None) -> torch.Tensor:
     d = plan.desc
@@ -869,16 +913,34 @@
         d.act, d.slope = ACT[act], slope
         self.desc = d
         self.flops = 2.0 * dst.B * dst.H * dst.W * Cn * Cn * 9
-
-    def run(self, A0: torch.Tensor, A1=None, *, out_h: torch.Tensor, stream: Optional[int] = None):
+        self.head = None
+
+    def attach_head(self, head_w: torch.Tensor, head_b: float, mask: torch.Tensor, logits: Optional[torch.Tensor] = None):
+        d = self.desc
+        assert self.Cn == 32 and head_w.dtype == torch.float32 and head_w.numel() == 32 and head_w.is_contiguous()
+        for t in (mask, logits):
+            assert t is None or (t.dtype == torch.float32 and t.is_contiguous() and tuple(t.shape) == (d.B, d.H, d.W_))
+        self.head = (head_w, float(head_b), mask, logits)
+        self.flops += 2.0 * d.B * d.H * d.W_ * 32
+        return self
+
+    def run(self, A0: torch.Tensor, A1=None, *, out_h: Optional[torch.Tensor] = None, stream: Optional[int] = None):
         d = self.desc
         n = d.B * (d.H + 2 * d.PH) * (d.W_ + 2 * d.PW) * self.Cn
-        for t in (A0, out_h):
+        for t in (A0,) if self.head else (A0, out_h):
             assert t.dtype == torch.float16 and t.is_cuda and t.is_contiguous() and t.shape[0] == 2 and t.numel() == 2 * n
-        d.X, d.W, d.out_h = A0.data_ptr(), self.w.data_ptr(), out_h.data_ptr()
+        d.X, d.W = A0.data_ptr(), self.w.data_ptr()
         d.bias = self.bias.data_ptr() if self.bias is not None else None
         if stream is None:
             stream = torch.cuda.current_stream().cuda_stream
+        if self.head:
+            hw, hb, mask, logits = self.head
+            d.out_h = None
+            _lib.check(_lib.lib().advh_conv_taps2d_split_head(C.byref(d), self.Cn, n, self.w.stride(0), hw.data_ptr(), hb, mask.data_ptr(),
+                                                              logits.data_ptr() if logits is not None else None, stream),
+                       "advh_conv_taps2d_split_head")
+            return
+        d.out_h = out_h.data_ptr()
         _lib.check(_lib.lib().advh_conv_taps2d_split(C.byref(d), self.Cn, n, self.w.stride(0), n, stream), "advh_conv_taps2d_split")
 
 
diff --git a/xai-audio-deepfakes_amd/addvisor_hip/unet.py b/xai-audio-deepfakes_amd/addvisor_hip/unet.py
--- a/xai-audio-deepfakes_amd/addvisor_hip/unet.py
+++ b/xai-audio-deepfakes_amd/addvisor_hip/unet.py
@@ -67,6 +67,26 @@
             return G.Taps2dPlan(fs[0], m[dst], w, b, slope=SLOPE, device=self.dev)
         return None
 
+    @property
+    def _fused_head(self) -> bool:
+        return self.split and self.line_tile
+
+    def _y1(self, B: int, H: int, W: int) -> G.FMap:
+        y1 = G.FMap(B, H, W, 32, 1, 1, split=self.split)
+        return y1 if self._fused_head else y1.alloc(self.dev)
+
+    def _finish(self, key, m, steps) -> dict:
+        B, H, W = key
+        ws = dict(maps=m, steps=steps, mask=torch.empty(B, H, W, dtype=torch.float32, device=self.dev),
+                  logits=torch.empty(B, H, W, dtype=torch.float32, device=self.dev))
+        ws["flops"] = reference_flops(B, H, W)
+        if self._fused_head:
+            last = steps[-1][0]
+            assert isinstance(last, G.Taps2dSplitPlan), "d1.block.3 is a 3x3 32-channel same-geometry layer"
+            last.attach_head(self.head_w, self.head_b, ws["mask"], ws["logits"])
+        self._ws[key] = ws
+        return ws
+
     def _workspace(self, B: int, H: int, W: int) -> dict:
         key = (B, H, W)
         if key in self._ws:
@@ -86,7 +106,7 @@
             u4=F(H // 8, W // 2, 256, 1, 1), y4a=F(H // 8, W // 2, 256, 1, 1), y4=F(H // 8, W // 2, 256, 0, 0),
             u3=F(H // 4, W, 128, 1, 1), y3a=F(H // 4, W, 128, 1, 1), y3=F(H // 4, W, 128, 0, 0),
             u2=F(H // 2, W, 64, 1, 1), y2a=F(H // 2, W, 64, 1, 1), y2=F(H // 2, W, 64, 1, 1),
-            u1=F(H, W, 40, 1, 1), y1a=F(H, W, 32, 1, 1), y1=F(H, W, 32, 1, 1),
+            u1=F(H, W, 40, 1, 1), y1a=F(H, W, 32, 1, 1), y1=self._y1(B, H, W),
         )
         steps = []
 
@@ -123,11 +143,7 @@
         block(["u2", "x1"], "y2a", "y2", "d2")
         up("y2", "u1", "up1", (2, 1))
         block(["u1"], "y1a", "y1", "d1")
-        ws = dict(maps=m, steps=steps, mask=torch.empty(B, H, W, dtype=torch.float32, device=dev),
-                  logits=torch.empty(B, H, W, dtype=torch.float32, device=dev))
-        ws["flops"] = reference_flops(B, H, W)
-        self._ws[key] = ws
-        return ws
+        return self._finish(key, m, steps)
 
     def _workspace_fused(self, B: int, H: int, W: int) -> dict:
         dev, sd = self.dev, self.sd
@@ -141,7 +157,7 @@
             y4a=F(H // 8, W // 2, 256, 1, 1), y4=G.add_indicator(F(H // 8, W // 2, 320, 1, 1), 256),
             y3a=F(H // 4, W, 128, 1, 1), y3=G.add_indicator(F(H // 4, W, 192, 1, 1), 128),
             y2a=F(H // 2, W, 64, 1, 1), y2=F(H // 2, W, 64, 1, 1),
-            xin=G.add_indicator(F(H, W, 8, 1, 1), 1), y1a=F(H, W, 32, 1, 1), y1=F(H, W, 32, 1, 1),
+            xin=G.add_indicator(F(H, W, 8, 1, 1), 1), y1a=F(H, W, 32, 1, 1), y1=self._y1(B, H, W),
         )
         steps = []
 
@@ -163,6 +179,8 @@
             wt, bt = sd[up_name + ".weight"].to(self.wdtype), sd[up_name + ".bias"].to(self.wdtype)
             if self.line_tile and not self.split and G.upconv_tile_supported(m[coarse], m[skip], m[mid], wt, wc, stride, indicator):
                 plan = G.UpconvTilePlan(m[coarse], m[skip], m[mid], wt, bt, wc, bc, slope=SLOPE, device=dev)
+            elif self.line_tile and G.upconv_tile_split_supported(m[coarse], m[skip], m[mid], wt, wc, stride, indicator):
+                plan = G.UpconvSplitTilePlan(m[coarse], m[skip], m[mid], wt, bt, wc, bc, slope=SLOPE, device=dev)
             else:
                 plan = G.plan_upconv2d(m[coarse], m[skip], m[mid], wt, bt, wc, bc, stride=stride, coarse_C=coarse_C,
                                        skip_C=skip_C, indicator=indicator, slope=SLOPE, device=dev)
@@ -179,11 +197,7 @@
         up_block("y4", "x2", "y3a", "y3", "up3", "d3", (2, 2), 256, 64, ("coarse", 256))
         up_block("y3", "x1", "y2a", "y2", "up2", "d2", (2, 1), 128, 32, ("coarse", 128))
         up_block("y2", "xin", "y1a", "y1", "up1", "d1", (2, 1), 64, 1, ("skip", 1))
-        ws = dict(maps=m, steps=steps, mask=torch.empty(B, H, W, dtype=torch.float32, device=dev),
-                  logits=torch.empty(B, H, W, dtype=torch.float32, device=dev))
-        ws["flops"] = reference_flops(B, H, W)
-        self._ws[(B, H, W)] = ws
-        return ws
+        return self._finish((B, H, W), m, steps)
 
     def flops(self, B: int, H: int, W: int) -> float:
         return self._workspace(B, H, W)["flops"]
@@ -216,7 +230,9 @@
             a1 = m[srcs[1]].t if len(srcs) > 1 else None
             plan.run(a0, a1, out_h=m[dst].t)
         y1 = m["y1"]
-        if self.split:
+        if self._fused_head:
+            pass
+        elif self.split:
             _lib.check(lib.advh_unet_head_split(y1.t.data_ptr(), y1.t.stride(0), B, H, W, y1.PH, y1.PW, self.head_w.data_ptr(),
                                                 self.head_b, ws["mask"].data_ptr(), ws["logits"].data_ptr(), st), "advh_unet_head_split")
         else:
diff --git a/xai-audio-deepfakes_amd/csrc/common.h b/xai-audio-deepfakes_amd/csrc/common.h
--- a/xai-audio-deepfakes_amd/csrc/common.h
+++ b/xai-audio-deepfakes_amd/csrc/common.h
@@ -18,6 +18,8 @@
 int advh_split_flag_unet_train(int* flag);
 int advh_split_flag_resblock_pair_x3(int* flag);
 int advh_split_flag_conv_taps2d_x3(int* flag);
+int advh_split_flag_conv_taps2d_head_x3(int* flag);
+int advh_split_flag_upconv_tile_x3(int* flag);
 
 int advh_attention_bwd_x3_launch(const void* qkv, long qkv_lo, const void* dctx, long dctx_lo, void* dqkv, long dqkv_lo, int B, int T, int H,
                                  int heads, hipStream_t s);
diff --git a/xai-audio-deepfakes_amd/csrc/conv_taps2d_head_x3.hip b/xai-audio-deepfakes_amd/csrc/conv_taps2d_head_x3.hip
--- /dev/null
+++ b/xai-audio-deepfakes_amd/csrc/conv_taps2d_head_x3.hip
@@ -0,0 +1,17 @@
+#include "conv_taps2d_x3.h"
+
+using namespace advh;
+
+extern "C" int advh_conv_taps2d_split_head(const advh_taps2d_desc* d, int C, int64_t x_lo, int64_t w_lo, const float* head_w, float head_b,
+                                           float* mask, float* logits, advh_stream_t stream) {
+    const taps2d_head hd = {head_w, head_b, mask, logits};
+    const int lds = taps2d_x3_lds<32>();
+    long grid = 0;
+    const int rc = advh_taps2d_split_check(d, C, x_lo, w_lo, 0, &hd, lds, &grid);
+    if (rc != ADVH_OK) return rc;
+    if (advh_ensure_lds((const void*)conv_taps2d_x3_kernel<32, true>) != ADVH_OK) return ADVH_ELAUNCH;
+    hipLaunchKernelGGL((conv_taps2d_x3_kernel<32, true>), dim3((unsigned)grid), dim3(256), lds, (hipStream_t)stream, *d, (long)x_lo, (long)w_lo, 0L, hd);
+    return ADVH_LAUNCH_CHECK();
+}
+
+ADVH_SPLIT_FLAG_SETTER(advh_split_flag_conv_taps2d_head_x3)
diff --git a/xai-audio-deepfakes_amd/csrc/conv_taps2d_x3.h b/xai-audio-deepfakes_amd/csrc/conv_taps2d_x3.h
--- /dev/null
+++ b/xai-audio-deepfakes_amd/csrc/conv_taps2d_x3.h
@@ -0,0 +1,221 @@
+#pragma once
+#include <hip/hip_runtime.h>
+#include <hip/hip_fp16.h>
+#include "addvisor_hip.h"
+#include "common.h"
+#include "device_math.h"
+
+namespace advh {
+
+typedef _Float16 f16x8 __attribute__((ext_vector_type(8)));
+typedef float f32x4 __attribute__((ext_vector_type(4)));
+
+#define GLOBAL_PTR(p) ((const __attribute__((address_space(1))) void*)(p))
+#define LDS_PTR(p) ((__attribute__((address_space(3))) void*)(p))
+
+template <int C> __device__ __forceinline__ int swz2(int r) { return C == 64 ? (r & 7) : ((r >> 1) & 2); }
+__device__ __forceinline__ int cout_of2(int R) { return ((R >> 5) << 5) + (((R >> 2) & 3) << 3) + (((R >> 4) & 1) << 2) + (R & 3); }
+
+template <int C> struct Taps2dX3Cfg;
+template <> struct Taps2dX3Cfg<32> { static constexpr int NJ = 4, NW = 4, NSLOT = 9; static constexpr bool RES = true; };
+template <> struct Taps2dX3Cfg<64> { static constexpr int NJ = 2, NW = 8, NSLOT = 4; static constexpr bool RES = false; };
+
+constexpr int T2_PR = 18, T2_SR = T2_PR * T2_PR;
+
+template <int C> constexpr int taps2d_x3_src() { return (T2_SR * (C / 8) + 63) & ~63; }
+struct taps2d_head { const float* w; float bias; float* mask; float* logits; };
+
+template <int C> constexpr int taps2d_x3_lds() { return Taps2dX3Cfg<C>::NSLOT * 2 * C * C * 2 + 2 * taps2d_x3_src<C>() * 16; }
+
+template <int C, bool HEAD>
+__global__ __launch_bounds__(64 * Taps2dX3Cfg<C>::NW, 2 * 4 / Taps2dX3Cfg<C>::NW)
+void conv_taps2d_x3_kernel(const advh_taps2d_desc p, long x_lo, long w_lo, long o_lo, const taps2d_head hd) {
+    static_assert(!HEAD || C == 32, "the mask head is a 32-channel dot product (unet_head_kernel's four 8-channel chains)");
+    constexpr int NJ = Taps2dX3Cfg<C>::NJ, NW = Taps2dX3Cfg<C>::NW, NSLOT = Taps2dX3Cfg<C>::NSLOT;
+    constexpr bool RES = Taps2dX3Cfg<C>::RES;
+    static_assert(NJ * NW == 16, "one 16 x 16 output tile per workgroup");
+    constexpr int CH = C / 8, CT = C / 16, KS = C / 32, NTH = 64 * NW, WTAP = C * C * 2, SRC = taps2d_x3_src<C>();
+    constexpr int AHEAD = NSLOT - 1, WPT = RES ? 0 : 2 * (C * CH / NTH);
+    static_assert(RES || C * CH == NTH, "a streamed tap is one 16-byte chunk per thread and plane");
+    extern __shared__ __attribute__((aligned(16))) char lds[];
+    const int tid = threadIdx.x, lane = tid & 63, wv = tid >> 6;
+    const int fr = lane & 15, g = lane >> 4;
+    char* Wl = lds;
+    char* Xl = lds + NSLOT * 2 * WTAP;
+    const _Float16* Wg = (const _Float16*)p.W;
+    const _Float16* X = (const _Float16*)p.X;
+    const int Hp = p.H + 2 * p.PH, Wp = p.W_ + 2 * p.PW;
+    const int tx = (p.W_ + 15) / 16, ty = (p.H + 15) / 16, ntiles = p.B * ty * tx;
+    auto origin = [&](int tile, int& b, int& y0, int& x0) {
+        x0 = (tile % tx) * 16;
+        const int r = tile / tx;
+        y0 = (r % ty) * 16;
+        b = r / ty;
+    };
+    auto load_weights = [&](int t, int slot) {
+        char* dst = Wl + (size_t)slot * 2 * WTAP;
+        for (int i = tid; i < C * CH; i += NTH) {
+            const int row = i / CH, pos = i % CH;
+            const _Float16* src = Wg + ((long)t * C + cout_of2(row)) * C + ((pos ^ swz2<C>(row)) * 8);
+            __builtin_amdgcn_global_load_lds(GLOBAL_PTR(src), LDS_PTR(dst + (size_t)(i - lane) * 16), 16, 0, 0);
+            __builtin_amdgcn_global_load_lds(GLOBAL_PTR(src + w_lo), LDS_PTR(dst + WTAP + (size_t)(i - lane) * 16), 16, 0, 0);
+        }
+    };
+    auto load_patch = [&](int tile) {
+        int b, y0, x0;
+        origin(tile, b, y0, x0);
+        for (int i = tid; i < SRC; i += NTH) {
+            int row = i / CH;
+            const int pos = i % CH;
+            if (row >= T2_SR) row = 0;
+            const int gy = min(y0 + p.PH - 1 + row / T2_PR, Hp - 1), gx = min(x0 + p.PW - 1 + row % T2_PR, Wp - 1);
+            const _Float16* src = X + (((long)b * Hp + gy) * Wp + gx) * C + ((pos ^ swz2<C>(i / CH)) * 8);
+            __builtin_amdgcn_global_load_lds(GLOBAL_PTR(src), LDS_PTR(Xl + (size_t)(i - lane) * 16), 16, 0, 0);
+            __builtin_amdgcn_global_load_lds(GLOBAL_PTR(src + x_lo), LDS_PTR(Xl + (size_t)SRC * 16 + (size_t)(i - lane) * 16), 16, 0, 0);
+        }
+    };
+    float4 bias[CT];
+#pragma unroll
+    for (int i = 0; i < CT; ++i)
+        bias[i] = p.bias ? *(const float4*)(p.bias + (i >> 1) * 32 + g * 8 + (i & 1) * 4) : make_float4(0.f, 0.f, 0.f, 0.f);
+    float hw[8];
+#pragma unroll
+    for (int r = 0; r < 8; ++r) hw[r] = HEAD ? hd.w[g * 8 + r] : 0.f;
+
+    const int mytiles = (int)blockIdx.x < ntiles ? (ntiles - 1 - (int)blockIdx.x) / (int)gridDim.x + 1 : 0;
+    const int ntot = mytiles * 9;
+    if (RES) {
+        if (mytiles)
+            for (int t = 0; t < 9; ++t) load_weights(t, t);
+    } else {
+        for (int n = 0; n < AHEAD && n < ntot; ++n) load_weights(n % 9, n % NSLOT);
+    }
+    if (mytiles) load_patch(blockIdx.x);
+    int n = 0;
+    for (int tile = blockIdx.x; tile < ntiles; tile += gridDim.x) {
+        f32x4 acc[CT][NJ], accx[CT][NJ];
+#pragma unroll
+        for (int i = 0; i < CT; ++i)
+#pragma unroll
+            for (int j = 0; j < NJ; ++j) { acc[i][j] = f32x4{0.f, 0.f, 0.f, 0.f}; accx[i][j] = f32x4{0.f, 0.f, 0.f, 0.f}; }
+        f16x8 fwh[2][CT], fwl[2][CT], fxh[2][NJ], fxl[2][NJ];
+        auto fetch = [&](int set, int slot, int t, int ks) {
+            const char* wb = Wl + (size_t)slot * 2 * WTAP;
+            const int c = ks * 4 + g, kh = t / 3, kw = t - kh * 3;
+#pragma unroll
+            for (int i = 0; i < CT; ++i) {
+                const int wo = ((i * 16 + fr) * CH + (c ^ swz2<C>(fr))) * 16;
+                fwh[set][i] = *(const f16x8*)(wb + wo);
+                fwl[set][i] = *(const f16x8*)(wb + WTAP + wo);
+            }
+#pragma unroll
+            for (int j = 0; j < NJ; ++j) {
+                const int row = (wv * NJ + j + kh) * T2_PR + kw + fr;
+                const int xo = (row * CH + (c ^ swz2<C>(row))) * 16;
+                fxh[set][j] = *(const f16x8*)(Xl + xo);
+                fxl[set][j] = *(const f16x8*)(Xl + (size_t)SRC * 16 + xo);
+            }
+        };
+        auto mma = [&](int set) {
+#pragma unroll
+            for (int j = 0; j < NJ; ++j) {
+#pragma unroll
+                for (int i = 0; i < CT; ++i) accx[i][j] = __builtin_amdgcn_mfma_f32_16x16x32_f16(fwh[set][i], fxl[set][j], accx[i][j], 0, 0, 0);
+#pragma unroll
+                for (int i = 0; i < CT; ++i) acc[i][j] = __builtin_amdgcn_mfma_f32_16x16x32_f16(fwh[set][i], fxh[set][j], acc[i][j], 0, 0, 0);
+#pragma unroll
+                for (int i = 0; i < CT; ++i) accx[i][j] = __builtin_amdgcn_mfma_f32_16x16x32_f16(fwl[set][i], fxh[set][j], accx[i][j], 0, 0, 0);
+            }
+        };
+        auto slot_of = [&](int t) { return RES ? t : (n + t) % NSLOT; };
+#pragma unroll
+        for (int t = 0; t < 9; ++t) {
+            if (t == 0 || !RES) {
+                if (t == 0 || n + t + 2 >= ntot) asm volatile("s_waitcnt vmcnt(0)" ::: "memory");
+                else asm volatile("s_waitcnt vmcnt(%0)" ::"n"(WPT) : "memory");
+                __syncthreads();
+                if (!RES && n + t + AHEAD < ntot) load_weights((n + t + AHEAD) % 9, (n + t + AHEAD) % NSLOT);
+            }
+            if (t == 0) fetch(0, slot_of(0), 0, 0);
+#pragma unroll
+            for (int ks = 0; ks < KS; ++ks) {
+                const int s = t * KS + ks, cur = s & 1;
+                if (ks + 1 < KS) fetch(cur ^ 1, slot_of(t), t, ks + 1);
+                else if (t + 1 < 9) fetch(cur ^ 1, slot_of(t + 1), t + 1, 0);
+                __builtin_amdgcn_sched_barrier(0);
+                mma(cur);
+                __builtin_amdgcn_sched_barrier(0);
+            }
+        }
+        n += 9;
+        if (tile + (int)gridDim.x < ntiles) {
+            __syncthreads();
+            load_patch(tile + gridDim.x);
+        }
+        int b, y0, x0;
+        origin(tile, b, y0, x0);
+#pragma unroll
+        for (int j = 0; j < NJ; ++j) {
+            const int gy = y0 + wv * NJ + j, gx = x0 + fr;
+            const bool inside = gy < p.H && gx < p.W_;
+            if (!HEAD && !inside) continue;
+            const long pos = ((long)b * Hp + gy + p.PH) * Wp + gx + p.PW;
+#pragma unroll
+            for (int q = 0; q < CT / 2; ++q) {
+                const long o = pos * C + q * 32 + g * 8;
+                float v[8];
+#pragma unroll
+                for (int r = 0; r < 4; ++r) {
+                    v[r] = fmaf(accx[2 * q][j][r], SPLIT_LO_INV, acc[2 * q][j][r]);
+                    v[4 + r] = fmaf(accx[2 * q + 1][j][r], SPLIT_LO_INV, acc[2 * q + 1][j][r]);
+                }
+                v[0] += bias[2 * q].x; v[1] += bias[2 * q].y; v[2] += bias[2 * q].z; v[3] += bias[2 * q].w;
+                v[4] += bias[2 * q + 1].x; v[5] += bias[2 * q + 1].y; v[6] += bias[2 * q + 1].z; v[7] += bias[2 * q + 1].w;
+                if (p.act == ADVH_ACT_LEAKY) {
+#pragma unroll
+                    for (int r = 0; r < 8; ++r) v[r] = v[r] > 0.f ? v[r] : p.slope * v[r];
+                }
+                if (!HEAD) {
+                    store_h_rt<8>((_Float16*)p.out_h, o, o_lo, v);
+                } else {
+                    if (!inside) {
+#pragma unroll
+                        for (int r = 0; r < 8; ++r) v[r] = 0.f;
+                    }
+                    f16x8 hv, lv;
+                    split_f32_vec<8>(v, hv, lv);
+                    float s = 0.f;
+#pragma unroll
+                    for (int r = 0; r < 8; ++r) s = fmaf(join_f32(hv[r], lv[r]), hw[r], s);
+                    s += __shfl_xor(s, 16, 64);
+                    s += __shfl_xor(s, 32, 64);
+                    s += hd.bias;
+                    if (g == 0 && inside) {
+                        const long i = ((long)b * p.H + gy) * p.W_ + gx;
+                        if (hd.logits) hd.logits[i] = s;
+                        hd.mask[i] = 1.f / (1.f + expf(-s));
+                    }
+                }
+            }
+        }
+    }
+    asm volatile("s_waitcnt vmcnt(0)" ::: "memory");
+}
+
+}
+
+inline int advh_taps2d_split_check(const advh_taps2d_desc* d, int C, int64_t x_lo, int64_t w_lo, int64_t o_lo, const advh::taps2d_head* hd,
+                                   int lds, long* grid) {
+    if (!d || !d->X || !d->W || (!hd && !d->out_h) || d->B <= 0 || d->H <= 0 || d->W_ <= 0 || d->PH < 1 || d->PW < 1) return ADVH_EINVAL;
+    if (hd && (!hd->w || !hd->mask)) return ADVH_EINVAL;
+    if (C != 32 && (hd || C != 64)) return ADVH_EUNSUPPORTED;
+    if (d->act != ADVH_ACT_NONE && d->act != ADVH_ACT_LEAKY) return ADVH_EINVAL;
+    if (!hd && d->X == d->out_h) return ADVH_EINVAL;
+    const long plane = (long)d->B * (d->H + 2 * d->PH) * (d->W_ + 2 * d->PW) * C;
+    if (x_lo < plane || (!hd && o_lo < plane) || w_lo < 9L * C * C || x_lo % 8 || w_lo % 8 || (!hd && o_lo % 8)) return ADVH_EINVAL;
+    const long ntiles = (long)d->B * ((d->H + 15) / 16) * ((d->W_ + 15) / 16);
+    if (ntiles > 0x7fffffffL) return ADVH_EINVAL;
+    const long per_cu = 160 * 1024 / lds;
+    *grid = ntiles < 256 * per_cu ? ntiles : 256 * per_cu;
+    return ADVH_OK;
+}
diff --git a/xai-audio-deepfakes_amd/csrc/conv_taps2d_x3.hip b/xai-audio-deepfakes_amd/csrc/conv_taps2d_x3.hip
--- a/xai-audio-deepfakes_amd/csrc/conv_taps2d_x3.hip
+++ b/xai-audio-deepfakes_amd/csrc/conv_taps2d_x3.hip
@@ -1,180 +1,4 @@
-#include <hip/hip_runtime.h>
-#include <hip/hip_fp16.h>
-#include "addvisor_hip.h"
-#include "common.h"
-#include "device_math.h"
-
-namespace advh {
-
-typedef _Float16 f16x8 __attribute__((ext_vector_type(8)));
-typedef float f32x4 __attribute__((ext_vector_type(4)));
-
-#define GLOBAL_PTR(p) ((const __attribute__((address_space(1))) void*)(p))
-#define LDS_PTR(p) ((__attribute__((address_space(3))) void*)(p))
-
-template <int C> __device__ __forceinline__ int swz2(int r) { return C == 64 ? (r & 7) : ((r >> 1) & 2); }
-__device__ __forceinline__ int cout_of2(int R) { return ((R >> 5) << 5) + (((R >> 2) & 3) << 3) + (((R >> 4) & 1) << 2) + (R & 3); }
-
-template <int C> struct Taps2dX3Cfg;
-template <> struct Taps2dX3Cfg<32> { static constexpr int NJ = 4, NW = 4, NSLOT = 9; static constexpr bool RES = true; };
-template <> struct Taps2dX3Cfg<64> { static constexpr int NJ = 2, NW = 8, NSLOT = 4; static constexpr bool RES = false; };
-
-constexpr int T2_PR = 18, T2_SR = T2_PR * T2_PR;
-
-template <int C> constexpr int taps2d_x3_src() { return (T2_SR * (C / 8) + 63) & ~63; }
-template <int C> constexpr int taps2d_x3_lds() { return Taps2dX3Cfg<C>::NSLOT * 2 * C * C * 2 + 2 * taps2d_x3_src<C>() * 16; }
-
-template <int C>
-__global__ __launch_bounds__(64 * Taps2dX3Cfg<C>::NW, 2 * 4 / Taps2dX3Cfg<C>::NW)
-void conv_taps2d_x3_kernel(const advh_taps2d_desc p, long x_lo, long w_lo, long o_lo) {
-    constexpr int NJ = Taps2dX3Cfg<C>::NJ, NW = Taps2dX3Cfg<C>::NW, NSLOT = Taps2dX3Cfg<C>::NSLOT;
-    constexpr bool RES = Taps2dX3Cfg<C>::RES;
-    static_assert(NJ * NW == 16, "one 16 x 16 output tile per workgroup");
-    constexpr int CH = C / 8, CT = C / 16, KS = C / 32, NTH = 64 * NW, WTAP = C * C * 2, SRC = taps2d_x3_src<C>();
-    constexpr int AHEAD = NSLOT - 1, WPT = RES ? 0 : 2 * (C * CH / NTH);
-    static_assert(RES || C * CH == NTH, "a streamed tap is one 16-byte chunk per thread and plane");
-    extern __shared__ __attribute__((aligned(16))) char lds[];
-    const int tid = threadIdx.x, lane = tid & 63, wv = tid >> 6;
-    const int fr = lane & 15, g = lane >> 4;
-    char* Wl = lds;
-    char* Xl = lds + NSLOT * 2 * WTAP;
-    const _Float16* Wg = (const _Float16*)p.W;
-    const _Float16* X = (const _Float16*)p.X;
-    const int Hp = p.H + 2 * p.PH, Wp = p.W_ + 2 * p.PW;
-    const int tx = (p.W_ + 15) / 16, ty = (p.H + 15) / 16, ntiles = p.B * ty * tx;
-    auto origin = [&](int tile, int& b, int& y0, int& x0) {
-        x0 = (tile % tx) * 16;
-        const int r = tile / tx;
-        y0 = (r % ty) * 16;
-        b = r / ty;
-    };
-    auto load_weights = [&](int t, int slot) {
-        char* dst = Wl + (size_t)slot * 2 * WTAP;
-        for (int i = tid; i < C * CH; i += NTH) {
-            const int row = i / CH, pos = i % CH;
-            const _Float16* src = Wg + ((long)t * C + cout_of2(row)) * C + ((pos ^ swz2<C>(row)) * 8);
-            __builtin_amdgcn_global_load_lds(GLOBAL_PTR(src), LDS_PTR(dst + (size_t)(i - lane) * 16), 16, 0, 0);
-            __builtin_amdgcn_global_load_lds(GLOBAL_PTR(src + w_lo), LDS_PTR(dst + WTAP + (size_t)(i - lane) * 16), 16, 0, 0);
-        }
-    };
-    auto load_patch = [&](int tile) {
-        int b, y0, x0;
-        origin(tile, b, y0, x0);
-        for (int i = tid; i < SRC; i += NTH) {
-            int row = i / CH;
-            const int pos = i % CH;
-            if (row >= T2_SR) row = 0;
-            const int gy = min(y0 + p.PH - 1 + row / T2_PR, Hp - 1), gx = min(x0 + p.PW - 1 + row % T2_PR, Wp - 1);
-            const _Float16* src = X + (((long)b * Hp + gy) * Wp + gx) * C + ((pos ^ swz2<C>(i / CH)) * 8);
-            __builtin_amdgcn_global_load_lds(GLOBAL_PTR(src), LDS_PTR(Xl + (size_t)(i - lane) * 16), 16, 0, 0);
-            __builtin_amdgcn_global_load_lds(GLOBAL_PTR(src + x_lo), LDS_PTR(Xl + (size_t)SRC * 16 + (size_t)(i - lane) * 16), 16, 0, 0);
-        }
-    };
-    float4 bias[CT];
-#pragma unroll
-    for (int i = 0; i < CT; ++i)
-        bias[i] = p.bias ? *(const float4*)(p.bias + (i >> 1) * 32 + g * 8 + (i & 1) * 4) : make_float4(0.f, 0.f, 0.f, 0.f);
-
-    const int mytiles = (int)blockIdx.x < ntiles ? (ntiles - 1 - (int)blockIdx.x) / (int)gridDim.x + 1 : 0;
-    const int ntot = mytiles * 9;
-    if (RES) {
-        if (mytiles)
-            for (int t = 0; t < 9; ++t) load_weights(t, t);
-    } else {
-        for (int n = 0; n < AHEAD && n < ntot; ++n) load_weights(n % 9, n % NSLOT);
-    }
-    if (mytiles) load_patch(blockIdx.x);
-    int n = 0;
-    for (int tile = blockIdx.x; tile < ntiles; tile += gridDim.x) {
-        f32x4 acc[CT][NJ], accx[CT][NJ];
-#pragma unroll
-        for (int i = 0; i < CT; ++i)
-#pragma unroll
-            for (int j = 0; j < NJ; ++j) { acc[i][j] = f32x4{0.f, 0.f, 0.f, 0.f}; accx[i][j] = f32x4{0.f, 0.f, 0.f, 0.f}; }
-        f16x8 fwh[2][CT], fwl[2][CT], fxh[2][NJ], fxl[2][NJ];
-        auto fetch = [&](int set, int slot, int t, int ks) {
-            const char* wb = Wl + (size_t)slot * 2 * WTAP;
-            const int c = ks * 4 + g, kh = t / 3, kw = t - kh * 3;
-#pragma unroll
-            for (int i = 0; i < CT; ++i) {
-                const int wo = ((i * 16 + fr) * CH + (c ^ swz2<C>(fr))) * 16;
-                fwh[set][i] = *(const f16x8*)(wb + wo);
-                fwl[set][i] = *(const f16x8*)(wb + WTAP + wo);
-            }
-#pragma unroll
-            for (int j = 0; j < NJ; ++j) {
-                const int row = (wv * NJ + j + kh) * T2_PR + kw + fr;
-                const int xo = (row * CH + (c ^ swz2<C>(row))) * 16;
-                fxh[set][j] = *(const f16x8*)(Xl + xo);
-                fxl[set][j] = *(const f16x8*)(Xl + (size_t)SRC * 16 + xo);
-            }
-        };
-        auto mma = [&](int set) {
-#pragma unroll
-            for (int j = 0; j < NJ; ++j) {
-#pragma unroll
-                for (int i = 0; i < CT; ++i) accx[i][j] = __builtin_amdgcn_mfma_f32_16x16x32_f16(fwh[set][i], fxl[set][j], accx[i][j], 0, 0, 0);
-#pragma unroll
-                for (int i = 0; i < CT; ++i) acc[i][j] = __builtin_amdgcn_mfma_f32_16x16x32_f16(fwh[set][i], fxh[set][j], acc[i][j], 0, 0, 0);
-#pragma unroll
-                for (int i = 0; i < CT; ++i) accx[i][j] = __builtin_amdgcn_mfma_f32_16x16x32_f16(fwl[set][i], fxh[set][j], accx[i][j], 0, 0, 0);
-            }
-        };
-        auto slot_of = [&](int t) { return RES ? t : (n + t) % NSLOT; };
-#pragma unroll
-        for (int t = 0; t < 9; ++t) {
-            if (t == 0 || !RES) {
-                if (t == 0 || n + t + 2 >= ntot) asm volatile("s_waitcnt vmcnt(0)" ::: "memory");
-                else asm volatile("s_waitcnt vmcnt(%0)" ::"n"(WPT) : "memory");
-                __syncthreads();
-                if (!RES && n + t + AHEAD < ntot) load_weights((n + t + AHEAD) % 9, (n + t + AHEAD) % NSLOT);
-            }
-            if (t == 0) fetch(0, slot_of(0), 0, 0);
-#pragma unroll
-            for (int ks = 0; ks < KS; ++ks) {
-                const int s = t * KS + ks, cur = s & 1;
-                if (ks + 1 < KS) fetch(cur ^ 1, slot_of(t), t, ks + 1);
-                else if (t + 1 < 9) fetch(cur ^ 1, slot_of(t + 1), t + 1, 0);
-                __builtin_amdgcn_sched_barrier(0);
-                mma(cur);
-                __builtin_amdgcn_sched_barrier(0);
-            }
-        }
-        n += 9;
-        if (tile + (int)gridDim.x < ntiles) {
-            __syncthreads();
-            load_patch(tile + gridDim.x);
-        }
-        int b, y0, x0;
-        origin(tile, b, y0, x0);
-#pragma unroll
-        for (int j = 0; j < NJ; ++j) {
-            const int gy = y0 + wv * NJ + j, gx = x0 + fr;
-            if (gy >= p.H || gx >= p.W_) continue;
-            const long pos = ((long)b * Hp + gy + p.PH) * Wp + gx + p.PW;
-#pragma unroll
-            for (int q = 0; q < CT / 2; ++q) {
-                const long o = pos * C + q * 32 + g * 8;
-                float v[8];
-#pragma unroll
-                for (int r = 0; r < 4; ++r) {
-                    v[r] = fmaf(accx[2 * q][j][r], SPLIT_LO_INV, acc[2 * q][j][r]);
-                    v[4 + r] = fmaf(accx[2 * q + 1][j][r], SPLIT_LO_INV, acc[2 * q + 1][j][r]);
-                }
-                v[0] += bias[2 * q].x; v[1] += bias[2 * q].y; v[2] += bias[2 * q].z; v[3] += bias[2 * q].w;
-                v[4] += bias[2 * q + 1].x; v[5] += bias[2 * q + 1].y; v[6] += bias[2 * q + 1].z; v[7] += bias[2 * q + 1].w;
-                if (p.act == ADVH_ACT_LEAKY) {
-#pragma unroll
-                    for (int r = 0; r < 8; ++r) v[r] = v[r] > 0.f ? v[r] : p.slope * v[r];
-                }
-                store_h_rt<8>((_Float16*)p.out_h, o, o_lo, v);
-            }
-        }
-    }
-    asm volatile("s_waitcnt vmcnt(0)" ::: "memory");
-}
-
-}
+#include "conv_taps2d_x3.h"
 
 using namespace advh;
 
@@ -183,21 +7,15 @@
 }
 
 extern "C" int advh_conv_taps2d_split(const advh_taps2d_desc* d, int C, int64_t x_lo, int64_t w_lo, int64_t o_lo, advh_stream_t stream) {
-    if (!d || !d->X || !d->W || !d->out_h || d->B <= 0 || d->H <= 0 || d->W_ <= 0 || d->PH < 1 || d->PW < 1) return ADVH_EINVAL;
-    if (C != 32 && C != 64) return ADVH_EUNSUPPORTED;
-    if (d->act != ADVH_ACT_NONE && d->act != ADVH_ACT_LEAKY) return ADVH_EINVAL;
-    if (d->X == d->out_h) return ADVH_EINVAL;
-    const long plane = (long)d->B * (d->H + 2 * d->PH) * (d->W_ + 2 * d->PW) * C;
-    if (x_lo < plane || o_lo < plane || w_lo < 9L * C * C || x_lo % 8 || w_lo % 8 || o_lo % 8) return ADVH_EINVAL;
-    const long ntiles = (long)d->B * ((d->H + 15) / 16) * ((d->W_ + 15) / 16);
-    if (ntiles > 0x7fffffffL) return ADVH_EINVAL;
     const int lds = advh_conv_taps2d_split_lds_bytes(C);
-    const void* fn = C == 64 ? (const void*)conv_taps2d_x3_kernel<64> : (const void*)conv_taps2d_x3_kernel<32>;
+    long grid = 0;
+    const int rc = advh_taps2d_split_check(d, C, x_lo, w_lo, o_lo, nullptr, lds, &grid);
+    if (rc != ADVH_OK) return rc;
+    const void* fn = C == 64 ? (const void*)conv_taps2d_x3_kernel<64, false> : (const void*)conv_taps2d_x3_kernel<32, false>;
     if (advh_ensure_lds(fn) != ADVH_OK) return ADVH_ELAUNCH;
-    const long per_cu = 160 * 1024 / lds;
-    const long grid = ntiles < 256 * per_cu ? ntiles : 256 * per_cu;
-    if (C == 64) hipLaunchKernelGGL(conv_taps2d_x3_kernel<64>, dim3((unsigned)grid), dim3(512), lds, (hipStream_t)stream, *d, (long)x_lo, (long)w_lo, (long)o_lo);
-    else hipLaunchKernelGGL(conv_taps2d_x3_kernel<32>, dim3((unsigned)grid), dim3(256), lds, (hipStream_t)stream, *d, (long)x_lo, (long)w_lo, (long)o_lo);
+    const taps2d_head none = {nullptr, 0.f, nullptr, nullptr};
+    if (C == 64) hipLaunchKernelGGL((conv_taps2d_x3_kernel<64, false>), dim3((unsigned)grid), dim3(512), lds, (hipStream_t)stream, *d, (long)x_lo, (long)w_lo, (long)o_lo, none);
+    else hipLaunchKernelGGL((conv_taps2d_x3_kernel<32, false>), dim3((unsigned)grid), dim3(256), lds, (hipStream_t)stream, *d, (long)x_lo, (long)w_lo, (long)o_lo, none);
     return ADVH_LAUNCH_CHECK();
 }
 
diff --git a/xai-audio-deepfakes_amd/csrc/stft.hip b/xai-audio-deepfakes_amd/csrc/stft.hip
--- a/xai-audio-deepfakes_amd/csrc/stft.hip
+++ b/xai-audio-deepfakes_amd/csrc/stft.hip
@@ -437,7 +437,7 @@
     int* dflag = nullptr;
     if (hipHostGetDevicePointer((void**)&dflag, g_split_flag_host, 0) != hipSuccess) return ADVH_ELAUNCH;
     int (*const setters[])(int*) = {advh_split_flag_attention, advh_split_flag_attention_bwd_f32, advh_split_flag_attention_bwd_x3, advh_split_flag_backward, advh_split_flag_conv_taps, advh_split_flag_frontend, advh_split_flag_frontend_bwd, advh_split_flag_gemm, advh_split_flag_hifigan, advh_split_flag_rowops, advh_split_flag_unet_misc, advh_split_flag_unet_train, advh_split_flag_resblock_pair_x3,
-                                   advh_split_flag_conv_taps2d_x3};
+                                   advh_split_flag_conv_taps2d_x3, advh_split_flag_conv_taps2d_head_x3, advh_split_flag_upconv_tile_x3};
     for (auto set : setters)
         if ((rc = set(dflag)) != ADVH_OK) return rc;
     g_init_done[dev] = true;
diff --git a/xai-audio-deepfakes_amd/csrc/upconv_tile_x3.hip b/xai-audio-deepfakes_amd/csrc/upconv_tile_x3.hip
--- /dev/null
+++ b/xai-audio-deepfakes_amd/csrc/upconv_tile_x3.hip
@@ -0,0 +1,187 @@
+#include <hip/hip_runtime.h>
+#include <hip/hip_fp16.h>
+#include "addvisor_hip.h"
+#include "common.h"
+#include "device_math.h"
+
+namespace advh {
+
+typedef _Float16 f16x8 __attribute__((ext_vector_type(8)));
+typedef float f32x4 __attribute__((ext_vector_type(4)));
+
+#define GLOBAL_PTR(p) ((const __attribute__((address_space(1))) void*)(p))
+#define LDS_PTR(p) ((__attribute__((address_space(3))) void*)(p))
+
+constexpr int UX_N = 32, UX_C0 = 64, UX_NS = 15, UX_NW = 8, UX_NTH = 64 * UX_NW;
+constexpr int UX_WCH = UX_NS * UX_N * 4;
+constexpr int UX_PR = 18, UX_CROWS = 17, UX_SROWS = 33;
+constexpr int UX_PC = UX_CROWS * UX_PR, UX_PS = UX_SROWS * UX_PR;
+constexpr int UX_CCH = (UX_PC * 8 + 63) & ~63, UX_SCH = (UX_PS + 63) & ~63;
+constexpr int UX_PLANE = (UX_CCH + UX_SCH) * 16;
+constexpr int UX_LDS = 2 * UX_WCH * 16 + 2 * UX_PLANE;
+static_assert(UX_WCH % 64 == 0, "the weights are whole-wave loads");
+static_assert(UX_LDS <= 160 * 1024, "one workgroup per CU");
+
+__global__ __launch_bounds__(UX_NTH, 1)
+void upconv21_tile_x3_kernel(const advh_upconv_desc p, long xc_lo, long xs_lo, long w_lo, long o_lo) {
+    extern __shared__ __attribute__((aligned(16))) char lds[];
+    const int tid = threadIdx.x, lane = tid & 63, wv = tid >> 6;
+    const int fr = lane & 15, g = lane >> 4;
+    char* Wl = lds;
+    char* Xl = lds + 2 * UX_WCH * 16;
+    const _Float16* Xc = (const _Float16*)p.Xc;
+    const _Float16* Xs = (const _Float16*)p.Xs;
+    const int Hf = 2 * p.Hc;
+    const int Hpc = p.Hc + 2 * p.PHc, Wpc = p.W_ + 2 * p.PWc, Hps = Hf + 2 * p.PHs, Wps = p.W_ + 2 * p.PWs;
+    const int Hpo = Hf + 2 * p.PHo, Wpo = p.W_ + 2 * p.PWo;
+    const int tx = (p.W_ + 15) / 16, ty = (Hf + 31) / 32, ntiles = p.B * ty * tx;
+    const int ph = (blockIdx.x >> 3) & 1, slot = (blockIdx.x & 7) + 8 * (blockIdx.x >> 4), nslots = gridDim.x >> 1;
+    if (slot >= ntiles) return;
+    auto origin = [&](int tile, int& b, int& y0, int& x0) {
+        x0 = (tile % tx) * 16;
+        const int r = tile / tx;
+        y0 = (r % ty) * 32;
+        b = r / ty;
+    };
+    const _Float16* Wg = (const _Float16*)p.W + (long)ph * (UX_WCH * 8);
+    for (int i = tid; i < UX_WCH; i += UX_NTH) {
+        const int row = i >> 2, pos = i & 3;
+        const _Float16* src = Wg + (long)row * 32 + ((pos ^ ((row >> 1) & 2)) * 8);
+        __builtin_amdgcn_global_load_lds(GLOBAL_PTR(src), LDS_PTR(Wl + (size_t)(i - lane) * 16), 16, 0, 0);
+        __builtin_amdgcn_global_load_lds(GLOBAL_PTR(src + w_lo), LDS_PTR(Wl + (size_t)UX_WCH * 16 + (size_t)(i - lane) * 16), 16, 0, 0);
+    }
+    auto load_patches = [&](int tile) {
+        int b, y0, x0;
+        origin(tile, b, y0, x0);
+        char* ds = Xl + UX_CCH * 16;
+        for (int i = tid; i < UX_CCH; i += UX_NTH) {
+            int row = i >> 3;
+            const int pos = i & 7;
+            if (row >= UX_PC) row = 0;
+            const int gy = min((y0 >> 1) + p.PHc - 1 + ph + row / UX_PR, Hpc - 1), gx = min(x0 + p.PWc - 1 + row % UX_PR, Wpc - 1);
+            const _Float16* src = Xc + (((long)b * Hpc + gy) * Wpc + gx) * UX_C0 + ((pos ^ ((i >> 3) & 7)) * 8);
+            __builtin_amdgcn_global_load_lds(GLOBAL_PTR(src), LDS_PTR(Xl + (size_t)(i - lane) * 16), 16, 0, 0);
+            __builtin_amdgcn_global_load_lds(GLOBAL_PTR(src + xc_lo), LDS_PTR(Xl + UX_PLANE + (size_t)(i - lane) * 16), 16, 0, 0);
+        }
+        for (int i = tid; i < UX_SCH; i += UX_NTH) {
+            const int row = i < UX_PS ? i : 0;
+            const int gy = min(y0 + p.PHs - 1 + ph + row / UX_PR, Hps - 1), gx = min(x0 + p.PWs - 1 + row % UX_PR, Wps - 1);
+            const _Float16* src = Xs + (((long)b * Hps + gy) * Wps + gx) * 8;
+            __builtin_amdgcn_global_load_lds(GLOBAL_PTR(src), LDS_PTR(ds + (size_t)(i - lane) * 16), 16, 0, 0);
+            __builtin_amdgcn_global_load_lds(GLOBAL_PTR(src + xs_lo), LDS_PTR(ds + UX_PLANE + (size_t)(i - lane) * 16), 16, 0, 0);
+        }
+    };
+    const int a0 = 2 * wv;
+    float4 bias[2];
+#pragma unroll
+    for (int e = 0; e < 2; ++e) bias[e] = p.bias ? *(const float4*)(p.bias + g * 8 + e * 4) : make_float4(0.f, 0.f, 0.f, 0.f);
+    const int wo0 = (fr * 4 + (g ^ ((fr >> 1) & 2))) * 16;
+
+    load_patches(slot);
+    for (int tile = slot; tile < ntiles; tile += nslots) {
+        f32x4 acc[2][2], accx[2][2];
+#pragma unroll
+        for (int i = 0; i < 2; ++i)
+#pragma unroll
+            for (int j = 0; j < 2; ++j) { acc[i][j] = f32x4{0.f, 0.f, 0.f, 0.f}; accx[i][j] = f32x4{0.f, 0.f, 0.f, 0.f}; }
+        f16x8 fwh[2][2], fwl[2][2], fxh[2][2], fxl[2][2];
+        auto fetch = [&](int set, int s) {
+#pragma unroll
+            for (int i = 0; i < 2; ++i) {
+                const int wo = wo0 + (s * UX_N + i * 16) * 64;
+                fwh[set][i] = *(const f16x8*)(Wl + wo);
+                fwl[set][i] = *(const f16x8*)(Wl + UX_WCH * 16 + wo);
+            }
+#pragma unroll
+            for (int j = 0; j < 2; ++j) {
+                int xo;
+                if (s < 12) {
+                    const int t = s >> 1, ti = t / 3, tj = t - ti * 3, c = (s & 1) * 4 + g;
+                    const int row = (a0 + j + ti) * UX_PR + tj + fr;
+                    xo = (row * 8 + (c ^ (row & 7))) * 16;
+                } else {
+                    const int tap = min(4 * (s - 12) + g, 8), kh = tap / 3, kw = tap - kh * 3;
+                    xo = UX_CCH * 16 + ((2 * (a0 + j) + kh) * UX_PR + kw + fr) * 16;
+                }
+                fxh[set][j] = *(const f16x8*)(Xl + xo);
+                fxl[set][j] = *(const f16x8*)(Xl + UX_PLANE + xo);
+            }
+        };
+        auto mma = [&](int set) {
+#pragma unroll
+            for (int j = 0; j < 2; ++j) {
+#pragma unroll
+                for (int i = 0; i < 2; ++i) accx[i][j] = __builtin_amdgcn_mfma_f32_16x16x32_f16(fwh[set][i], fxl[set][j], accx[i][j], 0, 0, 0);
+#pragma unroll
+                for (int i = 0; i < 2; ++i) acc[i][j] = __builtin_amdgcn_mfma_f32_16x16x32_f16(fwh[set][i], fxh[set][j], acc[i][j], 0, 0, 0);
+#pragma unroll
+                for (int i = 0; i < 2; ++i) accx[i][j] = __builtin_amdgcn_mfma_f32_16x16x32_f16(fwl[set][i], fxh[set][j], accx[i][j], 0, 0, 0);
+            }
+        };
+        asm volatile("s_waitcnt vmcnt(0)" ::: "memory");
+        __syncthreads();
+        fetch(0, 0);
+#pragma unroll
+        for (int s = 0; s < UX_NS; ++s) {
+            const int cur = s & 1;
+            if (s + 1 < UX_NS) fetch(cur ^ 1, s + 1);
+            __builtin_amdgcn_sched_barrier(0);
+            mma(cur);
+            __builtin_amdgcn_sched_barrier(0);
+        }
+        if (tile + nslots < ntiles) {
+            __syncthreads();
+            load_patches(tile + nslots);
+        }
+        int b, y0, x0;
+        origin(tile, b, y0, x0);
+#pragma unroll
+        for (int j = 0; j < 2; ++j) {
+            const int gy = y0 + 2 * (a0 + j) + ph, gx = x0 + fr;
+            if (gy >= Hf || gx >= p.W_) continue;
+            const long o = (((long)b * Hpo + gy + p.PHo) * Wpo + gx + p.PWo) * UX_N + g * 8;
+            float v[8];
+#pragma unroll
+            for (int r = 0; r < 4; ++r) {
+                v[r] = fmaf(accx[0][j][r], SPLIT_LO_INV, acc[0][j][r]);
+                v[4 + r] = fmaf(accx[1][j][r], SPLIT_LO_INV, acc[1][j][r]);
+            }
+            v[0] += bias[0].x; v[1] += bias[0].y; v[2] += bias[0].z; v[3] += bias[0].w;
+            v[4] += bias[1].x; v[5] += bias[1].y; v[6] += bias[1].z; v[7] += bias[1].w;
+            if (p.act == ADVH_ACT_LEAKY) {
+#pragma unroll
+                for (int r = 0; r < 8; ++r) v[r] = v[r] > 0.f ? v[r] : p.slope * v[r];
+            }
+            store_h_rt<8>((_Float16*)p.out_h, o, o_lo, v);
+        }
+    }
+    asm volatile("s_waitcnt vmcnt(0)" ::: "memory");
+}
+
+}
+
+using namespace advh;
+
+extern "C" int advh_upconv21_tile_split_lds_bytes(void) { return UX_LDS; }
+
+extern "C" int advh_upconv21_tile_split(const advh_upconv_desc* d, int Cc, int N, int64_t xc_lo, int64_t xs_lo, int64_t w_lo, int64_t o_lo,
+                                        advh_stream_t stream) {
+    if (!d || !d->Xc || !d->Xs || !d->W || !d->out_h || d->B <= 0 || d->Hc <= 0 || d->W_ <= 0) return ADVH_EINVAL;
+    if (d->PHc < 1 || d->PWc < 1 || d->PHs < 1 || d->PWs < 1 || d->PHo < 0 || d->PWo < 0) return ADVH_EINVAL;
+    if (Cc != UX_C0 || N != UX_N) return ADVH_EUNSUPPORTED;
+    if (d->act != ADVH_ACT_NONE && d->act != ADVH_ACT_LEAKY) return ADVH_EINVAL;
+    if (d->Xc == d->out_h || d->Xs == d->out_h) return ADVH_EINVAL;
+    const long Hf = 2L * d->Hc;
+    const long pc = (long)d->B * (d->Hc + 2 * d->PHc) * (d->W_ + 2 * d->PWc) * UX_C0, ps = (long)d->B * (Hf + 2 * d->PHs) * (d->W_ + 2 * d->PWs) * 8;
+    const long po = (long)d->B * (Hf + 2 * d->PHo) * (d->W_ + 2 * d->PWo) * UX_N;
+    if (xc_lo < pc || xs_lo < ps || o_lo < po || w_lo < 2L * UX_WCH * 8 || xc_lo % 8 || xs_lo % 8 || w_lo % 8 || o_lo % 8) return ADVH_EINVAL;
+    const long ntiles = (long)d->B * ((Hf + 31) / 32) * ((d->W_ + 15) / 16);
+    if (ntiles > 0x7fffffffL) return ADVH_EINVAL;
+    if (advh_ensure_lds((const void*)upconv21_tile_x3_kernel) != ADVH_OK) return ADVH_ELAUNCH;
+    const long grid = ntiles >= 128 ? 256 : 16 * ((ntiles + 7) / 8);
+    hipLaunchKernelGGL(upconv21_tile_x3_kernel, dim3((unsigned)grid), dim3(UX_NTH), UX_LDS, (hipStream_t)stream, *d, (long)xc_lo, (long)xs_lo,
+                       (long)w_lo, (long)o_lo);
+    return ADVH_LAUNCH_CHECK();
+}
+
+ADVH_SPLIT_FLAG_SETTER(advh_split_flag_upconv_tile_x3)
```

New measurement: 1383 explanations/s, median of 6. 1.01x the previous value.
